# instance-based-loc/instance-based-loc

Hardware: AMD Instinct MI355X
Metric: query-frames localized/sec (embed+match+register) (higher is better)
Workload: dtype f16 (ViT MFMA operands, f32 accumulate) / f32+f64 (match, registration); 1 GPU; T: dinov2_vitb14 crops 224^2 (Q=7), 10000-instance memory (E=4), FPFH+RANSAC+coloured ICP on 5000-pt clouds, whole-memory evaluate; synthetic objects of extent U[0.15, 0.6] m on a 2.50 m grid (SURVEY 8d's U[0.2, 1.5] m re-scoped: its 5 000 points are too sparse to survive the radius-outlier removal); memory_instances=10000, points_per_object=5000, resident_feature_bytes_per_point=264, parallelism=frames-dp1+memory-replicated

## Files before the change

### include/ibloc.h

```cpp
#ifndef IBLOC_H
#define IBLOC_H

#include <stdint.h>

#ifdef __cplusplus
extern "C" {
#endif

int ibl_version(void);
const char* ibl_last_error(void);

int ibl_prof_enable(int on);
int ibl_prof_read(int id, double* ms, double* units, int64_t* launches);


#define IBL_VIT_MAX_LAYERS 32
#define IBL_VIT_LAYERSCALE 1
#define IBL_VIT_PRE_LN 2
#define IBL_VIT_FINAL_LN 4
#define IBL_VIT_QUICK_GELU 8
#define IBL_VIT_PROJ 16
#define IBL_VIT_OUT_ALL_TOKENS 32
#define IBL_VIT_ACT_TERMS2 64
#define IBL_VIT_ACT_TERMS3 128
// ... 92 lines not shown

int ibl_preprocess_depth(const float* src, const int64_t* offsets, const int32_t* sizes, int n_crops, int out_h, int out_w,
                         int patch, int patch_k_pad, float dmin, float dmax, void* patches, void* stream);


int ibl_normalize_rows(const float* in, float* out, int64_t n_rows, int dim, void* stream);

int64_t ibl_closest_similarity_workspace_bytes(int64_t n_query, int64_t n_mem_rows);
int ibl_closest_similarity(const float* det, int64_t n_query, const float* mem, int64_t n_mem_rows,
                           const int32_t* emb_offsets, int64_t n_inst, int dim, float* out_sims,
                           uint16_t* out_aug, void* workspace, int64_t workspace_bytes, void* stream);

int ibl_topk_select(const uint16_t* aug, int64_t n_rows, int64_t ld, int n_cols, int k_hi, int k_lo, int index_base,
                    uint16_t* out_val, int32_t* out_idx, int32_t* out_cnt, void* stream);

int64_t ibl_match_topk_workspace_bytes(int64_t n_query, int64_t n_mem_rows, int64_t n_inst);
int ibl_match_topk(const float* det, int64_t n_query, const float* mem, int64_t n_mem_rows, const int32_t* emb_offsets, int64_t n_inst,
                   int dim, int k_hi, int k_lo, int index_base, uint16_t* out_val, int32_t* out_idx, int32_t* out_cnt, uint16_t* out_aug,
                   void* workspace, int64_t workspace_bytes, void* stream);


int ibl_assign_batch(const uint16_t* aug_half, const int32_t* q_per_frame, int n_frames, int q_stride,
                     int M, int num_per_length, int32_t* out_assn, int32_t* out_len, int32_t* out_count,
                     int max_assn, int n_threads);

int ibl_assign_candidates(const uint16_t* cand_val, const int32_t* cand_idx, const int32_t* cand_cnt, int64_t cand_stride,
                          const int32_t* row_first, const int32_t* q_per_frame, int n_frames, int M_total, int k_hi, int k_lo,
                          int num_per_length, int32_t* out_assn, int32_t* out_len, int32_t* out_count, uint8_t* out_exact,
                          int max_assn, int n_threads);


typedef struct ibl_comm ibl_comm;
int ibl_comm_unique_id(void* out, int out_bytes);
int ibl_comm_init(ibl_comm** out, int rank, int world, const void* unique_id, int id_bytes);
int ibl_comm_destroy(ibl_comm* comm);
int ibl_allgather_topk(ibl_comm* comm, const void* send, void* recv, int64_t bytes_per_rank, void* stream);
int ibl_alltoall(ibl_comm* comm, const void* send, void* recv, int64_t bytes_per_pair, void* stream);
int ibl_allreduce_min(ibl_comm* comm, float* buf, int64_t n, void* stream);
int ibl_allreduce_max_i32(ibl_comm* comm, int32_t* buf, int64_t n, void* stream);


typedef struct ibl_reg_ctx ibl_reg_ctx;
int ibl_reg_ctx_create(ibl_reg_ctx** out, int64_t arena_bytes);
int ibl_reg_ctx_destroy(ibl_reg_ctx* ctx);
int ibl_reg_ctx_reset(ibl_reg_ctx* ctx);
int64_t ibl_reg_ctx_high_water(const ibl_reg_ctx* ctx);
int ibl_reg_ctx_status(ibl_reg_ctx* ctx, int clear);


enum { IBL_DEPTH_F32 = 0, IBL_DEPTH_U16 = 1, IBL_DEPTH_F64 = 2 };
int ibl_unproject_masks(ibl_reg_ctx* ctx, const void* depth, int depth_type, const uint8_t* rgb, const uint8_t* masks, int n_masks,
                        int H, int W, double fx, double fy, double depth_factor, float* pts4, int64_t capacity,
                        int32_t* seg_off_dev, int32_t* seg_off_host, void* stream);
int ibl_unproject_masks_f64(ibl_reg_ctx* ctx, const void* depth, int depth_type, const uint8_t* rgb, const uint8_t* masks, int n_masks,
                            int H, int W, double fx, double fy, double depth_factor, float* pts4, double* pts3_f64, double* colors3_f64,
                            int64_t capacity, int32_t* seg_off_dev, int32_t* seg_off_host, void* stream);

int ibl_radius_outlier_batch(ibl_reg_ctx* ctx, const float* pts4, const int32_t* seg_off_dev, const int32_t* seg_off_host,
                             int n_seg, double radius, int nb_points, uint8_t* keep, void* stream);

int ibl_normals_fpfh_batch(ibl_reg_ctx* ctx, const float* pts4, const int32_t* seg_off_dev, const int32_t* seg_off_host,
                           int n_seg, double radius_normal, int max_nn_normal, double radius_feature, int max_nn_feature,
                           float* normals4, float* fpfh, void* stream);

#define IBL_REG_HAVE_COLORS 1
#define IBL_REG_CENTER 2
#define IBL_REG_FIXED_BUDGET 4
int ibl_register_batch(ibl_reg_ctx* ctx, const float* det_pts4, const int32_t* det_off_dev, const int32_t* det_off_host,
                       int n_det_seg, const float* mem_pts4, const int32_t* mem_off_dev, const int32_t* mem_off_host,
                       int n_mem_seg, const int32_t* job_src_seg, const int32_t* job_tgt_seg, int n_jobs, double voxel_size,
                       double global_dist_factor, double local_dist_factor, uint64_t seed, uint32_t job_id_base,
                       int64_t ransac_max_iter, int flags, double* T_out, double* rmse_out, double* fitness_out,
                       double* means_out, double* T_ransac_out, int64_t* ransac_stats_out, void* stream);

typedef struct {
    const float* normals4;
    const float* fpfh;
    const uint16_t* fpfh_split;
    const float* fpfh_norm;
    const float* grad4;
    const float* bbox;
    double voxel_size;
    double grad_radius;
} ibl_instance_features;
int ibl_instance_features_batch(ibl_reg_ctx* ctx, const float* pts4, const int32_t* seg_off_dev, const int32_t* seg_off_host,
                                int n_seg, double voxel_size, double grad_radius, float* normals4, float* fpfh, uint16_t* fpfh_split,
                                float* fpfh_norm, float* grad4, float* bbox_host, void* stream);
int ibl_register_batch_cached(ibl_reg_ctx* ctx, const float* det_pts4, const int32_t* det_off_dev, const int32_t* det_off_host,
                              int n_det_seg, const float* mem_pts4, const int32_t* mem_off_dev, const int32_t* mem_off_host,
                              int n_mem_seg, const int32_t* job_src_seg, const int32_t* job_tgt_seg, int n_jobs, double voxel_size,
                              double global_dist_factor, double local_dist_factor, uint64_t seed, uint32_t job_id_base,
                              int64_t ransac_max_iter, int flags, const ibl_instance_features* det_features,
                              const ibl_instance_features* mem_features, double* T_out, double* rmse_out, double* fitness_out,
                              double* means_out, double* T_ransac_out, int64_t* ransac_stats_out, int64_t* reuse_stats_out,
                              void* stream);
int ibl_register_batch_ids(ibl_reg_ctx* ctx, const float* det_pts4, const int32_t* det_off_dev, const int32_t* det_off_host,
                           int n_det_seg, const float* mem_pts4, const int32_t* mem_off_dev, const int32_t* mem_off_host,
                           int n_mem_seg, const int32_t* job_src_seg, const int32_t* job_tgt_seg, const uint32_t* job_ids, int n_jobs,
                           double voxel_size, double global_dist_factor, double local_dist_factor, uint64_t seed,
                           int64_t ransac_max_iter, int flags, const ibl_instance_features* det_features,
                           const ibl_instance_features* mem_features, double* T_out, double* rmse_out, double* fitness_out,
                           double* means_out, double* T_ransac_out, int64_t* ransac_stats_out, int64_t* reuse_stats_out, void* stream);


int ibl_voxel_downsample_batch(ibl_reg_ctx* ctx, const double* points, const double* colors, const int32_t* seg_off_host, int32_t n_seg,
                               double voxel_size, double* out_points, double* out_colors, int32_t* out_counts,
                               int32_t* out_seg_off_host, void* stream);

int ibl_dbscan_batch(ibl_reg_ctx* ctx, const double* points, const int32_t* grp_off_host, int32_t n_grp, double eps, int32_t min_points,
                     int32_t* labels, int32_t* n_clusters_host, void* stream);

typedef struct ibl_memgrid ibl_memgrid;
int ibl_memgrid_build(ibl_reg_ctx* ctx, const float* mem_pts4, int64_t n, double cell, ibl_memgrid** out, void* stream);
int ibl_memgrid_destroy(ibl_memgrid* grid);

int ibl_evaluate_batch(ibl_reg_ctx* ctx, const ibl_memgrid* grid, const float* det_pts4, const int32_t* job_begin,
                       const int32_t* job_end, const double* T_global, int n_jobs, double threshold, double* rmse_out,
                       double* fitness_out, void* stream);

int ibl_register_evaluate_batch(ibl_reg_ctx* ctx, const float* det_pts4, const int32_t* det_off_dev, const int32_t* det_off_host,
                                int n_det_seg, const int32_t* q_per_frame, int n_frames, const int32_t* assn, const int32_t* assn_len,
                                const int32_t* assn_count, int max_assn, const float* mem_pts4, const int32_t* mem_off_dev,
                                const int32_t* mem_off_host, int n_mem_seg, const ibl_instance_features* mem_features,
                                const ibl_memgrid* grid, double voxel_size, double global_dist_factor, double local_dist_factor,
                                double outlier_radius, int outlier_nb_points, double eval_threshold, uint64_t seed, uint32_t job_id_base,
                                int64_t ransac_max_iter, int flags, int max_jobs, int32_t* clean_off_host, int32_t* n_jobs_out,
                                double* T_out, double* rmse_out, double* fitness_out, double* means_out, double* T_ransac_out,
                                int64_t* ransac_stats_out, int64_t* reuse_stats_out, double* T_global_out, double* full_rmse_out,
                                double* full_fitness_out, int32_t* best_out, void* stream);

int ibl_evaluate_points(ibl_reg_ctx* ctx, const ibl_memgrid* grid, const float* det_pts4, const int32_t* job_begin,
                        const int32_t* job_end, const double* T_global, int n_jobs, double threshold, float* d2_out, double* rmse_out,
                        double* fitness_out, void* stream);

int ibl_obb_iou_matrix(ibl_reg_ctx* ctx, const double* boxes, const int32_t* valid, int64_t n, double* dist,
                       int64_t* n_overlapping, void* stream);

#ifdef __cplusplus
}
#endif
#endif
```

### instance-based-loc_amd/_lib.py

```python
import ctypes as C
import os

import torch

_HERE = os.path.dirname(os.path.abspath(__file__))
LIB_PATH = os.environ.get("IBLOC_LIB") or os.path.join(_HERE, "libibloc_hip.so")


class IblError(RuntimeError):
    pass


def _load():
    if not os.path.exists(LIB_PATH):
        raise IblError(
            f"{LIB_PATH} not found: build it with `python -c 'import __graft_entry__ as g; g.build()'` "
            "(or `make -C instance-based-loc_amd/csrc`). There is no CPU fallback.")
    return C.CDLL(LIB_PATH)


lib = _load()

c_i32p = C.POINTER(C.c_int32)
c_u16p = C.POINTER(C.c_uint16)
vp = C.c_void_p

_SIGS = {
    "ibl_version": (C.c_int, []),
    "ibl_last_error": (C.c_char_p, []),
    "ibl_prof_enable": (C.c_int, [C.c_int]),
    "ibl_prof_read": (C.c_int, [C.c_int, C.POINTER(C.c_double), C.POINTER(C.c_double), C.POINTER(C.c_int64)]),
    "ibl_normalize_rows": (C.c_int, [vp, vp, C.c_int64, C.c_int, vp]),
    "ibl_closest_similarity_workspace_bytes": (C.c_int64, [C.c_int64, C.c_int64]),
    "ibl_closest_similarity": (C.c_int, [vp, C.c_int64, vp, C.c_int64, vp, C.c_int64, C.c_int, vp, vp, vp,
                                         C.c_int64, vp]),
    "ibl_preprocess_crops": (C.c_int, [vp, vp, C.c_int, C.c_int, vp, vp, C.c_int, C.c_int, C.c_int, C.c_int, C.c_int,
                                       vp, vp, vp, vp, vp]),
    "ibl_vit_workspace_bytes": (C.c_int64, [vp, C.c_int]),
    "ibl_linear_f16": (C.c_int, [vp, C.c_int64, vp, C.c_int64, vp, vp, C.c_int64, C.c_int, C.c_int, C.c_int, vp, C.c_int64, vp]),
    "ibl_vit_forward": (C.c_int, [vp, vp, vp, C.c_int, vp, vp, C.c_int64, vp]),
    "ibl_attention_f16": (C.c_int, [vp, vp, C.c_int, C.c_int, C.c_int, C.c_int, C.c_int, C.c_int, vp]),
    "ibl_layernorm_f32": (C.c_int, [vp, C.c_int64, C.c_int64, C.c_int, vp, vp, C.c_float, vp, C.c_int64, C.c_int, vp]),
    "ibl_reg_ctx_create": (C.c_int, [C.POINTER(vp), C.c_int64]),
    "ibl_reg_ctx_destroy": (C.c_int, [vp]),
    "ibl_reg_ctx_reset": (C.c_int, [vp]),
    "ibl_reg_ctx_high_water": (C.c_int64, [vp]),
    "ibl_reg_ctx_status": (C.c_int, [vp, C.c_int]),
    "ibl_unproject_masks": (C.c_int, [vp, vp, C.c_int, vp, vp, C.c_int, C.c_int, C.c_int, C.c_double, C.c_double, C.c_double, vp, C.c_int64,
                                      vp, vp, vp]),
    "ibl_voxel_downsample_batch": (C.c_int, [vp, vp, vp, vp, C.c_int32, C.c_double, vp, vp, vp, vp, vp]),
    "ibl_dbscan_batch": (C.c_int, [vp, vp, vp, C.c_int32, C.c_double, C.c_int32, vp, vp, vp]),
    "ibl_unproject_masks_f64": (C.c_int, [vp, vp, C.c_int, vp, vp, C.c_int, C.c_int, C.c_int, C.c_double, C.c_double, C.c_double, vp, vp, vp,
                                          C.c_int64, vp, vp, vp]),
    "ibl_radius_outlier_batch": (C.c_int, [vp, vp, vp, vp, C.c_int, C.c_double, C.c_int, vp, vp]),
    "ibl_normals_fpfh_batch": (C.c_int, [vp, vp, vp, vp, C.c_int, C.c_double, C.c_int, C.c_double, C.c_int, vp, vp, vp]),
    "ibl_register_batch": (C.c_int, [vp, vp, vp, vp, C.c_int, vp, vp, vp, C.c_int, vp, vp, C.c_int, C.c_double, C.c_double,
                                     C.c_double, C.c_uint64, C.c_uint32, C.c_int64, C.c_int, vp, vp, vp, vp, vp, vp, vp]),
    "ibl_instance_features_batch": (C.c_int, [vp, vp, vp, vp, C.c_int, C.c_double, C.c_double, vp, vp, vp, vp, vp, vp, vp]),
    "ibl_register_batch_cached": (C.c_int, [vp, vp, vp, vp, C.c_int, vp, vp, vp, C.c_int, vp, vp, C.c_int, C.c_double, C.c_double,
                                            C.c_double, C.c_uint64, C.c_uint32, C.c_int64, C.c_int, vp, vp, vp, vp, vp, vp, vp, vp,
                                            vp, vp]),
    "ibl_register_batch_ids": (C.c_int, [vp, vp, vp, vp, C.c_int, vp, vp, vp, C.c_int, vp, vp, vp, C.c_int, C.c_double, C.c_double,
                                         C.c_double, C.c_uint64, C.c_int64, C.c_int, vp, vp, vp, vp, vp, vp, vp, vp, vp, vp]),
    "ibl_memgrid_build": (C.c_int, [vp, vp, C.c_int64, C.c_double, C.POINTER(vp), vp]),
    "ibl_memgrid_destroy": (C.c_int, [vp]),
    "ibl_evaluate_batch": (C.c_int, [vp, vp, vp, vp, vp, vp, C.c_int, C.c_double, vp, vp, vp]),
    "ibl_register_evaluate_batch": (C.c_int, [vp, vp, vp, vp, C.c_int, vp, C.c_int, vp, vp, vp, C.c_int, vp, vp, vp, C.c_int, vp, vp,
                                              C.c_double, C.c_double, C.c_double, C.c_double, C.c_int, C.c_double, C.c_uint64, C.c_uint32,
                                              C.c_int64, C.c_int, C.c_int, vp, vp, vp, vp, vp, vp, vp, vp, vp, vp, vp, vp, vp, vp]),
    "ibl_evaluate_points": (C.c_int, [vp, vp, vp, vp, vp, vp, C.c_int, C.c_double, vp, vp, vp, vp]),
    "ibl_dator_head_workspace_bytes": (C.c_int64, [C.c_int]),
    "ibl_dator_head_forward": (C.c_int, [vp, vp, vp, C.c_int, vp, vp, C.c_int64, vp]),
    "ibl_preprocess_depth": (C.c_int, [vp, vp, vp, C.c_int, C.c_int, C.c_int, C.c_int, C.c_int, C.c_float, C.c_float, vp, vp]),
    "ibl_assign_batch": (C.c_int, [vp, vp, C.c_int, C.c_int, C.c_int, C.c_int, vp, vp, vp, C.c_int, C.c_int]),
    "ibl_assign_candidates": (C.c_int, [vp, vp, vp, C.c_int64, vp, vp, C.c_int, C.c_int, C.c_int, C.c_int, C.c_int, vp, vp, vp, vp,
                                        C.c_int, C.c_int]),
    "ibl_resample_ksize": (C.c_int, [C.c_int, C.c_int, C.c_int]),
    "ibl_resample_table": (C.c_int, [C.c_int, C.c_int, C.c_int, C.c_int, C.c_int, vp]),
    "ibl_comm_unique_id": (C.c_int, [vp, C.c_int]),
    "ibl_comm_init": (C.c_int, [vp, C.c_int, C.c_int, vp, C.c_int]),
    "ibl_comm_destroy": (C.c_int, [vp]),
    "ibl_allgather_topk": (C.c_int, [vp, vp, vp, C.c_int64, vp]),
    "ibl_alltoall": (C.c_int, [vp, vp, vp, C.c_int64, vp]),
    "ibl_allreduce_min": (C.c_int, [vp, vp, C.c_int64, vp]),
    "ibl_allreduce_max_i32": (C.c_int, [vp, vp, C.c_int64, vp]),
    "ibl_topk_select": (C.c_int, [vp, C.c_int64, C.c_int64, C.c_int, C.c_int, C.c_int, C.c_int, vp, vp, vp, vp]),
    "ibl_match_topk_workspace_bytes": (C.c_int64, [C.c_int64, C.c_int64, C.c_int64]),
    "ibl_match_topk": (C.c_int, [vp, C.c_int64, vp, C.c_int64, vp, C.c_int64, C.c_int, C.c_int, C.c_int, C.c_int, vp, vp, vp, vp, vp,
                                 C.c_int64, vp]),
    "ibl_obb_iou_matrix": (C.c_int, [vp, vp, vp, C.c_int64, vp, vp, vp]),
}


def _bind():
    for name, (res, args) in _SIGS.items():
        fn = getattr(lib, name)
        fn.restype = res
        fn.argtypes = args


_bind()


def check(status, what=""):
    if status != 0:
        msg = lib.ibl_last_error()
        raise IblError(f"{what} failed ({status}): {msg.decode() if msg else ''}")


def declared_symbols():
    return list(_SIGS.keys())
```

### instance-based-loc_amd/csrc/localise.hip

```cpp
#pragma clang fp contract(off)
#include <hip/hip_runtime.h>
#include <hipcub/hipcub.hpp>

#include <cmath>
#include <vector>

#include "ibloc.h"
#include "reg_common.h"

namespace {

struct KeepToInt {
    __host__ __device__ __forceinline__ int operator()(unsigned char v) const { return v ? 1 : 0; }
};

__global__ __launch_bounds__(256) void ibl_compact_kept_kernel(const float4* __restrict__ pts, const unsigned char* __restrict__ keep,
                                                               const int* __restrict__ pos, int n, float4* __restrict__ clean) {
    const int i = blockIdx.x * 256 + threadIdx.x;
    if (i < n && keep[i]) clean[pos[i]] = pts[i];
}

__global__ __launch_bounds__(256) void ibl_compact_offsets_kernel(const int* __restrict__ seg_off, const int* __restrict__ pos, int n_seg,
                                                                  int* __restrict__ new_off) {
    const int s = blockIdx.x * 256 + threadIdx.x;
// ... 3 lines not shown
}

extern "C" int ibl_register_evaluate_batch(ibl_reg_ctx* ctx, const float* det_pts4, const int32_t* det_off_dev, const int32_t* det_off_host,
                                           int n_det_seg, const int32_t* q_per_frame, int n_frames, const int32_t* assn,
                                           const int32_t* assn_len, const int32_t* assn_count, int max_assn, const float* mem_pts4,
                                           const int32_t* mem_off_dev, const int32_t* mem_off_host, int n_mem_seg,
                                           const ibl_instance_features* mem_features, const ibl_memgrid* grid, double voxel_size,
                                           double global_dist_factor, double local_dist_factor, double outlier_radius, int outlier_nb_points,
                                           double eval_threshold, uint64_t seed, uint32_t job_id_base, int64_t ransac_max_iter, int flags,
                                           int max_jobs, int32_t* clean_off_host, int32_t* n_jobs_out, double* T_out, double* rmse_out,
                                           double* fitness_out, double* means_out, double* T_ransac_out, int64_t* ransac_stats_out,
                                           int64_t* reuse_stats_out, double* T_global_out, double* full_rmse_out, double* full_fitness_out,
                                           int32_t* best_out, void* stream) {
    if (!ctx || !det_pts4 || !det_off_dev || !det_off_host || !q_per_frame || !assn || !assn_len || !assn_count || !mem_pts4 || !mem_off_dev ||
        !mem_off_host || !mem_features || !grid || !clean_off_host || !n_jobs_out || !T_out || !rmse_out || !fitness_out || !means_out ||
        !T_global_out || !full_rmse_out || !full_fitness_out || !best_out)
        return ibl_set_error(IBL_ERR_ARG, "ibl_register_evaluate_batch: null pointer");
    if (n_frames < 0 || n_det_seg < 0 || max_assn <= 0 || voxel_size <= 0 || outlier_radius <= 0 || eval_threshold <= 0)
        return ibl_set_error(IBL_ERR_ARG, "ibl_register_evaluate_batch: bad sizes");
    hipStream_t s = (hipStream_t)stream;
    std::vector<int> row0(n_frames + 1, 0);
    for (int f = 0; f < n_frames; ++f) {
        if (q_per_frame[f] < 0 || q_per_frame[f] > 7) return ibl_set_error(IBL_ERR_ARG, "ibl_register_evaluate_batch: q_per_frame out of range");
        row0[f + 1] = row0[f] + q_per_frame[f];
    }
    if (row0[n_frames] != n_det_seg) return ibl_set_error(IBL_ERR_ARG, "ibl_register_evaluate_batch: detections per frame do not add up to the segments");
    std::vector<int32_t> job_src, job_tgt;
    std::vector<int> job_frame, first_job(n_frames + 1, 0);
    for (int f = 0; f < n_frames; ++f) {
        const int na = assn_count[f];
        if (na < 0 || na > max_assn) return ibl_set_error(IBL_ERR_ARG, "ibl_register_evaluate_batch: assignment count out of range");
        for (int a = 0; a < na; ++a) {
            const int len = assn_len[(size_t)f * max_assn + a];
            if (len < 1 || len > 3) return ibl_set_error(IBL_ERR_ARG, "ibl_register_evaluate_batch: an assignment has 1 to 3 pairs");
            const int32_t* pr = assn + ((size_t)f * max_assn + a) * 6;
            for (int t = 0; t < 3; ++t) {
                if (t < len) {
                    if (pr[2 * t] < 0 || pr[2 * t] >= q_per_frame[f] || pr[2 * t + 1] < 0 || pr[2 * t + 1] >= n_mem_seg)
                        return ibl_set_error(IBL_ERR_ARG, "ibl_register_evaluate_batch: assignment index out of range");
                    job_src.push_back(row0[f] + pr[2 * t]);
                    job_tgt.push_back(pr[2 * t + 1]);
                } else {
                    job_src.push_back(-1);
                    job_tgt.push_back(-1);
                }
            }
            job_frame.push_back(f);
        }
        first_job[f + 1] = (int)job_frame.size();
    }
    const int J = (int)job_frame.size();
    *n_jobs_out = J;
    for (int f = 0; f < n_frames; ++f) best_out[f] = -1;
    if (J > max_jobs) return ibl_set_error(IBL_ERR_ARG, "ibl_register_evaluate_batch: %d jobs, the output arrays hold %d", J, max_jobs);

    ArenaMark mark(ctx);
    const int n = det_off_host[n_det_seg];
    unsigned char* keep; int *pos, *new_off; float4* clean;
    IBL_ARENA(keep, unsigned char, (int64_t)n + 64);
    IBL_ARENA(pos, int, (int64_t)n + 64);
    IBL_ARENA(new_off, int, n_det_seg + 2);
    IBL_ARENA(clean, float4, (int64_t)n + 1);
    for (int i = 0; i <= n_det_seg; ++i) clean_off_host[i] = 0;
    if (n > 0) {
        int st = ibl_radius_outlier_batch(ctx, det_pts4, det_off_dev, det_off_host, n_det_seg, outlier_radius, outlier_nb_points, keep, stream);
        if (st) return st;
        IBL_HIP_CHECK(hipMemsetAsync(keep + n, 0, 1, s));
        size_t tmp_bytes = 0;
        hipcub::TransformInputIterator<int, KeepToInt, const unsigned char*> flags(keep, KeepToInt());
        IBL_HIP_CHECK(hipcub::DeviceScan::ExclusiveSum(nullptr, tmp_bytes, flags, pos, n + 1, s));
        unsigned char* tmp;
        IBL_ARENA(tmp, unsigned char, (int64_t)tmp_bytes + 256);
        IBL_HIP_CHECK(hipcub::DeviceScan::ExclusiveSum(tmp, tmp_bytes, flags, pos, n + 1, s));
        hipLaunchKernelGGL(ibl_compact_kept_kernel, dim3((n + 255) / 256), dim3(256), 0, s, reinterpret_cast<const float4*>(det_pts4), keep, pos, n, clean);
        IBL_LAUNCH_CHECK();
        hipLaunchKernelGGL(ibl_compact_offsets_kernel, dim3((n_det_seg + 256) / 256), dim3(256), 0, s, det_off_dev, pos, n_det_seg, new_off);
        IBL_LAUNCH_CHECK();
        IBL_HIP_CHECK(hipMemcpyAsync(clean_off_host, new_off, sizeof(int) * (size_t)(n_det_seg + 1), hipMemcpyDeviceToHost, s));
        IBL_HIP_CHECK(hipStreamSynchronize(s));
    }
    if (J == 0) return IBL_OK;
    const int nc = clean_off_host[n_det_seg];

    float4* nrm; float* fpfh; uint16_t* split; float* fnorm;
    IBL_ARENA(nrm, float4, (int64_t)nc + 1);
    IBL_ARENA(fpfh, float, (int64_t)nc * 33 + 64);
    IBL_ARENA(split, uint16_t, (int64_t)nc * 48 + 64);
    IBL_ARENA(fnorm, float, (int64_t)nc + 64);
    std::vector<float> bbox((size_t)n_det_seg * 6 + 6, 0.0f);
    int st = ibl_instance_features_batch(ctx, reinterpret_cast<const float*>(clean), new_off, clean_off_host, n_det_seg, voxel_size, 0.0,
                                         reinterpret_cast<float*>(nrm), fpfh, split, fnorm, nullptr, bbox.data(), stream);
    if (st) return st;
    ibl_instance_features det_feat{reinterpret_cast<const float*>(nrm), fpfh, split, fnorm, nullptr, bbox.data(), voxel_size, 0.0};

    st = ibl_register_batch_cached(ctx, reinterpret_cast<const float*>(clean), new_off, clean_off_host, n_det_seg, mem_pts4, mem_off_dev,
                                   mem_off_host, n_mem_seg, job_src.data(), job_tgt.data(), J, voxel_size, global_dist_factor, local_dist_factor,
                                   seed, job_id_base, ransac_max_iter, flags, &det_feat, mem_features, T_out, rmse_out, fitness_out, means_out,
                                   T_ransac_out, ransac_stats_out, reuse_stats_out, stream);
    if (st) return st;

    std::vector<int32_t> jb(J), je(J);
    for (int j = 0; j < J; ++j) {
        const double* T = T_out + 16 * (size_t)j;
        const double* dm = means_out + 6 * (size_t)j;
        const double* mm = dm + 3;
        double* G = T_global_out + 16 * (size_t)j;
        for (int i = 0; i < 16; ++i) G[i] = T[i];
        for (int r = 0; r < 3; ++r) G[4 * r + 3] = T[4 * r + 3] + mm[r] - ((T[4 * r] * dm[0] + T[4 * r + 1] * dm[1]) + T[4 * r + 2] * dm[2]);
        const int f = job_frame[j];
        jb[j] = clean_off_host[row0[f]];
        je[j] = clean_off_host[row0[f + 1]];
    }
    st = ibl_evaluate_batch(ctx, grid, reinterpret_cast<const float*>(clean), jb.data(), je.data(), T_global_out, J, eval_threshold, full_rmse_out,
                            full_fitness_out, stream);
    if (st) return st;

    for (int f = 0; f < n_frames; ++f) {
        int best = -1;
        for (int j = first_job[f]; j < first_job[f + 1]; ++j)
            if (best < 0 || full_fitness_out[j] > full_fitness_out[best]) best = j;
        best_out[f] = best < 0 ? -1 : best - first_job[f];
    }
    return IBL_OK;
}
```

### instance-based-loc_amd/csrc/reg_api.hip

```cpp
#pragma clang fp contract(off)
#include <hip/hip_runtime.h>

#include <hipcub/hipcub.hpp>

#include <vector>

#include "ibloc.h"
#include "reg_common.h"

#ifndef KNN_CELLS_NORMAL
#define KNN_CELLS_NORMAL 3.0
#endif
#ifndef KNN_CELLS_FEATURE
#define KNN_CELLS_FEATURE 5.0
#endif

#ifndef KNN_TILE_NORMAL
#define KNN_TILE_NORMAL 4
#endif
#ifndef KNN_TILE_FEATURE
#define KNN_TILE_FEATURE 2
#endif

int ibl_launch_normals(ibl_reg_ctx* ctx, const BatchGrid& g, const float4* pts, const int* seg_off, int n, double radius, int max_nn, float4* normals,
                       int* status, hipStream_t s);
int ibl_launch_fpfh(ibl_reg_ctx* ctx, const BatchGrid& g, const float4* pts, const float4* normals, const int* seg_off, int n, double radius, int max_nn,
                    unsigned char* spfh, int* nbr_idx, float* nbr_d2, int* nbr_cnt, float* fpfh, int matching_order, int* status,
                    hipStream_t s);
int ibl_launch_radius_count(const BatchGrid& g, const float4* pts, const int* seg_off, int n, double radius, int nb_points,
                            unsigned char* keep, hipStream_t s);

bool ibl_normals_fpfh_fusable(double radius_normal, int max_nn_normal, double radius_feature, int max_nn_feature);
int ibl_launch_normals_fpfh(ibl_reg_ctx* ctx, const BatchGrid& g, const float4* pts, const int* seg_off, int n, double radius_normal,
                            int max_nn_normal, double radius_feature, int max_nn_feature, float4* normals, unsigned char* spfh, int* nbr_idx,
                            float* nbr_d2, int* nbr_cnt, float* fpfh, int matching_order, int* status, hipStream_t s);
int ibl_launch_color_grad(ibl_reg_ctx* ctx, const BatchGrid& g, const float4* pts, const float4* normals, const int* seg_off, int q0, int q1, double radius,
                          int max_nn, float4* grad, int* status, hipStream_t s);

static int ibl_bbox_to_host(ibl_reg_ctx* ctx, const float4* P, const int* seg_off_dev, int n_seg, float* bbox_host, hipStream_t s) {
    if (n_seg <= 0) return IBL_OK;
    ArenaMark m(ctx);
    float* bbox;
    IBL_ARENA(bbox, float, (int64_t)n_seg * 6 + 6);
    int st = ibl_launch_bbox(P, seg_off_dev, n_seg, bbox, s);
    if (st) return st;
    IBL_HIP_CHECK(hipMemcpyAsync(bbox_host, bbox, sizeof(float) * 6 * (size_t)n_seg, hipMemcpyDeviceToHost, s));
    IBL_HIP_CHECK(hipStreamSynchronize(s));
    return IBL_OK;
}

extern "C" int ibl_reg_ctx_create(ibl_reg_ctx** out, int64_t arena_bytes) {
    if (!out || arena_bytes < (1 << 20)) return ibl_set_error(IBL_ERR_ARG, "ibl_reg_ctx_create: bad argument");
    ibl_reg_ctx* c = new ibl_reg_ctx();
    IBL_HIP_CHECK(hipGetDevice(&c->device));
    hipError_t e = hipMalloc(reinterpret_cast<void**>(&c->base), (size_t)arena_bytes);
    if (e != hipSuccess) {
        delete c;
        return ibl_set_error(IBL_ERR_HIP, "ibl_reg_ctx_create: hipMalloc(%lld) failed: %s", (long long)arena_bytes, hipGetErrorString(e));
    }
    c->size = arena_bytes;
    c->d_status = reinterpret_cast<int*>(c->base);
    c->used = 256;
    e = hipMemset(c->base, 0, 256);
    if (e != hipSuccess) { (void)hipFree(c->base); delete c; return ibl_set_error(IBL_ERR_HIP, "ibl_reg_ctx_create: memset failed"); }
    c->pin_size = 32 << 20;
    if (hipHostMalloc(reinterpret_cast<void**>(&c->pin), (size_t)c->pin_size, hipHostMallocDefault) != hipSuccess) { c->pin = nullptr; c->pin_size = 0; }
    *out = c;
    return IBL_OK;
}

extern "C" int ibl_reg_ctx_destroy(ibl_reg_ctx* ctx) {
    if (!ctx) return IBL_OK;
    (void)hipFree(ctx->base);
    if (ctx->pin) (void)hipHostFree(ctx->pin);
    delete ctx;
    return IBL_OK;
}

extern "C" int ibl_reg_ctx_reset(ibl_reg_ctx* ctx) {
    if (!ctx) return ibl_set_error(IBL_ERR_ARG, "ibl_reg_ctx_reset: null context");
    ctx->used = 256;
    return IBL_OK;
}

extern "C" int64_t ibl_reg_ctx_high_water(const ibl_reg_ctx* ctx) { return ctx ? ctx->high_water : -1; }

extern "C" int ibl_reg_ctx_status(ibl_reg_ctx* ctx, int clear) {
    if (!ctx) return -1;
    int h = 0;
    if (hipMemcpy(&h, ctx->d_status, sizeof(int), hipMemcpyDeviceToHost) != hipSuccess) return -1;
    if (clear) (void)hipMemset(ctx->d_status, 0, sizeof(int));
    return h;
}

static int check_seg(const int32_t* seg_off_host, int n_seg, const char* who) {
    if (!seg_off_host || n_seg < 0) return ibl_set_error(IBL_ERR_ARG, "%s: bad segment table", who);
    if (seg_off_host[0] != 0) return ibl_set_error(IBL_ERR_ARG, "%s: seg_off[0] must be 0", who);
    for (int s = 0; s < n_seg; ++s)
        if (seg_off_host[s + 1] < seg_off_host[s]) return ibl_set_error(IBL_ERR_ARG, "%s: seg_off must be non-decreasing", who);
    return IBL_OK;
}

extern "C" int ibl_radius_outlier_batch(ibl_reg_ctx* ctx, const float* pts4, const int32_t* seg_off_dev, const int32_t* seg_off_host,
                                        int n_seg, double radius, int nb_points, uint8_t* keep, void* stream) {
    if (!ctx || !pts4 || !seg_off_dev || !keep || radius <= 0) return ibl_set_error(IBL_ERR_ARG, "ibl_radius_outlier_batch: bad argument");
    int st = check_seg(seg_off_host, n_seg, "ibl_radius_outlier_batch");
    if (st) return st;
    ArenaMark mark(ctx);
    hipStream_t s = (hipStream_t)stream;
    BatchGrid g;
    void* tok;
    ibl_prof_begin(IBL_PROF_ST_OUTLIER, 13.0 * (double)seg_off_host[n_seg], s, &tok);
    st = ibl_build_batch_grid(ctx, reinterpret_cast<const float4*>(pts4), seg_off_dev, seg_off_host, n_seg, (float)radius,
                              (int64_t)64 << 20, &g, s);
    if (st) return st;
    st = ibl_launch_radius_count(g, reinterpret_cast<const float4*>(pts4), seg_off_dev, seg_off_host[n_seg], radius, nb_points, keep, s);
    ibl_prof_end(tok, s);
    return st;
}

extern "C" int ibl_normals_fpfh_batch(ibl_reg_ctx* ctx, const float* pts4, const int32_t* seg_off_dev, const int32_t* seg_off_host,
                                      int n_seg, double radius_normal, int max_nn_normal, double radius_feature, int max_nn_feature,
                                      float* normals4, float* fpfh, void* stream) {
    if (!ctx || !pts4 || !seg_off_dev || !normals4 || radius_normal <= 0 || max_nn_normal <= 0)
        return ibl_set_error(IBL_ERR_ARG, "ibl_normals_fpfh_batch: bad argument");
    int st = check_seg(seg_off_host, n_seg, "ibl_normals_fpfh_batch");
    if (st) return st;
    const int n = seg_off_host[n_seg];
    ArenaMark mark(ctx);
    hipStream_t s = (hipStream_t)stream;
    const float4* P = reinterpret_cast<const float4*>(pts4);
    std::vector<float> bbox_host((size_t)n_seg * 6 + 6);
    st = ibl_bbox_to_host(ctx, P, seg_off_dev, n_seg, bbox_host.data(), s);
    if (st) return st;
    const bool fused = fpfh && radius_feature > 0 && max_nn_feature > 0 && ibl_normals_fpfh_fusable(radius_normal, max_nn_normal, radius_feature, max_nn_feature);
    if (!fused) {
        ArenaMark m2(ctx);
        BatchGrid g;
        st = ibl_build_tile_grid(ctx, P, seg_off_dev, seg_off_host, n_seg, bbox_host.data(), radius_normal, max_nn_normal, KNN_TILE_NORMAL,
                                 (int64_t)64 << 20, &g, s);
        if (st) return st;
        st = ibl_launch_normals(ctx, g, P, seg_off_dev, n, radius_normal, max_nn_normal, reinterpret_cast<float4*>(normals4), ctx->d_status, s);
        if (st) return st;
    }
    if (fpfh) {
        if (radius_feature <= 0 || max_nn_feature <= 0) return ibl_set_error(IBL_ERR_ARG, "ibl_normals_fpfh_batch: bad feature parameters");
        BatchGrid g;
        st = ibl_build_tile_grid(ctx, P, seg_off_dev, seg_off_host, n_seg, bbox_host.data(), radius_feature, max_nn_feature, KNN_TILE_FEATURE,
                                 (int64_t)64 << 20, &g, s);
        if (st) return st;
        unsigned char* spfh; int* nbr_idx; float* nbr_d2; int* nbr_cnt;
        IBL_ARENA(spfh, unsigned char, (int64_t)n * 36 + 64);
        IBL_ARENA(nbr_idx, int, (int64_t)n * max_nn_feature + 64);
        IBL_ARENA(nbr_d2, float, (int64_t)n * max_nn_feature + 64);
        IBL_ARENA(nbr_cnt, int, n + 64);
        if (fused)
            st = ibl_launch_normals_fpfh(ctx, g, P, seg_off_dev, n, radius_normal, max_nn_normal, radius_feature, max_nn_feature,
                                         reinterpret_cast<float4*>(normals4), spfh, nbr_idx, nbr_d2, nbr_cnt, fpfh, 0, ctx->d_status, s);
        else
            st = ibl_launch_fpfh(ctx, g, P, reinterpret_cast<const float4*>(normals4), seg_off_dev, n, radius_feature, max_nn_feature, spfh,
                                 nbr_idx, nbr_d2, nbr_cnt, fpfh, 0, ctx->d_status, s);
        if (st) return st;
    }
    IBL_HIP_CHECK(hipStreamSynchronize(s));
    ibl_stage_reset(ctx);
    return IBL_OK;
}

__global__ __launch_bounds__(256) void ibl_fpfh_half_kernel(const float* __restrict__ fpfh, int n, unsigned short* __restrict__ split,
                                                            float* __restrict__ norm) {
    const int i = blockIdx.x * 256 + threadIdx.x;
    if (i >= n) return;
    const float* __restrict__ x = fpfh + (int64_t)i * 33;
    const float a = fm_centred_norm(x);
    norm[i] = a;
    if (!split) return;
    uint4* dst = reinterpret_cast<uint4*>(split + (int64_t)i * 48);
#pragma unroll
    for (int pc = 0; pc < 6; ++pc) {
        float x8[8];
#pragma unroll
        for (int e = 0; e < 8; ++e) x8[e] = 8 * pc + e < 33 ? x[8 * pc + e] : 0.0f;
        const fm_piece_t r = fm_operand_piece(x8, a, pc);
        uint4 v;
        __builtin_memcpy(&v, &r, 16);
        dst[pc] = v;
    }
}

int ibl_features_on_batch(ibl_reg_ctx* ctx, const float4* P, const int* seg_off_dev, const int* seg_off_host, int n_seg, const float* bbox_host,
                          double voxel_size, double grad_radius, int gq0, int gq1, float4* normals, float* fpfh, unsigned short* fpfh_split,
                          float* fpfh_norm, float4* grad, hipStream_t s) {
    const int n = seg_off_host[n_seg];
    if (n <= 0) return IBL_OK;
    int st;
    std::vector<float> own_bbox;
    if (!bbox_host) {
        own_bbox.resize((size_t)n_seg * 6 + 6);
        st = ibl_bbox_to_host(ctx, P, seg_off_dev, n_seg, own_bbox.data(), s);
        if (st) return st;
        bbox_host = own_bbox.data();
    }
    const bool fused = fpfh && ibl_normals_fpfh_fusable(voxel_size * 2, 30, voxel_size * 5, 100);
    if (!fused) {
        ArenaMark mA(ctx);
        BatchGrid gA;
        st = ibl_build_tile_grid(ctx, P, seg_off_dev, seg_off_host, n_seg, bbox_host, voxel_size * 2, 30, KNN_TILE_NORMAL, (int64_t)128 << 20, &gA, s);
        if (st) return st;
        st = ibl_launch_normals(ctx, gA, P, seg_off_dev, n, voxel_size * 2, 30, normals, ctx->d_status, s);
        if (st) return st;
    }
    if (fpfh) {
        ArenaMark mB(ctx);
        BatchGrid gB;
        st = ibl_build_tile_grid(ctx, P, seg_off_dev, seg_off_host, n_seg, bbox_host, voxel_size * 5, 100, KNN_TILE_FEATURE, (int64_t)128 << 20, &gB, s);
        if (st) return st;
        unsigned char* spfh; float* nbr_d2; int *nbr_idx, *nbr_cnt;
        IBL_ARENA(spfh, unsigned char, (int64_t)n * 36 + 64);
        IBL_ARENA(nbr_idx, int, (int64_t)n * 100 + 64);
        IBL_ARENA(nbr_d2, float, (int64_t)n * 100 + 64);
        IBL_ARENA(nbr_cnt, int, n + 64);
        if (fused) st = ibl_launch_normals_fpfh(ctx, gB, P, seg_off_dev, n, voxel_size * 2, 30, voxel_size * 5, 100, normals, spfh, nbr_idx, nbr_d2, nbr_cnt,
                                                fpfh, 1, ctx->d_status, s);
        else st = ibl_launch_fpfh(ctx, gB, P, normals, seg_off_dev, n, voxel_size * 5, 100, spfh, nbr_idx, nbr_d2, nbr_cnt, fpfh, 1, ctx->d_status, s);
        if (st) return st;
        if (fpfh_norm) {
            hipLaunchKernelGGL(ibl_fpfh_half_kernel, dim3((unsigned)((n + 255) / 256)), dim3(256), 0, s, fpfh, n, fpfh_split, fpfh_norm);
            IBL_LAUNCH_CHECK();
        }
    }
    if (grad && gq1 > gq0) {
        if (grad_radius <= 0) return ibl_set_error(IBL_ERR_ARG, "colour gradients need a positive radius");
        ArenaMark mG(ctx);
        BatchGrid gG;
        st = ibl_build_tile_grid(ctx, P, seg_off_dev, seg_off_host, n_seg, bbox_host, grad_radius, 30, KNN_TILE_NORMAL, (int64_t)128 << 20, &gG, s);
        if (st) return st;
        st = ibl_launch_color_grad(ctx, gG, P, normals, seg_off_dev, gq0, gq1, grad_radius, 30, grad, ctx->d_status, s);
        if (st) return st;
    }
    return IBL_OK;
}

extern "C" int ibl_instance_features_batch(ibl_reg_ctx* ctx, const float* pts4, const int32_t* seg_off_dev, const int32_t* seg_off_host,
                                           int n_seg, double voxel_size, double grad_radius, float* normals4, float* fpfh,
                                           uint16_t* fpfh_split, float* fpfh_norm, float* grad4, float* bbox_host, void* stream) {
    if (!ctx || !pts4 || !seg_off_dev || !normals4 || !fpfh || !fpfh_norm || voxel_size <= 0)
        return ibl_set_error(IBL_ERR_ARG, "ibl_instance_features_batch: bad argument");
    if (grad4 && grad_radius <= 0) return ibl_set_error(IBL_ERR_ARG, "ibl_instance_features_batch: colour gradients need grad_radius > 0");
    int st = check_seg(seg_off_host, n_seg, "ibl_instance_features_batch");
    if (st) return st;
    ArenaMark mark(ctx);
    hipStream_t s = (hipStream_t)stream;
    const float4* P = reinterpret_cast<const float4*>(pts4);
    std::vector<float> own_bbox;
    if (!bbox_host) { own_bbox.resize((size_t)n_seg * 6 + 6); bbox_host = own_bbox.data(); }
    if (n_seg > 0) {
        st = ibl_bbox_to_host(ctx, P, seg_off_dev, n_seg, bbox_host, s);
        if (st) return st;
    }
    void* tok;
    ibl_prof_begin(IBL_PROF_ST_FEATURES, 444.0 * (double)(n_seg > 0 ? seg_off_host[n_seg] : 0), s, &tok);
    const int64_t total_pts = n_seg > 0 ? (int64_t)seg_off_host[n_seg] : 0;
    const int64_t cap_pts = (int64_t)3 << 19;
    const int64_t n_chunks = std::max<int64_t>(1, (total_pts + cap_pts - 1) / cap_pts);
    const int64_t chunk_pts = std::min<int64_t>(cap_pts, (total_pts + n_chunks - 1) / n_chunks + 65536);
    std::vector<int> rebased;
    for (int s0 = 0; s0 < n_seg;) {
        int s1 = s0 + 1;
        while (s1 < n_seg && (int64_t)seg_off_host[s1 + 1] - seg_off_host[s0] <= chunk_pts) ++s1;
        const int o0 = seg_off_host[s0], ns = s1 - s0;
        ArenaMark mc(ctx);
        const int* off_dev = seg_off_dev;
        const int* off_host = seg_off_host;
        if (!(s0 == 0 && s1 == n_seg)) {
            rebased.resize(ns + 1);
            for (int i = 0; i <= ns; ++i) rebased[i] = seg_off_host[s0 + i] - o0;
            int* d;
            IBL_ARENA(d, int, ns + 1);
            st = ibl_stage_upload(ctx, d, rebased.data(), sizeof(int) * (int64_t)(ns + 1), s);
            if (st) return st;
            off_dev = d;
            off_host = rebased.data();
        }
        const int cnt = off_host[ns];
        st = ibl_features_on_batch(ctx, P + o0, off_dev, off_host, ns, bbox_host + 6 * (size_t)s0, voxel_size, grad_radius, 0, grad4 ? cnt : 0,
                                   reinterpret_cast<float4*>(normals4) + o0, fpfh + (int64_t)o0 * 33, fpfh_split ? fpfh_split + (int64_t)o0 * 48 : nullptr,
                                   fpfh_norm + o0, grad4 ? reinterpret_cast<float4*>(grad4) + o0 : nullptr, s);
        if (st) return st;
        s0 = s1;
        if (ctx->pin_used > ctx->pin_size / 2) {
            IBL_HIP_CHECK(hipStreamSynchronize(s));
            ibl_stage_reset(ctx);
        }
    }
    ibl_prof_end(tok, s);
    IBL_HIP_CHECK(hipStreamSynchronize(s));
    ibl_stage_reset(ctx);
    return IBL_OK;
}

__device__ __forceinline__ double depth_at(const void* depth, int type, int64_t p) {
    return type == 1 ? (double)reinterpret_cast<const unsigned short*>(depth)[p]
                     : (type == 2 ? reinterpret_cast<const double*>(depth)[p] : (double)reinterpret_cast<const float*>(depth)[p]);
}
__device__ __forceinline__ double depth_z(const void* depth, int type, int64_t p, double factor) {
    if (type == 0) return (double)(reinterpret_cast<const float*>(depth)[p] / (float)factor);
    return depth_at(depth, type, p) / factor;
}

__global__ __launch_bounds__(256) void ibl_unproject_flag_kernel(const void* __restrict__ depth, int is_u16, const unsigned char* __restrict__ masks,
                                                                 int64_t HW, int64_t total, double depth_factor, int* __restrict__ flags) {
    const int64_t t = (int64_t)blockIdx.x * 256 + threadIdx.x;
    if (t >= total) return;
    const int64_t p = t % HW;
    const double z = depth_z(depth, is_u16, p, depth_factor);
    flags[t] = (masks[t] != 0 && z != 0.0) ? 1 : 0;
}

__global__ __launch_bounds__(256) void ibl_unproject_write_kernel(const void* __restrict__ depth, int is_u16, const unsigned char* __restrict__ rgb,
                                                                  const int* __restrict__ flags, const int* __restrict__ pos, int64_t HW, int W,
                                                                  int64_t total, const float* __restrict__ hx, const float* __restrict__ vy,
                                                                  double fx, double fy, double depth_factor, int64_t capacity,
                                                                  float4* __restrict__ out, double* __restrict__ out_pts64, double* __restrict__ out_cols64) {
    const int64_t t = (int64_t)blockIdx.x * 256 + threadIdx.x;
    if (t >= total || !flags[t]) return;
    const int o = pos[t];
    if (o >= capacity) return;
    const int64_t p = t % HW;
    const int row = (int)(p / W), col = (int)(p - (int64_t)row * W);
    const double z = depth_z(depth, is_u16, p, depth_factor);
    double x, y;
    if (is_u16 == 0) {
        const float zf = (float)z;
        x = (double)((hx[col] * zf) / (float)fx);
        y = (double)((vy[row] * zf) / (float)fy);
    } else {
        x = (double)hx[col] * z / fx;
        y = (double)vy[row] * z / fy;
    }
    const float r = (float)rgb[3 * p] / 255.0f, g = (float)rgb[3 * p + 1] / 255.0f, b = (float)rgb[3 * p + 2] / 255.0f;
    const double inten = ((double)r + (double)g + (double)b) / 3.0;
    out[o] = make_float4((float)x, (float)y, (float)z, (float)inten);
    if (out_pts64) {
        out_pts64[3 * (int64_t)o] = x; out_pts64[3 * (int64_t)o + 1] = y; out_pts64[3 * (int64_t)o + 2] = is_u16 == 0 ? (double)(float)z : z;
    }
    if (out_cols64) { out_cols64[3 * (int64_t)o] = (double)r; out_cols64[3 * (int64_t)o + 1] = (double)g; out_cols64[3 * (int64_t)o + 2] = (double)b; }
}

static void linspace_f32(double start, double stop, int num, std::vector<float>& out) {
    out.resize(num);
    if (num == 1) { out[0] = (float)start; return; }
    const double step = (stop - start) / (double)(num - 1);
    for (int i = 0; i < num; ++i) {
        volatile double prod = (double)i * step;
        out[i] = (float)(prod + start);
    }
    out[num - 1] = (float)stop;
}

extern "C" int ibl_unproject_masks_f64(ibl_reg_ctx* ctx, const void* depth, int depth_type, const uint8_t* rgb, const uint8_t* masks,
                                       int n_masks, int H, int W, double fx, double fy, double depth_factor, float* pts4, double* pts3_f64,
                                       double* colors3_f64, int64_t capacity, int32_t* seg_off_dev, int32_t* seg_off_host, void* stream);

extern "C" int ibl_unproject_masks(ibl_reg_ctx* ctx, const void* depth, int depth_type, const uint8_t* rgb, const uint8_t* masks,
                                   int n_masks, int H, int W, double fx, double fy, double depth_factor, float* pts4, int64_t capacity,
                                   int32_t* seg_off_dev, int32_t* seg_off_host, void* stream) {
    return ibl_unproject_masks_f64(ctx, depth, depth_type, rgb, masks, n_masks, H, W, fx, fy, depth_factor, pts4, nullptr, nullptr, capacity,
                                   seg_off_dev, seg_off_host, stream);
}

extern "C" int ibl_unproject_masks_f64(ibl_reg_ctx* ctx, const void* depth, int depth_type, const uint8_t* rgb, const uint8_t* masks,
                                       int n_masks, int H, int W, double fx, double fy, double depth_factor, float* pts4, double* pts3_f64,
                                       double* colors3_f64, int64_t capacity, int32_t* seg_off_dev, int32_t* seg_off_host, void* stream) {
    if (!ctx || !seg_off_dev || !seg_off_host || n_masks < 0 || (n_masks > 0 && (!depth || !rgb || !masks || !pts4)) || H <= 0 || W <= 0 || fx == 0 || fy == 0 ||
        depth_factor == 0 || capacity < 0 || depth_type < 0 || depth_type > 2)
        return ibl_set_error(IBL_ERR_ARG, "ibl_unproject_masks: bad argument");
// ... 40 lines not shown
```

### instance-based-loc_amd/csrc/reg_common.h

```cpp
#pragma once
#include <hip/hip_runtime.h>

#include <cstdint>

#include "ibl_common.h"

struct SegGrid {
    float minx, miny, minz, inv;
    int nx, ny, nz;
    int cell_base;
};

struct BatchGrid {
    const SegGrid* seg;
    const int* cell_start;
    const float4* sorted_pts;
    const int* order;
    int n_seg;
    const int* tile_base;
    const int* tile_seg;
    int n_tiles;
    int ts;
};

struct ibl_reg_ctx {
    unsigned char* base = nullptr;
    int64_t size = 0;
    int64_t used = 0;
    int64_t high_water = 0;
    int device = 0;
    int* d_status = nullptr;
    unsigned char* pin = nullptr;
    int64_t pin_size = 0;
    int64_t pin_used = 0;
};

int ibl_stage_upload(ibl_reg_ctx* ctx, void* dst_dev, const void* src_host, int64_t bytes, hipStream_t s);
static inline void ibl_stage_reset(ibl_reg_ctx* ctx) { ctx->pin_used = 0; }

struct ArenaMark {
    ibl_reg_ctx* ctx;
    int64_t mark;
    explicit ArenaMark(ibl_reg_ctx* c) : ctx(c), mark(c->used) {}
    ~ArenaMark() { ctx->used = mark; }
};

template <typename T>
static inline T* arena_alloc(ibl_reg_ctx* ctx, int64_t count, bool* ok) {
    int64_t bytes = ibl_align_up(count * (int64_t)sizeof(T), 256);
    if (bytes < 256) bytes = 256;
    if (ctx->used + bytes > ctx->size) {
        *ok = false;
        return nullptr;
    }
    T* p = reinterpret_cast<T*>(ctx->base + ctx->used);
    ctx->used += bytes;
    if (ctx->used > ctx->high_water) ctx->high_water = ctx->used;
    return p;
}

#define IBL_ARENA(ptr, type, count)                                                                  \
    do {                                                                                             \
        bool _ok = true;                                                                             \
        ptr = arena_alloc<type>(ctx, (count), &_ok);                                                 \
        if (!_ok)                                                                                    \
            return ibl_set_error(IBL_ERR_ARENA, "device arena exhausted (%lld of %lld bytes used, need %lld more) at %s:%d", \
                                 (long long)ctx->used, (long long)ctx->size,                         \
                                 (long long)((count) * (int64_t)sizeof(type)), __FILE__, __LINE__);  \
    } while (0)

#define IBL_ERR_ARENA (-5)
#define IBL_ERR_OVERFLOW (-6)

#define IBL_ST_GRID_OVERFLOW 1
#define IBL_ST_KNN_SLOWPATH 2
#define IBL_ST_FEAT_OVERFLOW 4
#define IBL_ST_RANSAC_OVERFLOW 8
#define IBL_ST_FEAT_REDONE 16
#define IBL_ST_RANSAC_REDONE 32

int ibl_build_batch_grid(ibl_reg_ctx* ctx, const float4* pts, const int* seg_off_dev, const int* seg_off_host, int n_seg,
                         float cell, int64_t max_cells, BatchGrid* out, hipStream_t s);
int ibl_build_batch_grid_bounded(ibl_reg_ctx* ctx, const float4* pts, const int* seg_off_dev, const int* seg_off_host, int n_seg,
                                 float cell, int64_t cells_bound, BatchGrid* out, hipStream_t s);
double ibl_knn_safety();
int ibl_knn_rho();
int ibl_build_tile_grid(ibl_reg_ctx* ctx, const float4* pts, const int* seg_off_dev, const int* seg_off_host, int n_seg,
                        const float* bbox_host, double radius, int max_nn, int ts, int64_t max_cells, BatchGrid* out, hipStream_t s);

int ibl_launch_bbox(const float4* pts, const int* seg_off_dev, int n_seg, float* bbox_dev, hipStream_t s);

struct FeatSources { const float4* normals[3]; const float* fpfh[3]; const float4* grad[3]; const unsigned short* split[3]; const float* norm[3]; };
struct FeatPair { int qkind, qsrc, qcnt, dkind, dsrc, dcnt, out, pad; };

int ibl_feat_search_mfma(ibl_reg_ctx* ctx, const FeatPair* d_pairs, int n_pairs, int max_q, const FeatSources& src, int* pair_idx,
                         float* pair_d2, const int* need_pos, const int* need_list, int out0, int64_t out_count, bool* overflow,
                         hipStream_t s);

int ibl_features_on_batch(ibl_reg_ctx* ctx, const float4* P, const int* seg_off_dev, const int* seg_off_host, int n_seg, const float* bbox_host, double voxel_size,
                          double grad_radius, int gq0, int gq1, float4* normals, float* fpfh, unsigned short* fpfh_split, float* fpfh_norm,
                          float4* grad, hipStream_t s);

#ifdef __HIPCC__
__device__ __constant__ const float FM_MU[33] = {87.f, 46.f, 101.f, 26.f, 28.f, 17.f, 26.f, 26.f, 17.f, 14.f, 21.f, 7.f, 14.f, 19.f, 7.f, 8.f, 14.f,
                                                 6.f,  8.f,  13.f,  6.f,  5.f,  11.f, 6.f,  5.f,  10.f, 6.f,  3.f,  7.f,  14.f, 3.f, 6.f,  14.f};
typedef __attribute__((ext_vector_type(8))) _Float16 fm_piece_t;
struct __attribute__((aligned(4))) ibl_u4_a4 { unsigned x, y, z, w; };
__device__ __forceinline__ float fm_centred_norm(const float* __restrict__ x) {
    float a = 0.0f;
    for (int k = 0; k < 33; ++k) { const float v = x[k] - FM_MU[k]; a = __builtin_fmaf(v, v, a); }
    return a;
}
__device__ __forceinline__ fm_piece_t fm_operand_piece(const float* x8, float a, int pc) {
    fm_piece_t r;
#pragma unroll
    for (int e = 0; e < 8; ++e) r[e] = (_Float16)0.0f;
    if (pc < 4) {
#pragma unroll
        for (int e = 0; e < 8; ++e) r[e] = (_Float16)(x8[e] - FM_MU[8 * pc + e]);
    } else if (pc == 4) {
        const float w = a * 0.125f;
        const _Float16 nh = (_Float16)w, nl = (_Float16)(w - (float)nh);
        const float cw = 1.0e-3f * a + 4.0e-3f;
        _Float16 cu = (_Float16)cw;
        if ((float)cu < cw) cu = __builtin_bit_cast(_Float16, (unsigned short)(__builtin_bit_cast(unsigned short, cu) + 1));
        r[0] = (_Float16)(x8[0] - FM_MU[32]);
        r[1] = (_Float16)8.0f; r[2] = (_Float16)8.0f; r[3] = nh; r[4] = nl; r[5] = cu;
    }
    return r;
}
__device__ __forceinline__ int seg_of(const int* __restrict__ seg_off, int n_seg, int i) {
    int lo = 0, hi = n_seg;
    while (hi - lo > 1) {
        int mid = (lo + hi) >> 1;
        if (seg_off[mid] <= i) lo = mid; else hi = mid;
    }
    return lo;
}

__device__ __forceinline__ int cell_clamp(float v, float mn, float inv, int n) {
    int c = (int)floorf((v - mn) * inv);
    return c < 0 ? 0 : (c >= n ? n - 1 : c);
}

__device__ __forceinline__ float dist2f(float ax, float ay, float az, float bx, float by, float bz) {
    const float dx = ax - bx, dy = ay - by, dz = az - bz;
    return __builtin_fmaf(dz, dz, __builtin_fmaf(dy, dy, dx * dx));
}

__device__ __forceinline__ double wave_sum_d(double v) {
#pragma unroll
    for (int off = 32; off >= 1; off >>= 1) v += __shfl_xor(v, off, 64);
    return v;
}
__device__ __forceinline__ int wave_sum_i(int v) {
#pragma unroll
    for (int off = 32; off >= 1; off >>= 1) v += __shfl_xor(v, off, 64);
    return v;
}

__device__ __forceinline__ void cross3d(const double* a, const double* b, double* o) {
    o[0] = a[1] * b[2] - a[2] * b[1]; o[1] = a[2] * b[0] - a[0] * b[2]; o[2] = a[0] * b[1] - a[1] * b[0];
}
__device__ __forceinline__ double dot3d(const double* a, const double* b) { return a[0] * b[0] + a[1] * b[1] + a[2] * b[2]; }

__device__ __forceinline__ void xform_d(const double* T, double x, double y, double z, double* o) {
    o[0] = T[0] * x + T[1] * y + T[2] * z + T[3];
    o[1] = T[4] * x + T[5] * y + T[6] * z + T[7];
    o[2] = T[8] * x + T[9] * y + T[10] * z + T[11];
}

__device__ __forceinline__ void philox4x32(unsigned c0, unsigned c1, unsigned c2, unsigned c3, unsigned k0, unsigned k1,
                                           unsigned* out) {
#pragma unroll
    for (int r = 0; r < 10; ++r) {
        const unsigned long long p0 = (unsigned long long)0xD2511F53u * c0, p1 = (unsigned long long)0xCD9E8D57u * c2;
        const unsigned n0 = (unsigned)(p1 >> 32) ^ c1 ^ k0, n1 = (unsigned)p1, n2 = (unsigned)(p0 >> 32) ^ c3 ^ k1, n3 = (unsigned)p0;
        c0 = n0; c1 = n1; c2 = n2; c3 = n3;
        k0 += 0x9E3779B9u; k1 += 0xBB67AE85u;
    }
    out[0] = c0; out[1] = c1; out[2] = c2; out[3] = c3;
}

__device__ inline void jacobi_eig3_d(double A[3][3], double V[3][3], double* w) {
// ... 90 lines not shown
```

### instance-based-loc_amd/csrc/reg_knn.hip

```cpp
#pragma clang fp contract(off)
#include <hip/hip_runtime.h>

#include <algorithm>
#include <cstdio>
#include <cstdlib>

#include "reg_common.h"

#define KNN_BINS 256
#ifndef KNN_ROWS
#define KNN_ROWS 8
#endif
#define KNN_CAPB 256
#ifndef KNN_TILE_CAP3
#define KNN_TILE_CAP3 1600
#endif
#ifndef KNN_GUESS_SHIFT
#define KNN_GUESS_SHIFT 2
#endif

__device__ __forceinline__ int wave_incl_scan_i(int v) {
    v += __builtin_amdgcn_update_dpp(0, v, 0x111, 0xf, 0xf, false);
    v += __builtin_amdgcn_update_dpp(0, v, 0x112, 0xf, 0xf, false);
    v += __builtin_amdgcn_update_dpp(0, v, 0x114, 0xf, 0xf, false);
// ... 1457 lines not shown
};
struct ListNormalFactory {
    static constexpr bool WIDE = true;
    typedef NoPending Pending;
    unsigned* nrm_mask; int* nbr_idx; float* nbr_d2; int* nbr_cnt; int K; float rn2; int kn;
    template <class Acc> __device__ void flush(Pending*, const Acc&) const {}
    template <class Acc> __device__ void flush_block(Pending*, const Acc&) const {}
    template <class Acc> __device__ ListNormalConsumer<Acc> make(int qi, const float4&, WaveLds* L, const Acc& acc, Pending* = nullptr) const {
        ListNormalConsumer<Acc> c;
        c.nrm_mask = nrm_mask; c.acc = acc; c.nbr_idx = nbr_idx; c.nbr_d2 = nbr_d2; c.nbr_cnt = nbr_cnt; c.K = K; c.rn2 = rn2; c.kn = kn;
        c.qi = qi; c.L = L; c.ncount = 0;
        return c;
    }
};
struct GradFactory {
    static constexpr bool WIDE = false;
    typedef NoPending Pending;
    const float4* normals; float4* grad;
    template <class Acc> __device__ void flush(Pending*, const Acc&) const {}
    template <class Acc> __device__ void flush_block(Pending*, const Acc&) const {}
    template <class Acc> __device__ GradConsumer<Acc> make(int qi, const float4& q, WaveLds* L, const Acc& acc, Pending* = nullptr) const {
        GradConsumer<Acc> c;
        c.normals = normals; c.acc = acc; c.grad = grad; c.qi = qi; c.q = q; c.qn = normals[qi]; c.L = L; c.ncount = 0;
        return c;
    }
};

template <int TS, int CAP, class Factory, int NW = 4, bool PACK = false, int OCC = 1>
__global__ __launch_bounds__(NW * 64, OCC) void ibl_knn_tile_kernel(BatchGrid g, float radius, float r2, int max_nn, NeedPop need_pop, Factory fac,
                                                              int q_lo, int q_hi, int* __restrict__ fb_list, int* __restrict__ fb_count) {
    __shared__ TileLds<CAP, PACK> T;
    __shared__ WaveLds wl[NW];
    __shared__ typename Factory::Pending pend[NW];
#ifdef KNN_LAB_PAD_LDS
    __shared__ int lab_pad[KNN_LAB_PAD_LDS / 4];
    if (threadIdx.x == 0 && q_lo == -12345) lab_pad[max_nn] = 1;
#endif
    tile_knn_block<TS, NW>(g, radius, r2, max_nn, need_pop, fb_list, fb_count, fac, q_lo, q_hi, T, wl, pend);
}

template <class Factory>
__global__ __launch_bounds__(256) void ibl_knn_list_kernel(BatchGrid g, const int* __restrict__ seg_off, float radius, float r2, int max_nn,
                                                           Factory fac, const int* __restrict__ list, const int* __restrict__ count, int* status) {
    __shared__ WaveLds lds[4];
    const int n = *count;
    for (int e = blockIdx.x * 4 + (threadIdx.x >> 6); e < n; e += gridDim.x * 4) {
        const int jq = list[e];
        const int qi = g.order[jq];
        const float4 q = g.sorted_pts[jq];
        const int s = seg_of(seg_off, g.n_seg, qi);
        auto cons = fac.template make<GlobalAcc>(qi, q, &lds[threadIdx.x >> 6], GlobalAcc{g.sorted_pts, g.order});
        hybrid_select(g, g.seg[s], q, qi, radius, r2, max_nn, &lds[threadIdx.x >> 6], cons, status);
    }
}

template <class Factory>
__global__ __launch_bounds__(256) void ibl_knn_query_kernel(BatchGrid g, const float4* __restrict__ pts, const int* __restrict__ seg_off,
                                                            float radius, float r2, int max_nn, Factory fac, int q0, int q1, int* status) {
    __shared__ WaveLds lds[4];
    const int qi = q0 + blockIdx.x * 4 + (threadIdx.x >> 6);
    if (qi >= q1) return;
    const int s = seg_of(seg_off, g.n_seg, qi);
    const float4 q = pts[qi];
    auto cons = fac.template make<GlobalAcc>(qi, q, &lds[threadIdx.x >> 6], GlobalAcc{g.sorted_pts, g.order});
    hybrid_select(g, g.seg[s], q, qi, radius, r2, max_nn, &lds[threadIdx.x >> 6], cons, status);
}

__constant__ int FEAT_POS[33] = {29, 23, 17, 11, 5, 2, 8, 14, 20, 26, 32, 27, 21, 15, 9, 3, 0, 6, 12, 18, 24, 30, 28, 22, 16, 10, 4, 1, 7, 13, 19, 25, 31};

__device__ __forceinline__ float spfh_value(const unsigned char* __restrict__ spfh_cnt, const int* __restrict__ nbr_cnt, int j, int b) {
    const int kj = nbr_cnt[j];
    if (kj <= 1) return 0.0f;
    return (float)((double)spfh_cnt[(int64_t)j * 36 + b] * (100.0 / (double)(kj - 1)));
}

struct FpfhTile {
    unsigned char cnt[64][36];
    double w[64];
};

#define FPFH_Q 7
__global__ __launch_bounds__(256) void ibl_fpfh_kernel(const unsigned char* __restrict__ spfh_cnt, const int* __restrict__ nbr_idx,
                                                       const float* __restrict__ nbr_d2, const int* __restrict__ nbr_cnt, int K, int n,
                                                       int matching_order, float* __restrict__ fpfh) {
    __shared__ FpfhTile tiles[FPFH_Q];
    __shared__ double accs[FPFH_Q][33];
    __shared__ int kq[FPFH_Q];
    const int tid = threadIdx.x;
    const int q0 = IBL_XCD_BLOCK(blockIdx.x, gridDim.x) * FPFH_Q;
    if (tid < FPFH_Q) kq[tid] = q0 + tid < n ? nbr_cnt[q0 + tid] : 0;
    __syncthreads();
    int kmax = 0;
#pragma unroll
    for (int u = 0; u < FPFH_Q; ++u) kmax = max(kmax, kq[u]);
    const int qq = tid / 33, b = tid - qq * 33;
    const bool mine = qq < FPFH_Q && q0 + qq < n;
    const int qi = q0 + qq;
    const int k = mine ? kq[qq] : 0;
    double acc = 0.0;
    for (int t0 = 0; t0 < kmax; t0 += 64) {
        for (int e = tid; e < FPFH_Q * 64; e += 256) {
            const int sq = e >> 6, r = e & 63, t = t0 + r, si = q0 + sq;
            if (si < n && t < kq[sq]) {
                FpfhTile& S = tiles[sq];
                const int j = nbr_idx[(int64_t)si * K + t];
                const double dist = (double)nbr_d2[(int64_t)si * K + t];
                const int kj = nbr_cnt[j];
                const unsigned char* src = spfh_cnt + (int64_t)j * 36;
                const ibl_u4_a4 r0 = *reinterpret_cast<const ibl_u4_a4*>(src), r1 = *reinterpret_cast<const ibl_u4_a4*>(src + 16);
                const unsigned r2w = *reinterpret_cast<const unsigned*>(src + 32);
                unsigned int* dst = reinterpret_cast<unsigned int*>(S.cnt[r]);
                dst[0] = r0.x; dst[1] = r0.y; dst[2] = r0.z; dst[3] = r0.w; dst[4] = r1.x; dst[5] = r1.y; dst[6] = r1.z; dst[7] = r1.w; dst[8] = r2w;
                S.w[r] = (j == si || dist == 0.0 || kj <= 1) ? 0.0 : (100.0 / (double)(kj - 1)) / dist;
            }
        }
        __syncthreads();
        if (mine && k > 1) {
            const FpfhTile& T = tiles[qq];
            const int m = min(64, k - t0);
            for (int r = 0; r < m; ++r)
                acc = fma(__hiloint2double(0x43300000, (int)T.cnt[r][b]) - 4503599627370496.0, T.w[r], acc);
        }
        __syncthreads();
    }
    if (mine) accs[qq][b] = acc;
    __syncthreads();
    if (mine) {
        double sum = 0.0;
        const int blk = b / 11;
        for (int t = 0; t < 11; ++t) sum += accs[qq][blk * 11 + t];
        float out = 0.0f;
        if (k > 1) {
            const double sc = sum != 0.0 ? 100.0 / sum : 0.0;
            out = (float)(acc * sc + (double)spfh_value(spfh_cnt, nbr_cnt, qi, b));
        }
        fpfh[(int64_t)qi * 33 + (matching_order ? FEAT_POS[b] : b)] = out;
    }
}

__global__ __launch_bounds__(256) void ibl_radius_count_kernel(BatchGrid g, const float4* __restrict__ pts, const int* __restrict__ seg_off,
                                                               float radius, float r2, int nb_points, unsigned char* __restrict__ keep) {
    const int n = seg_off[g.n_seg];
    const int qi = blockIdx.x * 256 + threadIdx.x;
    if (qi >= n) return;
    const SegGrid sg = g.seg[seg_of(seg_off, g.n_seg, qi)];
    const float4 q = pts[qi];
    int reach = (int)ceilf(radius * sg.inv);
    if (reach < 1) reach = 1;
    const int cx = cell_clamp(q.x, sg.minx, sg.inv, sg.nx), cy = cell_clamp(q.y, sg.miny, sg.inv, sg.ny),
              cz = cell_clamp(q.z, sg.minz, sg.inv, sg.nz);
    int cnt = 0;
    for (int z = max(cz - reach, 0); z <= min(cz + reach, sg.nz - 1) && cnt <= nb_points; ++z)
        for (int y = max(cy - reach, 0); y <= min(cy + reach, sg.ny - 1) && cnt <= nb_points; ++y) {
            const int row = sg.cell_base + (z * sg.ny + y) * sg.nx;
            const int b = g.cell_start[row + max(cx - reach, 0)], e = g.cell_start[row + min(cx + reach, sg.nx - 1) + 1];
            for (int j = b; j < e && cnt <= nb_points; j += 4) {
                float4 p[4];
#pragma unroll
                for (int v = 0; v < 4; ++v) p[v] = g.sorted_pts[min(j + v, e - 1)];
#pragma unroll
                for (int v = 0; v < 4; ++v) cnt += (j + v < e && dist2f(q.x, q.y, q.z, p[v].x, p[v].y, p[v].z) < r2) ? 1 : 0;
            }
        }
    keep[qi] = cnt > nb_points ? 1 : 0;
}

static NeedPop need_pop_table(int max_nn, int ts) {
    NeedPop np;
    np.v[0] = 0.f;
    for (int rho = 1; rho < 8; ++rho)
        np.v[rho] = (float)(ibl_knn_safety() * max_nn * (ts + 2.0 * rho) * (ts + 2.0 * rho) / (3.14159265358979 * rho * rho));
    np.rho_start = ibl_knn_rho();
    const char* e = getenv("IBL_KNN_NOGUESS");
    np.guess = (e && atoi(e)) ? 0 : 1;
    return np;
}

template <class Factory>
static int launch_knn(ibl_reg_ctx* ctx, const BatchGrid& g, const float4* pts, const int* seg_off, int n, int q0, int q1, double radius, int max_nn,
                      const Factory& fac, int* status, hipStream_t s) {
    if (q1 <= q0) return IBL_OK;
    const float r = (float)radius, r2 = (float)(radius * radius);
    if (g.tile_base && g.n_tiles > 0) {
        ArenaMark m(ctx);
        int *fb_list, *fb_count;
        IBL_ARENA(fb_list, int, (int64_t)n + 64);
        IBL_ARENA(fb_count, int, 64);
        IBL_HIP_CHECK(hipMemsetAsync(fb_count, 0, sizeof(int), s));
        const NeedPop np = need_pop_table(max_nn, g.ts);
        bool packed = false;
        if constexpr (Factory::WIDE) {
            if (g.ts == 2) {
                packed = true;
#ifdef KNN_LAB_NW
                hipLaunchKernelGGL((ibl_knn_tile_kernel<2, KNN_TILE_CAP3, Factory, KNN_LAB_NW, true, KNN_LAB_OCC>), dim3(g.n_tiles), dim3(64 * KNN_LAB_NW), 0, s, g, r, r2, max_nn, np, fac, q0, q1, fb_list, fb_count);
#else
                hipLaunchKernelGGL((ibl_knn_tile_kernel<2, KNN_TILE_CAP3, Factory, 4, true, 3>), dim3(g.n_tiles), dim3(256), 0, s, g, r, r2, max_nn, np, fac, q0, q1, fb_list, fb_count);
#endif
            }
        }
        if (packed) {}
        else
        if (g.ts == 2) hipLaunchKernelGGL((ibl_knn_tile_kernel<2, 2560, Factory>), dim3(g.n_tiles), dim3(256), 0, s, g, r, r2, max_nn, np, fac, q0, q1, fb_list, fb_count);
        else if (g.ts == 4) hipLaunchKernelGGL((ibl_knn_tile_kernel<4, 1024, Factory>), dim3(g.n_tiles), dim3(256), 0, s, g, r, r2, max_nn, np, fac, q0, q1, fb_list, fb_count);
        else return ibl_set_error(IBL_ERR_INTERNAL, "k-NN tiles of %d^3 cells are not built", g.ts);
        IBL_LAUNCH_CHECK();
#ifdef KNN_LAB_CLK
        { unsigned long long h[16]; (void)hipStreamSynchronize(s); (void)hipMemcpyFromSymbol(h, HIP_SYMBOL(knn_lab_clk), sizeof(h));
          const double nt = (double)std::max<unsigned long long>(h[6], 1);
          fprintf(stderr, "[knn-clk] k=%d ts=%d tiles with queries %llu (%.1f queries each): clocks (100 MHz ticks) per tile: query rows %.0f, rho loop %.0f, staging %.0f, "
                  "pilot %.0f, queries(wave 0) %.0f, flush %.0f\n", max_nn, g.ts, h[6], (double)h[7] / nt, h[0] / nt, h[1] / nt, h[2] / nt, h[3] / nt, h[4] / nt, h[5] / nt);
          const double nq0 = (double)h[7] / 4.0;
          fprintf(stderr, "[knn-clk]   per query of wave 0: pass 1 %.0f, threshold %.0f, pass 2 %.0f, boundary rank %.0f, consumer finish %.0f\n", h[8] / nq0, h[9] / nq0,
                  h[10] / nq0, h[11] / nq0, h[12] / nq0);
          fprintf(stderr, "[knn-clk]   consumer finish: index sort %.0f, list write %.0f, inner selection %.0f\n", h[13] / nq0, h[14] / nq0, h[15] / nq0);
          unsigned long long z[16] = {0}; (void)hipMemcpyToSymbol(HIP_SYMBOL(knn_lab_clk), z, sizeof(z)); }
#endif
#ifdef KNN_LAB_STATS
        { int h[8]; (void)hipMemcpyFromSymbol(h, HIP_SYMBOL(knn_lab_stats), sizeof(h)); fprintf(stderr, "[knn-lab] k=%d queries %d from_list %d select_all %d guess_low %d overflow %d\n", max_nn, h[0], h[1], h[2], h[3], h[4]); int z[8] = {0}; (void)hipMemcpyToSymbol(HIP_SYMBOL(knn_lab_stats), z, sizeof(z)); }
#endif
        const int blocks = std::max(1, std::min(2048, (q1 - q0 + 3) / 4));
        hipLaunchKernelGGL((ibl_knn_list_kernel<Factory>), dim3(blocks), dim3(256), 0, s, g, seg_off, r, r2, max_nn, fac, fb_list, fb_count, status);
        if (getenv("IBL_KNN_DEBUG")) {
            int h = 0;
            (void)hipMemcpyAsync(&h, fb_count, sizeof(int), hipMemcpyDeviceToHost, s);
            (void)hipStreamSynchronize(s);
            fprintf(stderr, "[knn] r=%.3f k=%d ts=%d tiles=%d queries=%d fallback=%d (%.1f %%)\n", radius, max_nn, g.ts, g.n_tiles, q1 - q0, h, 100.0 * h / (q1 - q0));
        }
    } else {
        hipLaunchKernelGGL((ibl_knn_query_kernel<Factory>), dim3((q1 - q0 + 3) / 4), dim3(256), 0, s, g, pts, seg_off, r, r2, max_nn, fac, q0, q1, status);
    }
    IBL_LAUNCH_CHECK();
    return IBL_OK;
}

int ibl_launch_normals(ibl_reg_ctx* ctx, const BatchGrid& g, const float4* pts, const int* seg_off, int n, double radius, int max_nn, float4* normals,
                       int* status, hipStream_t s) {
    if (n <= 0) return IBL_OK;
    if (max_nn > 256) return ibl_set_error(IBL_ERR_UNSUPPORTED, "normals: max_nn %d > 256", max_nn);
    void* tok;
    ibl_prof_begin(IBL_PROF_NORMALS, 24.0 * (double)n, s, &tok);
    const int st = launch_knn(ctx, g, pts, seg_off, n, 0, n, radius, max_nn, NormalFactory{normals}, status, s);
    ibl_prof_end(tok, s);
    return st;
}

int ibl_launch_fpfh(ibl_reg_ctx* ctx, const BatchGrid& g, const float4* pts, const float4* normals, const int* seg_off, int n, double radius, int max_nn,
                    unsigned char* spfh, int* nbr_idx, float* nbr_d2, int* nbr_cnt, float* fpfh, int matching_order, int* status,
                    hipStream_t s) {
    if (n <= 0) return IBL_OK;
    if (max_nn > 256) return ibl_set_error(IBL_ERR_UNSUPPORTED, "fpfh: max_nn %d > 256 (SPFH histograms are stored as bytes)", max_nn);
    void* tok;
    ibl_prof_begin(IBL_PROF_SPFH, 156.0 * (double)n, s, &tok);
    const int st = launch_knn(ctx, g, pts, seg_off, n, 0, n, radius, max_nn, SpfhFactory{normals, spfh, nbr_idx, nbr_d2, nbr_cnt, max_nn}, status, s);
    ibl_prof_end(tok, s);
    if (st) return st;
    hipLaunchKernelGGL(ibl_fpfh_kernel, dim3((n + FPFH_Q - 1) / FPFH_Q), dim3(256), 0, s, spfh, nbr_idx, nbr_d2, nbr_cnt, max_nn, n, matching_order, fpfh);
    IBL_LAUNCH_CHECK();
    return IBL_OK;
}

__global__ __launch_bounds__(256) void ibl_normals_from_mask_kernel(const float4* __restrict__ pts, const int* __restrict__ nbr_idx, int K,
                                                                    const unsigned* __restrict__ nrm_mask, int n, float4* __restrict__ normals) {
    const int qi = IBL_XCD_BLOCK(blockIdx.x, gridDim.x) * 256 + threadIdx.x;
    if (qi >= n) return;
    const uint4 m4 = *reinterpret_cast<const uint4*>(nrm_mask + 4 * (int64_t)qi);
    const unsigned w[4] = {m4.x, m4.y, m4.z, m4.w};
    double c[9];
#pragma unroll
    for (int t = 0; t < 9; ++t) c[t] = 0.0;
    int k = 0;
#pragma unroll
    for (int u = 0; u < 4; ++u) {
        unsigned bits = w[u];
        while (bits) {
            int t[8];
#pragma unroll
            for (int v = 0; v < 8; ++v) {
                t[v] = -1;
                if (bits) { t[v] = 32 * u + __ffs((int)bits) - 1; bits &= bits - 1u; }
            }
            int j[8];
#pragma unroll
            for (int v = 0; v < 8; ++v) j[v] = nbr_idx[(int64_t)qi * K + (t[v] >= 0 ? t[v] : 0)];
            float4 p[8];
#pragma unroll
            for (int v = 0; v < 8; ++v) p[v] = pts[j[v]];
#pragma unroll
            for (int v = 0; v < 8; ++v) {
                if (t[v] < 0) continue;
                const double x = p[v].x, y = p[v].y, z = p[v].z;
                c[0] += x; c[1] += y; c[2] += z;
                c[3] += x * x; c[4] += x * y; c[5] += x * z; c[6] += y * y; c[7] += y * z; c[8] += z * z;
                ++k;
            }
        }
    }
    normal_from_moments(c, k, qi, normals);
}

#define SPFH_NQ 256
#define SPFH_QSTRIDE 64
template <bool FAST>
__global__ __launch_bounds__(256) void ibl_spfh_lists_kernel(const float4* __restrict__ pts, const float4* __restrict__ normals,
                                                             const int* __restrict__ nbr_idx, const int* __restrict__ nbr_cnt, int K, int n,
                                                             unsigned char* __restrict__ spfh_cnt, int2* __restrict__ queue, int* __restrict__ q_count,
                                                             int q_cap) {
    __shared__ int hists[4][36];
    __shared__ int stash[4][FAST ? 128 : 1];
    const int lane = threadIdx.x & 63, wave = threadIdx.x >> 6;
    if (!FAST && q_count != nullptr && q_count[SPFH_NQ * SPFH_QSTRIDE] == 0) return;
    int* hist = hists[wave];
  for (int qi = IBL_XCD_BLOCK(blockIdx.x, gridDim.x) * 4 + wave; qi < n; qi += gridDim.x * 4) {
    if (lane < 36) hist[lane] = 0;
    wave_lds_sync();
    const int k = nbr_cnt[qi];
    const float4 q = pts[qi], qn = normals[qi];
    int n_unsure = 0;
    for (int t0 = 0; t0 < k; t0 += 64) {
        const int t = t0 + lane;
        const int jo = t < k ? nbr_idx[(int64_t)qi * K + t] : qi;
        bool unsure = false;
        if (jo != qi) {
            if (FAST) {
                int b0, b1, b2;
                if (pair_bins_f32(q, qn, pts[jo], normals[jo], &b0, &b1, &b2)) {
                    atomicAdd(&hist[b0], 1);
                    atomicAdd(&hist[11 + b1], 1);
                    atomicAdd(&hist[22 + b2], 1);
                } else {
                    unsure = true;
                }
            } else {
                double f[3];
                pair_features_d(q, qn, pts[jo], normals[jo], f);
                atomicAdd(&hist[clamp_bin11((int)f[0])], 1);
                atomicAdd(&hist[11 + clamp_bin11((int)floor(11 * (f[1] + 1.0) * 0.5))], 1);
                atomicAdd(&hist[22 + clamp_bin11((int)floor(11 * (f[2] + 1.0) * 0.5))], 1);
            }
        }
        if (FAST) {
            const unsigned long long m = __ballot(unsure);
            if (unsure) stash[wave][(n_unsure + __popcll(m & ((1ull << lane) - 1ull))) & 127] = jo;
            n_unsure += __popcll(m);
        }
    }
    wave_lds_sync();
    if (lane < 36) spfh_cnt[(int64_t)qi * 36 + lane] = lane < 33 ? (unsigned char)hist[lane] : (unsigned char)0;
    if (FAST && n_unsure > 0) {
        const int qsel = blockIdx.x & (SPFH_NQ - 1);
        int base = 0;
        if (lane == 0) base = atomicAdd(&q_count[qsel * SPFH_QSTRIDE], n_unsure);
        base = __shfl(base, 0, 64);
        if (base + n_unsure <= q_cap) {
            for (int e = lane; e < n_unsure; e += 64) queue[(int64_t)qsel * q_cap + base + e] = make_int2(qi, stash[wave][e]);
        } else if (lane == 0) {
            q_count[SPFH_NQ * SPFH_QSTRIDE] = 1;
        }
    }
    wave_lds_sync();
  }
}

__global__ __launch_bounds__(256) void ibl_spfh_queue_kernel(const float4* __restrict__ pts, const float4* __restrict__ normals,
                                                             const int2* __restrict__ queue, const int* __restrict__ q_count, int q_cap,
                                                             unsigned char* __restrict__ spfh_cnt) {
    if (q_count[SPFH_NQ * SPFH_QSTRIDE] != 0) return;
    const int qsel = blockIdx.x & (SPFH_NQ - 1), part = blockIdx.x / SPFH_NQ, parts = gridDim.x / SPFH_NQ;
    const int total = min(q_count[qsel * SPFH_QSTRIDE], q_cap);
    for (int e = part * 256 + threadIdx.x; e < total; e += parts * 256) {
        const int2 pr = queue[(int64_t)qsel * q_cap + e];
        double f[3];
        pair_features_d(pts[pr.x], normals[pr.x], pts[pr.y], normals[pr.y], f);
        const int b[3] = {clamp_bin11((int)f[0]), 11 + clamp_bin11((int)floor(11 * (f[1] + 1.0) * 0.5)), 22 + clamp_bin11((int)floor(11 * (f[2] + 1.0) * 0.5))};
        unsigned* words = reinterpret_cast<unsigned*>(spfh_cnt + (int64_t)pr.x * 36);
#pragma unroll
        for (int c = 0; c < 3; ++c) atomicAdd(&words[b[c] >> 2], 1u << (8 * (b[c] & 3)));
    }
}

bool ibl_normals_fpfh_fusable(double radius_normal, int max_nn_normal, double radius_feature, int max_nn_feature) {
    const char* e = getenv("IBL_FEAT_UNFUSED");
    const bool off = e && atoi(e);
    return !off && radius_normal <= radius_feature && max_nn_normal <= max_nn_feature && max_nn_normal <= NP_MAXK && max_nn_feature <= 128;
}
int ibl_launch_normals_fpfh(ibl_reg_ctx* ctx, const BatchGrid& g, const float4* pts, const int* seg_off, int n, double radius_normal,
                            int max_nn_normal, double radius_feature, int max_nn_feature, float4* normals, unsigned char* spfh, int* nbr_idx,
                            float* nbr_d2, int* nbr_cnt, float* fpfh, int matching_order, int* status, hipStream_t s) {
    if (n <= 0) return IBL_OK;
    ArenaMark mk(ctx);
    unsigned* nrm_mask;
    IBL_ARENA(nrm_mask, unsigned, 4 * (int64_t)n + 64);
    void* tok;
    ibl_prof_begin(IBL_PROF_SPFH, 156.0 * (double)n, s, &tok);
    const int st = launch_knn(ctx, g, pts, seg_off, n, 0, n, radius_feature, max_nn_feature,
                              ListNormalFactory{nrm_mask, nbr_idx, nbr_d2, nbr_cnt, max_nn_feature, (float)(radius_normal * radius_normal), max_nn_normal},
                              status, s);
    ibl_prof_end(tok, s);
    if (st) return st;
    hipLaunchKernelGGL(ibl_normals_from_mask_kernel, dim3((n + 255) / 256), dim3(256), 0, s, pts, nbr_idx, max_nn_feature, nrm_mask, n, normals);
    IBL_LAUNCH_CHECK();
    {
        const char* e64 = getenv("IBL_SPFH_F64");
        bool fast = !(e64 && atoi(e64));
        if (fast) {
            int64_t cap64 = std::min<int64_t>((int64_t)n * max_nn_feature / (16 * SPFH_NQ) + 256, (int64_t)1 << 20);
            if (const char* ec = getenv("IBL_SPFH_QCAP")) cap64 = std::max<int64_t>(1, atoll(ec));
            int2* queue; int* q_count;
            IBL_ARENA(queue, int2, cap64 * SPFH_NQ);
            IBL_ARENA(q_count, int, SPFH_NQ * SPFH_QSTRIDE + 64);
            IBL_HIP_CHECK(hipMemsetAsync(q_count, 0, sizeof(int) * (SPFH_NQ * SPFH_QSTRIDE + 1), s));
            hipLaunchKernelGGL(ibl_spfh_lists_kernel<true>, dim3((n + 3) / 4), dim3(256), 0, s, pts, normals, nbr_idx, nbr_cnt, max_nn_feature, n, spfh,
                               queue, q_count, (int)cap64);
            IBL_LAUNCH_CHECK();
            hipLaunchKernelGGL(ibl_spfh_queue_kernel, dim3(SPFH_NQ * 4), dim3(256), 0, s, pts, normals, queue, q_count, (int)cap64, spfh);
            IBL_LAUNCH_CHECK();
            hipLaunchKernelGGL(ibl_spfh_lists_kernel<false>, dim3(2048), dim3(256), 0, s, pts, normals, nbr_idx, nbr_cnt, max_nn_feature, n, spfh,
                               (int2*)nullptr, q_count, (int)cap64);
            IBL_LAUNCH_CHECK();
            if (const char* es = getenv("IBL_SPFH_STATS"); es && atoi(es)) {
                std::vector<int> cnt(SPFH_NQ * SPFH_QSTRIDE + 1);
                IBL_HIP_CHECK(hipMemcpyAsync(cnt.data(), q_count, sizeof(int) * cnt.size(), hipMemcpyDeviceToHost, s));
                IBL_HIP_CHECK(hipStreamSynchronize(s));
                long long tot = 0; int mx = 0;
                for (int i = 0; i < SPFH_NQ; ++i) { tot += cnt[i * SPFH_QSTRIDE]; mx = std::max(mx, cnt[i * SPFH_QSTRIDE]); }
                fprintf(stderr, "[ibloc] spfh: %lld undecided pairs of at most %lld; fullest queue %d of %lld; overflow %d\n", tot,
                        (long long)n * max_nn_feature, mx, (long long)cap64, cnt.back());
            }
        } else {
            hipLaunchKernelGGL(ibl_spfh_lists_kernel<false>, dim3((n + 3) / 4), dim3(256), 0, s, pts, normals, nbr_idx, nbr_cnt, max_nn_feature, n, spfh,
                               (int2*)nullptr, (int*)nullptr, 0);
            IBL_LAUNCH_CHECK();
        }
    }
    if (fpfh) {
        hipLaunchKernelGGL(ibl_fpfh_kernel, dim3((n + FPFH_Q - 1) / FPFH_Q), dim3(256), 0, s, spfh, nbr_idx, nbr_d2, nbr_cnt, max_nn_feature, n, matching_order, fpfh);
        IBL_LAUNCH_CHECK();
    }
    return IBL_OK;
}

int ibl_launch_color_grad(ibl_reg_ctx* ctx, const BatchGrid& g, const float4* pts, const float4* normals, const int* seg_off, int q0, int q1, double radius,
                          int max_nn, float4* grad, int* status, hipStream_t s) {
    if (q1 <= q0) return IBL_OK;
    if (max_nn > 256) return ibl_set_error(IBL_ERR_UNSUPPORTED, "colour gradient: max_nn %d > 256", max_nn);
    return launch_knn(ctx, g, pts, seg_off, q1, q0, q1, radius, max_nn, GradFactory{normals, grad}, status, s);
}

int ibl_launch_radius_count(const BatchGrid& g, const float4* pts, const int* seg_off, int n, double radius, int nb_points,
                            unsigned char* keep, hipStream_t s) {
    if (n <= 0) return IBL_OK;
    hipLaunchKernelGGL(ibl_radius_count_kernel, dim3((n + 255) / 256), dim3(256), 0, s, g, pts, seg_off, (float)radius,
                       (float)(radius * radius), nb_points, keep);
    IBL_LAUNCH_CHECK();
    return IBL_OK;
}
```

### instance-based-loc_amd/csrc/reg_match.hip

```cpp
#pragma clang fp contract(off)
#include <hip/hip_runtime.h>

#include <hipcub/hipcub.hpp>

#include <algorithm>
#include <array>
#include <cmath>
#include <cstdlib>
#include <map>
#include <vector>

#include "ibloc.h"
#include "reg_common.h"
#include "reg_stages.h"

#define FEATCOPY_GRAD 4

__global__ __launch_bounds__(256) void ibl_group_gather_kernel(const GroupDesc* __restrict__ groups, int G, const float4* __restrict__ det,
                                                               const int* __restrict__ det_off, const float4* __restrict__ mem,
                                                               const int* __restrict__ mem_off, const int* __restrict__ grp_off,
                                                               float4* __restrict__ out) {
    const int n = grp_off[G];
    const int i = blockIdx.x * 256 + threadIdx.x;
    if (i >= n) return;
    const int g = seg_of(grp_off, G, i);
    int local = i - grp_off[g];
    const float4* pool = groups[g].pool ? mem : det;
    const int* off = groups[g].pool ? mem_off : det_off;
    float4 p = make_float4(0.f, 0.f, 0.f, 0.f);
    for (int t = 0; t < 3; ++t) {
        const int sg = groups[g].seg[t];
        if (sg < 0) continue;
        const int len = off[sg + 1] - off[sg];
        if (local < len) { p = pool[off[sg] + local]; break; }
        local -= len;
    }
    out[i] = p;
}

#define NEAR_SPLIT 8
#define NEAR_CAP 5120

__device__ __forceinline__ float box_dist2(const float* bx, float x, float y, float z) {
    const float dx = fmaxf(fmaxf(bx[0] - x, x - bx[3]), 0.0f), dy = fmaxf(fmaxf(bx[1] - y, y - bx[4]), 0.0f),
                dz = fmaxf(fmaxf(bx[2] - z, z - bx[5]), 0.0f);
    return dx * dx + dy * dy + dz * dz;
}

__global__ __launch_bounds__(256) void ibl_near_pair_kernel(const NearPair* __restrict__ pairs, const float4* __restrict__ det,
                                                            const int* __restrict__ det_off, const float4* __restrict__ mem,
                                                            const int* __restrict__ mem_off, float R2, int* __restrict__ flags) {
    const NearPair P = pairs[blockIdx.y];
    const float4* pool = P.pool ? mem : det;
    const int* off = P.pool ? mem_off : det_off;
    const int ab = off[P.a], ae = off[P.a + 1], bb = off[P.b], be = off[P.b + 1];
    __shared__ float sx[NEAR_CAP], sy[NEAR_CAP], sz[NEAR_CAP];
    __shared__ int nb, found;
    if (threadIdx.x == 0) { nb = 0; found = 0; }
    __syncthreads();
    for (int i = bb + threadIdx.x; i < be; i += 256) {
        const float4 p = pool[i];
        if (box_dist2(P.boxa, p.x, p.y, p.z) < R2) {
            const int pos = atomicAdd(&nb, 1);
            if (pos < NEAR_CAP) { sx[pos] = p.x; sy[pos] = p.y; sz[pos] = p.z; }
        }
    }
    __syncthreads();
    const int n = nb;
    if (n > NEAR_CAP) { if (threadIdx.x == 0) atomicOr(&flags[blockIdx.y], 1); return; }
    if (n == 0) return;
    for (int i0 = ab + blockIdx.x * 256; i0 < ae; i0 += NEAR_SPLIT * 256) {
        const int i = i0 + threadIdx.x;
        bool hit = false;
        if (i < ae) {
            const float4 p = pool[i];
            if (box_dist2(P.boxb, p.x, p.y, p.z) < R2)
                for (int j = 0; j < n; ++j)
                    if (dist2f(p.x, p.y, p.z, sx[j], sy[j], sz[j]) < R2) { hit = true; break; }
        }
        if (hit) found = 1;
        __syncthreads();
        if (found) break;
    }
    if (threadIdx.x == 0 && found) atomicOr(&flags[blockIdx.y], 1);
}

__global__ __launch_bounds__(256) void ibl_feat_assemble_kernel(const FeatCopy* __restrict__ copies, FeatSources src, float4* __restrict__ normals,
                                                                float* __restrict__ fpfh, float4* __restrict__ grad) {
    const FeatCopy c = copies[blockIdx.y];
    const int k = c.kind & 3;
    if (fpfh) {
        const float* sf = src.fpfh[k] + (int64_t)c.src * 33;
        float* df = fpfh + (int64_t)c.dst * 33;
        const int nf = c.count * 33;
        for (int i = blockIdx.x * 256 + threadIdx.x; i < nf; i += gridDim.x * 256) df[i] = sf[i];
    }
    const float4* sn = src.normals[k] + c.src;
    const float4* sg = src.grad[k] + c.src;
    const bool want_grad = (c.kind & FEATCOPY_GRAD) != 0;
    for (int i = blockIdx.x * 256 + threadIdx.x; i < c.count; i += gridDim.x * 256) {
        normals[c.dst + i] = sn[i];
        if (want_grad) grad[c.dst + i] = sg[i];
    }
}

#define FT_TILE 32

template <bool INDEXED>
__global__ __launch_bounds__(256) void ibl_feat_pair_nn_kernel(const FeatPair* __restrict__ pairs, FeatSources src, int* __restrict__ out_idx,
                                                               float* __restrict__ out_d2, const int* __restrict__ need_pos,
                                                               const int* __restrict__ need_list, int out0) {
    const FeatPair P = pairs[blockIdx.y];
    const int q0 = blockIdx.x * 256;
    int n_q = P.qcnt, l0 = 0;
    if (INDEXED) { l0 = need_pos[P.out - out0]; n_q = need_pos[P.out - out0 + P.qcnt] - l0; }
    if (q0 >= n_q) return;
    const float* __restrict__ qf = src.fpfh[P.qkind] + (int64_t)P.qsrc * 33;
    const float* __restrict__ df = src.fpfh[P.dkind] + (int64_t)P.dsrc * 33;
    const bool valid = q0 + (int)threadIdx.x < n_q;
    const int qv = valid ? q0 + (int)threadIdx.x : n_q - 1;
    const int qi = INDEXED ? need_list[l0 + qv] - (P.out - out0) : qv;
    float f[33];
    {
        const float* s = qf + (int64_t)qi * 33;
#pragma unroll
        for (int k = 0; k < 33; ++k) f[k] = s[k];
    }
    __shared__ __attribute__((aligned(16))) float tiles[2][FT_TILE * 36];
    constexpr int PRE = (FT_TILE * 33 + 255) / 256;
    float pre[PRE];
    auto fetch = [&](int t0) {
        const int nt = min(FT_TILE, P.dcnt - t0) * 33;
        const float* __restrict__ g = df + (int64_t)t0 * 33;
#pragma unroll
        for (int i = 0; i < PRE; ++i) { const int e = threadIdx.x + 256 * i; pre[i] = e < nt ? g[e] : 0.0f; }
    };
    auto stash = [&](float* __restrict__ tile) {
#pragma unroll
        for (int i = 0; i < PRE; ++i) {
            const int e = threadIdx.x + 256 * i;
            if (e < FT_TILE * 33) { const int r = e / 33; tile[r * 36 + (e - r * 33)] = pre[i]; }
        }
    };
    float best = INFINITY;
    int bj = 0;
    fetch(0);
    stash(tiles[0]);
    __syncthreads();
    int cur = 0;
    for (int t0 = 0; t0 < P.dcnt; t0 += FT_TILE, cur ^= 1) {
        const bool more = t0 + FT_TILE < P.dcnt;
        if (more) fetch(t0 + FT_TILE);
        const float* __restrict__ tile = tiles[cur];
        const int nt = min(FT_TILE, P.dcnt - t0);
        for (int t = 0; t < nt; ++t) {
            const float* __restrict__ row = tile + t * 36;
            float acc = 0.0f;
#define FT_STAGE(k0, k1)                                                                                       \
            _Pragma("unroll") for (int k = k0; k < k1; ++k) { const float d = f[k] - row[k]; acc = __builtin_fmaf(d, d, acc); }
// ... 38 lines not shown
        dbase += S.dcnt[b];
    }
    nn[i] = bj;
}

__global__ __launch_bounds__(256) void ibl_feat_need_kernel(const SidePairs* __restrict__ sides, const FeatPair* __restrict__ pairs,
                                                            const int* __restrict__ job_off, int J, const int* __restrict__ nn, int out0,
                                                            int* __restrict__ need) {
    const int ns = job_off[J];
    const int i = blockIdx.x * 256 + threadIdx.x;
    if (i >= ns) return;
    const int j = seg_of(job_off, J, i);
    const SidePairs S = sides[j];
    int local = nn[i], b = 0;
    if (local >= S.dcnt[0] + S.dcnt[1] + S.dcnt[2]) return;
    while (b < 2 && local >= S.dcnt[b]) { local -= S.dcnt[b]; ++b; }
    const SidePairs T = sides[J + j];
#pragma unroll
    for (int a = 0; a < 3; ++a) {
        const int p = T.pair[b][a];
        if (p >= 0) need[pairs[p].out - out0 + local] = 1;
    }
}

__global__ __launch_bounds__(256) void ibl_feat_need_list_kernel(const int* __restrict__ need, const int* __restrict__ pos, int n,
                                                                 int* __restrict__ list) {
    const int e = blockIdx.x * 256 + threadIdx.x;
    if (e < n && need[e]) list[pos[e]] = e;
}

__global__ __launch_bounds__(256) void ibl_mutual_kernel(const int* __restrict__ nn, const int* __restrict__ job_off, int J, int mutual,
                                                         int min_mutual, int2* __restrict__ corr ,
                                                         int* __restrict__ n_corr) {
    const int j = blockIdx.x;
    const int sb = job_off[j], se = job_off[j + 1], tb = job_off[J + j], te = job_off[J + j + 1];
    const int ns = se - sb, nt = te - tb;
    __shared__ int wave_cnt[4];
    __shared__ int base;
    if (threadIdx.x == 0) base = 0;
    __syncthreads();
    if (ns == 0 || nt == 0) { if (threadIdx.x == 0) n_corr[j] = 0; return; }
    const int lane = threadIdx.x & 63, wave = threadIdx.x >> 6;
    if (mutual) {
        for (int i0 = 0; i0 < ns; i0 += 256) {
            const int i = i0 + threadIdx.x;
            bool keep = false;
            int tj = 0;
            if (i < ns) { tj = nn[sb + i]; keep = nn[tb + tj] == i; }
            const unsigned long long m = __ballot(keep);
            if (lane == 0) wave_cnt[wave] = __popcll(m);
            __syncthreads();
            int pre = base;
            for (int w = 0; w < wave; ++w) pre += wave_cnt[w];
            if (keep) corr[sb + pre + __popcll(m & ((1ull << lane) - 1ull))] = make_int2(i, tj);
            __syncthreads();
            if (threadIdx.x == 0) base += wave_cnt[0] + wave_cnt[1] + wave_cnt[2] + wave_cnt[3];
            __syncthreads();
        }
        if (base >= min_mutual) { if (threadIdx.x == 0) n_corr[j] = base; return; }
    }
    for (int i = threadIdx.x; i < ns; i += 256) corr[sb + i] = make_int2(i, nn[sb + i]);
    if (threadIdx.x == 0) n_corr[j] = ns;
}

static double box_gap2(const float* ba, const float* bb) {
    double g2 = 0;
    for (int c = 0; c < 3; ++c) {
        const double gap = std::max(0.0, std::max((double)ba[c] - (double)bb[3 + c], (double)bb[c] - (double)ba[3 + c]));
        g2 += gap * gap;
    }
    return g2;
}

static void list_near_candidates(const HostTables& h, double R, MatchPlan* plan) {
    for (int sgi = 0; sgi < 2 * h.J; ++sgi) {
        const int pl = sgi >= h.J ? 1 : 0, j = pl ? sgi - h.J : sgi;
        if (!h.bbox[pl]) continue;
        const int* segs = pl ? h.jobs[j].tgt_seg : h.jobs[j].src_seg;
        for (int a = 0; a < 3; ++a)
            for (int b = a + 1; b < 3; ++b) {
                if (segs[a] < 0 || segs[b] < 0) continue;
                const std::array<int, 3> key = {pl, std::min(segs[a], segs[b]), std::max(segs[a], segs[b])};
                const float *ba = h.bbox[pl] + 6 * (size_t)key[1], *bb = h.bbox[pl] + 6 * (size_t)key[2];
                if (plan->near_id.count(key) || box_gap2(ba, bb) >= R * R) continue;
                NearPair np;
                np.pool = pl; np.a = key[1]; np.b = key[2]; np.pad = 0;
                for (int c = 0; c < 6; ++c) { np.boxa[c] = ba[c]; np.boxb[c] = bb[c]; }
                plan->near_id[key] = (int)plan->near.size();
                plan->near.push_back(np);
            }
    }
    plan->near_flag.assign(plan->near.size(), 0);
}

static void plan_feature_reuse(const HostTables& h, MatchPlan* plan) {
    std::map<std::array<int, 4>, int> gid[2];
    std::vector<std::array<int, 4>> gkeys[2];
    std::vector<SlotPlan>& slots = plan->slots;
    slots.reserve((size_t)6 * h.J);
    int64_t pts_cached = 0;
    for (int sgi = 0; sgi < 2 * h.J; ++sgi) {
        const int pl = sgi >= h.J ? 1 : 0, j = pl ? sgi - h.J : sgi;
        const int* segs = pl ? h.jobs[j].tgt_seg : h.jobs[j].src_seg;
        const int* off = h.off[pl];
        bool dirty[3] = {false, false, false};
        for (int a = 0; a < 3; ++a) {
            if (segs[a] < 0) continue;
            if (!h.bbox[pl]) { dirty[a] = true; continue; }
            for (int b = 0; b < 3; ++b) {
                if (b == a || segs[b] < 0) continue;
                const auto it = plan->near_id.find({pl, std::min(segs[a], segs[b]), std::max(segs[a], segs[b])});
                if (it != plan->near_id.end() && plan->near_flag[it->second]) dirty[a] = true;
            }
        }
        std::array<int, 4> key = {pl, -1, -1, -1};
        int nd = 0, pos[3] = {0, 0, 0}, acc = 0;
        for (int a = 0; a < 3; ++a)
            if (segs[a] >= 0 && dirty[a]) { key[1 + nd++] = segs[a]; pos[a] = acc; acc += off[segs[a] + 1] - off[segs[a]]; }
        int g = -1;
        if (nd > 0) {
            auto it = gid[pl].find(key);
            if (it == gid[pl].end()) { g = (int)gkeys[pl].size(); gid[pl][key] = g; gkeys[pl].push_back(key); }
            else g = it->second;
        }
        int dst = h.job_off[sgi];
        for (int a = 0; a < 3; ++a) {
            if (segs[a] < 0) continue;
            const int cnt = off[segs[a] + 1] - off[segs[a]];
            slots.push_back({dst, cnt, pl, segs[a], dirty[a] ? g : -1, pos[a], sgi, 0, 0});
            if (!dirty[a]) pts_cached += cnt;
            dst += cnt;
        }
    }
    const int G0 = (int)gkeys[0].size(), G = G0 + (int)gkeys[1].size();
    plan->G0 = G0;
    plan->groups.resize(G);
    plan->grp_off.assign(G + 1, 0);
    for (int g = 0; g < G; ++g) {
        const std::array<int, 4>& k = g < G0 ? gkeys[0][g] : gkeys[1][g - G0];
        const int* off = h.off[k[0]];
        plan->groups[g].pool = k[0];
        int cnt = 0;
        for (int t = 0; t < 3; ++t) { plan->groups[g].seg[t] = k[1 + t]; if (k[1 + t] >= 0) cnt += off[k[1 + t] + 1] - off[k[1 + t]]; }
        plan->grp_off[g + 1] = plan->grp_off[g] + cnt;
    }
    plan->reuse_stats[0] = pts_cached; plan->reuse_stats[1] = plan->grp_off[G]; plan->reuse_stats[2] = G; plan->reuse_stats[3] = 2 * h.J;
    plan->copies.reserve(slots.size());
    for (SlotPlan& sp : slots) {
        if (sp.grp < 0) { sp.kind = sp.pool; sp.src = h.off[sp.pool][sp.seg]; }
        else { sp.kind = 2; sp.src = plan->grp_off[(sp.pool ? G0 : 0) + sp.grp] + sp.pos; }
        if (sp.count <= 0) continue;
        FeatCopy c;
        c.dst = sp.dst; c.count = sp.count; c.kind = sp.kind; c.src = sp.src;
        if (sp.pool == 1) c.kind |= FEATCOPY_GRAD;
        plan->copies.push_back(c);
    }
}

static int plan_feature_pairs(const HostTables& h, MatchPlan* plan) {
    const int J = h.J;
    const std::vector<SlotPlan>& slots = plan->slots;
    std::vector<FeatPair>& pairs = plan->pairs;
    std::vector<int> side_first(2 * J + 1, 0);
    for (const SlotPlan& sp : slots) ++side_first[sp.side + 1];
    for (int i = 0; i < 2 * J; ++i) side_first[i + 1] += side_first[i];
    std::map<std::array<int, 4>, int> pid;
    plan->sides.assign(2 * J, SidePairs{});
    int64_t pair_pts = 0;
    for (int sgi = 0; sgi < 2 * J; ++sgi) {
        if (sgi == J) { plan->pts0 = pair_pts; plan->n_pairs0 = (int)pairs.size(); }
        const int other = sgi < J ? sgi + J : sgi - J;
        SidePairs& S = plan->sides[sgi];
        for (int a = 0; a < 3; ++a) { S.qcnt[a] = S.dcnt[a] = 0; for (int b = 0; b < 3; ++b) S.pair[a][b] = -1; }
        const int nq = side_first[sgi + 1] - side_first[sgi], nd = side_first[other + 1] - side_first[other];
        for (int a = 0; a < nq; ++a) S.qcnt[a] = slots[side_first[sgi] + a].count;
        for (int b = 0; b < nd; ++b) S.dcnt[b] = slots[side_first[other] + b].count;
        for (int a = 0; a < nq; ++a)
            for (int b = 0; b < nd; ++b) {
                const SlotPlan& q = slots[side_first[sgi] + a];
                const SlotPlan& d = slots[side_first[other] + b];
                if (q.count <= 0 || d.count <= 0) continue;
                const std::array<int, 4> key = {q.kind, q.src, d.kind, d.src};
                auto it = pid.find(key);
                int id;
                if (it == pid.end()) {
                    if (pair_pts + q.count > 0x7fffffff) return ibl_set_error(IBL_ERR_OVERFLOW, "feature matching: pair table exceeds 2^31 entries");
                    id = (int)pairs.size();
                    pid[key] = id;
                    pairs.push_back({q.kind, q.src, q.count, d.kind, d.src, d.count, (int)pair_pts, 0});
                    pair_pts += q.count;
                    plan->max_q = std::max(plan->max_q, q.count);
                } else id = it->second;
                S.pair[a][b] = id;
            }
    }
    plan->pair_pts = pair_pts;
    int64_t uses = 0;
    for (const SidePairs& S : plan->sides)
        for (int a = 0; a < 3; ++a)
            for (int b = 0; b < 3; ++b) uses += S.pair[a][b] >= 0 ? 1 : 0;
    plan->reuse_stats[4] = (int64_t)pairs.size();
    plan->reuse_stats[5] = uses;
    return IBL_OK;
}

static std::vector<float> group_boxes(const HostTables& h, const MatchPlan& plan) {
    std::vector<float> grp_bbox;
    for (const GroupDesc& g : plan.groups)
        if (!h.bbox[g.pool]) return grp_bbox;
    grp_bbox.resize(plan.groups.size() * 6);
    for (size_t g = 0; g < plan.groups.size(); ++g) {
        const GroupDesc& gd = plan.groups[g];
        union_of_boxes(gd.seg, -1, h.off[gd.pool], h.bbox[gd.pool], &grp_bbox[6 * g], &grp_bbox[6 * g + 3]);
    }
    return grp_bbox;
}

struct MatchDev { int* nn; SidePairs* d_sides; FeatPair* d_pairs; int* pair_idx; float* pair_d2; };

static int check_instance_features(const RegCall& c, double grad_radius) {
    const ibl_instance_features* feat[2] = {c.det_features, c.mem_features};
    for (int pl = 0; pl < 2; ++pl) {
        if (!feat[pl]) continue;
        if (!feat[pl]->normals4 || !feat[pl]->fpfh || !feat[pl]->fpfh_norm || !feat[pl]->bbox)
            return ibl_set_error(IBL_ERR_ARG, "ibl_register_batch_cached: instance features with null arrays");
        if (fabs(feat[pl]->voxel_size - c.voxel_size) > 1e-12 * c.voxel_size)
            return ibl_set_error(IBL_ERR_ARG, "ibl_register_batch_cached: instance features were built for voxel_size %g, not %g",
                                 feat[pl]->voxel_size, c.voxel_size);
        if (pl == 1 && (!feat[pl]->grad4 || fabs(feat[pl]->grad_radius - grad_radius) > 1e-12 * grad_radius))
            return ibl_set_error(IBL_ERR_ARG, "ibl_register_batch_cached: memory features need colour gradients of radius %g "
                                 "(2 * voxel_size * local_dist_factor)", grad_radius);
    }
    return IBL_OK;
}

static int test_near_pairs(ibl_reg_ctx* ctx, RegPass& ps, double R) {
    std::vector<NearPair>& near = ps.plan.near;
    if (near.empty()) return IBL_OK;
    hipStream_t s = ps.s;
    ArenaMark mn(ctx);
    NearPair* d_near; int* d_flags;
    IBL_ARENA(d_near, NearPair, (int64_t)near.size());
    IBL_ARENA(d_flags, int, (int64_t)near.size());
    const int st = ibl_stage_upload(ctx, d_near, near.data(), sizeof(NearPair) * (int64_t)near.size(), s);
    if (st) return st;
    IBL_HIP_CHECK(hipMemsetAsync(d_flags, 0, sizeof(int) * near.size(), s));
    const float Rf = nextafterf((float)R, INFINITY);
    for (size_t p0 = 0; p0 < near.size(); p0 += 32768) {
        const unsigned np = (unsigned)std::min<size_t>(32768, near.size() - p0);
        hipLaunchKernelGGL(ibl_near_pair_kernel, dim3(NEAR_SPLIT, np), dim3(256), 0, s, d_near + p0, ps.det, ps.call->det_off_dev, ps.mem,
                           ps.call->mem_off_dev, Rf * Rf * 1.000001f, d_flags + p0);
        IBL_LAUNCH_CHECK();
    }
    IBL_HIP_CHECK(hipMemcpyAsync(ps.plan.near_flag.data(), d_flags, sizeof(int) * near.size(), hipMemcpyDeviceToHost, s));
    IBL_HIP_CHECK(hipStreamSynchronize(s));
    return IBL_OK;
}

static int recompute_groups(ibl_reg_ctx* ctx, RegPass& ps, const HostTables& h, double grad_radius, FeatSources* src) {
    const MatchPlan& plan = ps.plan;
    const RegCall& c = *ps.call;
    hipStream_t s = ps.s;
    const int G = (int)plan.groups.size(), Nd = plan.grp_off[G];
    GroupDesc* d_groups; int* d_grp_off; float4 *Pd, *normals_d, *grad_d; float *fpfh_d, *norm_d; unsigned short* split_d;
    IBL_ARENA(d_groups, GroupDesc, G);
    IBL_ARENA(d_grp_off, int, G + 1);
    IBL_ARENA(Pd, float4, Nd + 1);
    IBL_ARENA(normals_d, float4, Nd + 1);
    IBL_ARENA(grad_d, float4, Nd + 1);
    IBL_ARENA(fpfh_d, float, (int64_t)Nd * 33 + 64);
    IBL_ARENA(split_d, unsigned short, (int64_t)Nd * 48 + 64);
    IBL_ARENA(norm_d, float, (int64_t)Nd + 64);
    int st = ibl_stage_upload(ctx, d_groups, plan.groups.data(), sizeof(GroupDesc) * (int64_t)G, s);
    if (st) return st;
    st = ibl_stage_upload(ctx, d_grp_off, plan.grp_off.data(), sizeof(int) * (int64_t)(G + 1), s);
    if (st) return st;
    hipLaunchKernelGGL(ibl_group_gather_kernel, dim3((Nd + 255) / 256), dim3(256), 0, s, d_groups, G, ps.det, c.det_off_dev, ps.mem,
                       c.mem_off_dev, d_grp_off, Pd);
    IBL_LAUNCH_CHECK();
    const std::vector<float> grp_bbox = group_boxes(h, plan);
    st = ibl_features_on_batch(ctx, Pd, d_grp_off, plan.grp_off.data(), G, grp_bbox.empty() ? nullptr : grp_bbox.data(), c.voxel_size, grad_radius,
                               plan.grp_off[plan.G0], Nd, normals_d, fpfh_d, split_d, norm_d, grad_d, s);
    if (st) return st;
    src->normals[2] = normals_d; src->fpfh[2] = fpfh_d; src->grad[2] = grad_d; src->split[2] = split_d; src->norm[2] = norm_d;
    return IBL_OK;
}

static int assemble_features(ibl_reg_ctx* ctx, RegPass& ps, const FeatSources& src) {
    const std::vector<FeatCopy>& copies = ps.plan.copies;
    FeatCopy* d_copies;
    IBL_ARENA(d_copies, FeatCopy, (int64_t)copies.size());
    const int st = ibl_stage_upload(ctx, d_copies, copies.data(), sizeof(FeatCopy) * (int64_t)copies.size(), ps.s);
    if (st) return st;
    for (size_t c0 = 0; c0 < copies.size(); c0 += 32768) {
        const unsigned nc = (unsigned)std::min<size_t>(32768, copies.size() - c0);
        hipLaunchKernelGGL(ibl_feat_assemble_kernel, dim3(8, nc), dim3(256), 0, ps.s, d_copies + c0, src, ps.normals, (float*)nullptr, ps.grad);
        IBL_LAUNCH_CHECK();
    }
    return IBL_OK;
}

static int search_needed_targets(ibl_reg_ctx* ctx, RegPass& ps, const FeatSources& src, const MatchDev& d, bool use_mfma) {
    const MatchPlan& plan = ps.plan;
    hipStream_t s = ps.s;
    const int J = ps.J, Ns = ps.Ns, n_pairs0 = plan.n_pairs0, max_q = plan.max_q;
    const int64_t pts0 = plan.pts0;
    const int n1 = (int)(plan.pair_pts - pts0);
    const int n_pairs1 = (int)plan.pairs.size() - n_pairs0;
    if (!(n1 > 0 && n_pairs1 > 0 && Ns > 0)) return IBL_OK;
    int *need, *need_pos, *need_list;
    IBL_ARENA(need, int, (int64_t)n1 + 1);
    IBL_ARENA(need_pos, int, (int64_t)n1 + 1);
    IBL_ARENA(need_list, int, (int64_t)n1 + 1);
    IBL_HIP_CHECK(hipMemsetAsync(need, 0, sizeof(int) * ((size_t)n1 + 1), s));
    IBL_HIP_CHECK(hipMemsetD32Async((hipDeviceptr_t)(d.pair_d2 + pts0), 0x7f800000, (size_t)n1, s));
    IBL_HIP_CHECK(hipMemsetAsync(d.pair_idx + pts0, 0, sizeof(int) * (size_t)n1, s));
    hipLaunchKernelGGL(ibl_feat_need_kernel, dim3((Ns + 255) / 256), dim3(256), 0, s, d.d_sides, d.d_pairs, ps.d_job_off, J, d.nn, (int)pts0, need);
    IBL_LAUNCH_CHECK();
    size_t tmp_bytes = 0;
    IBL_HIP_CHECK(hipcub::DeviceScan::ExclusiveSum(nullptr, tmp_bytes, need, need_pos, n1 + 1, s));
    unsigned char* tmp;
    IBL_ARENA(tmp, unsigned char, (int64_t)tmp_bytes + 256);
    IBL_HIP_CHECK(hipcub::DeviceScan::ExclusiveSum(tmp, tmp_bytes, need, need_pos, n1 + 1, s));
    hipLaunchKernelGGL(ibl_feat_need_list_kernel, dim3((n1 + 255) / 256), dim3(256), 0, s, need, need_pos, n1, need_list);
    IBL_LAUNCH_CHECK();
    ps.dbg("need list");
    bool over = !use_mfma;
    if (use_mfma) {
        const int st = ibl_feat_search_mfma(ctx, d.d_pairs + n_pairs0, n_pairs1, max_q, src, d.pair_idx, d.pair_d2, need_pos, need_list, (int)pts0, n1,
                                            &over, s);
        if (st) return st;
    }
    for (int p0 = 0; over && p0 < n_pairs1; p0 += 32768) {
        const unsigned np = (unsigned)std::min(32768, n_pairs1 - p0);
        hipLaunchKernelGGL(ibl_feat_pair_nn_kernel<true>, dim3((max_q + 255) / 256, np), dim3(256), 0, s, d.d_pairs + n_pairs0 + p0, src,
                           d.pair_idx, d.pair_d2, need_pos, need_list, (int)pts0);
        IBL_LAUNCH_CHECK();
    }
    return IBL_OK;
}

static int search_features(ibl_reg_ctx* ctx, RegPass& ps, const FeatSources& src, const MatchDev& d) {
    const MatchPlan& plan = ps.plan;
    hipStream_t s = ps.s;
    const int J = ps.J, N = ps.N, Ns = ps.Ns, n_pairs0 = plan.n_pairs0, max_q = plan.max_q;
    int st = ibl_stage_upload(ctx, d.d_sides, plan.sides.data(), sizeof(SidePairs) * (int64_t)plan.sides.size(), s);
    if (st) return st;
    if (plan.pairs.empty() || N <= 0) {
        if (N > 0) IBL_HIP_CHECK(hipMemsetAsync(d.nn, 0, sizeof(int) * (size_t)N, s));
        return IBL_OK;
    }
    st = ibl_stage_upload(ctx, d.d_pairs, plan.pairs.data(), sizeof(FeatPair) * (int64_t)plan.pairs.size(), s);
    if (st) return st;
    const bool use_mfma = getenv("IBL_FEAT_VALU") == nullptr && !ps.opt.force_valu;
    bool over = !use_mfma;
    ps.dbg("plan uploads");
    if (use_mfma) {
        st = ibl_feat_search_mfma(ctx, d.d_pairs, n_pairs0, max_q, src, d.pair_idx, d.pair_d2, nullptr, nullptr, 0, plan.pts0, &over, s);
        if (st) return st;
    }
    ps.dbg("forward search");
    for (int p0 = 0; over && p0 < n_pairs0; p0 += 32768) {
        const unsigned np = (unsigned)std::min(32768, n_pairs0 - p0);
        hipLaunchKernelGGL(ibl_feat_pair_nn_kernel<false>, dim3((max_q + 255) / 256, np), dim3(256), 0, s, d.d_pairs + p0, src, d.pair_idx,
                           d.pair_d2, (const int*)nullptr, (const int*)nullptr, 0);
        IBL_LAUNCH_CHECK();
    }
    if (Ns > 0) {
        hipLaunchKernelGGL(ibl_feat_fold_kernel, dim3((Ns + 255) / 256), dim3(256), 0, s, d.d_sides, d.d_pairs, d.pair_idx, d.pair_d2, ps.d_job_off,
                           J, 0, Ns, d.nn);
        IBL_LAUNCH_CHECK();
    }
    ps.dbg("forward fold");
    st = search_needed_targets(ctx, ps, src, d, use_mfma);
    if (st) return st;
    ps.dbg("reverse search");
    if (N > Ns) {
        hipLaunchKernelGGL(ibl_feat_fold_kernel, dim3((N - Ns + 255) / 256), dim3(256), 0, s, d.d_sides, d.d_pairs, d.pair_idx, d.pair_d2, ps.d_job_off,
                           J, Ns, N, d.nn);
        IBL_LAUNCH_CHECK();
    }
    ps.dbg("reverse fold");
    return IBL_OK;
}

static int features_and_search(ibl_reg_ctx* ctx, RegPass& ps, const HostTables& h, double grad_radius, const MatchDev& d) {
    const RegCall& c = *ps.call;
    ArenaMark md(ctx);
    FeatSources src{};
    const ibl_instance_features* feat[2] = {c.det_features, c.mem_features};
    for (int pl = 0; pl < 2; ++pl)
        if (feat[pl]) {
            src.normals[pl] = reinterpret_cast<const float4*>(feat[pl]->normals4);
            src.fpfh[pl] = feat[pl]->fpfh;
            src.split[pl] = feat[pl]->fpfh_split;
            src.norm[pl] = feat[pl]->fpfh_norm;
            src.grad[pl] = reinterpret_cast<const float4*>(feat[pl]->grad4);
        }
    int st;
    if (ps.plan.grp_off.back() > 0) {
        st = recompute_groups(ctx, ps, h, grad_radius, &src);
        if (st) return st;
    }
    if (!ps.plan.copies.empty()) {
        st = assemble_features(ctx, ps, src);
        if (st) return st;
    }
    ps.phase("recomputed groups + assemble");
    double fl = 0;
    for (int j = 0; j < ps.J; ++j)
        fl += 4.0 * 33.0 * (double)(ps.job_off[j + 1] - ps.job_off[j]) * (double)(ps.job_off[ps.J + j + 1] - ps.job_off[ps.J + j]);
    ibl_prof_begin(IBL_PROF_ST_FEATMATCH, fl, ps.s, &ps.tok_match);
    return search_features(ctx, ps, src, d);
}

int ibl_reg_match_stage(ibl_reg_ctx* ctx, RegPass& ps) {
    const RegCall& c = *ps.call;
    MatchPlan& plan = ps.plan;
    ArenaMark m2(ctx);
    MatchDev d = {};
    IBL_ARENA(d.nn, int, ps.N + 64);
    const double grad_radius = ps.max_dist_icp * 2.0;
    int st = check_instance_features(c, grad_radius);
    if (st) return st;
    const HostTables h = {ps.J, ps.jobs.data(), ps.job_off.data(), {c.det_off_host, c.mem_off_host},
                          {c.det_features ? c.det_features->bbox : nullptr, c.mem_features ? c.mem_features->bbox : nullptr}};
    const double rn = c.voxel_size * 2, rf = c.voxel_size * 5;
    const double R = std::max(2 * rf + rn, grad_radius + rn) * 1.001 + 1e-4;
    list_near_candidates(h, R, &plan);
    st = test_near_pairs(ctx, ps, R);
    if (st) return st;
    ps.phase("near-pair test");
    plan_feature_reuse(h, &plan);
    if (c.reuse_stats_out) for (int i = 0; i < 4; ++i) c.reuse_stats_out[i] = plan.reuse_stats[i];
    st = plan_feature_pairs(h, &plan);
    if (st) return st;
    if (c.reuse_stats_out) for (int i = 4; i < 6; ++i) c.reuse_stats_out[i] = plan.reuse_stats[i];
    ps.phase("host plan");
    IBL_ARENA(d.d_sides, SidePairs, 2 * ps.J);
    IBL_ARENA(d.d_pairs, FeatPair, (int64_t)plan.pairs.size() + 1);
    IBL_ARENA(d.pair_idx, int, plan.pair_pts + 64);
    IBL_ARENA(d.pair_d2, float, plan.pair_pts + 64);
    st = features_and_search(ctx, ps, h, grad_radius, d);
    if (st) return st;
    ibl_prof_end(ps.tok_match, ps.s);
    ps.phase("feature search");
    hipLaunchKernelGGL(ibl_mutual_kernel, dim3(ps.J), dim3(256), 0, ps.s, d.nn, ps.d_job_off, ps.J, 1, 9, ps.corr, ps.n_corr);
    IBL_LAUNCH_CHECK();
    return IBL_OK;
}
```

### instance-based-loc_amd/csrc/reg_stages.h

```cpp
#pragma once
#include <algorithm>
#include <array>
#include <map>
#include <vector>

#include "ibloc.h"
#include "reg_common.h"

#define ICP_BPJ 8

struct RegCall {
    const float* det_pts4; const int32_t* det_off_dev; const int32_t* det_off_host; int n_det_seg;
    const float* mem_pts4; const int32_t* mem_off_dev; const int32_t* mem_off_host; int n_mem_seg;
    const int32_t* job_src_seg; const int32_t* job_tgt_seg;
    const uint32_t* job_ids;
    int n_jobs;
    double voxel_size, global_dist_factor, local_dist_factor;
    uint64_t seed; uint32_t job_id_base; int64_t ransac_max_iter; int flags;
    const ibl_instance_features* det_features; const ibl_instance_features* mem_features;
    double *T_out, *rmse_out, *fitness_out, *means_out, *T_ransac_out;
    int64_t *ransac_stats_out, *reuse_stats_out;
    hipStream_t stream;
};
struct RegPassOpts {
    bool force_valu = false;
    bool ransac_full_list = false;
};

struct JobDesc {
    int src_seg[3];
    int tgt_seg[3];
};
struct GroupDesc { int pool; int seg[3]; };
struct FeatCopy { int dst, src, count, kind; };
struct NearPair { int pool, a, b, pad; float boxa[6], boxb[6]; };
struct SidePairs { int qcnt[3]; int dcnt[3]; int pair[3][3]; };

struct RansacState {
    double best_T[16];
    double best_fit, best_rmse;
    long long est_k, next_i, walked, validated, last_update;
    int best_inl;
    int done;
    unsigned job_id;
    int pad_;
};
struct IcpState {
    double T[16];
    double fitness, rmse;
    int iter, done, started;
};

struct HostTables { int J; const JobDesc* jobs; const int* job_off; const int* off[2]; const float* bbox[2]; };
struct SlotPlan { int dst, count, pool, seg, grp, pos, side, kind, src; };
struct MatchPlan {
    std::vector<NearPair> near;
    std::map<std::array<int, 3>, int> near_id;
    std::vector<int> near_flag;
    std::vector<SlotPlan> slots;
    std::vector<GroupDesc> groups;
    std::vector<int> grp_off;
    int G0 = 0;
    std::vector<FeatCopy> copies;
    std::vector<FeatPair> pairs;
    std::vector<SidePairs> sides;
    int64_t pair_pts = 0, pts0 = 0;
    int n_pairs0 = 0, max_q = 1;
    int64_t reuse_stats[6] = {0, 0, 0, 0, 0, 0};
};

static inline void union_of_boxes(const int* segs, int only, const int* off, const float* boxes, float* lo, float* hi) {
    bool any = false;
    for (int c = 0; c < 3; ++c) lo[c] = hi[c] = 0.0f;
    for (int t = 0; t < 3; ++t) {
        if (only >= 0 && t != only) continue;
        if (segs[t] < 0 || off[segs[t] + 1] == off[segs[t]]) continue;
        const float* b = boxes + 6 * (size_t)segs[t];
        for (int c = 0; c < 3; ++c) { lo[c] = any ? std::min(lo[c], b[c]) : b[c]; hi[c] = any ? std::max(hi[c], b[3 + c]) : b[3 + c]; }
        any = true;
    }
}

struct RegPass {
    const RegCall* call;
    RegPassOpts opt;
    hipStream_t s;
    int J, N, Ns;
    bool colored;
    double max_dist_icp;
    std::vector<JobDesc> jobs;
    std::vector<int> job_off;
    MatchPlan plan;
    const float4 *det, *mem;
    JobDesc* d_jobs; int* d_job_off; int* d_piece_off; double* d_means;
    float4 *P, *normals, *grad;
    BatchGrid gC;
    int2* corr; int* n_corr;
    RansacState* rs;
    IcpState* is;
    void *tok_match, *tok_ransac, *tok_icp;
    bool timing;
    double t_prev;
    void phase(const char* what);
    void dbg(const char* what) const;
};

int ibl_reg_match_stage(ibl_reg_ctx* ctx, RegPass& ps);
int ibl_reg_ransac_stage(ibl_reg_ctx* ctx, RegPass& ps);
int ibl_reg_icp_stage(ibl_reg_ctx* ctx, RegPass& ps);
```

### instance-based-loc_amd/engine.py

```python
import os
import warnings
from collections import deque
from concurrent.futures import ThreadPoolExecutor
from dataclasses import dataclass, field

import numpy as np
import torch
from scipy.spatial.transform import Rotation

from . import match
from .assign import K_HI, K_LO, assign_batch, assign_candidates
from .parallel import ShardExchange, shard_range, sharded_candidates
from .registration import (CloudBatch, InstanceFeatures, MemGrid, RegContext, evaluate_batch, evaluate_points,
                           instance_features_batch, radius_outlier_batch, register_batch, register_evaluate_batch)

IBL_ST_GRID_OVERFLOW = 1


def intensity_from_colors(colors) -> np.ndarray:
    c = np.asarray(colors, dtype=np.float64)
    return ((c[:, 0] + c[:, 1] + c[:, 2]) / 3.0).astype(np.float32)


class MemoryShard:

    def __init__(self, ctx: RegContext, embeddings, clouds=None, colors=None, intensities=None, eval_threshold=0.02, device="cuda",
                 shard=None, shard_clouds=False, compact_features=False):
        self.ctx = ctx
        self.compact_features = bool(compact_features)
        self.device = torch.device(device)
        self.M = len(embeddings)
        self.shard = shard
        self.lo, self.hi = shard_range(self.M, *shard) if shard is not None else (0, self.M)
        own = embeddings[self.lo:self.hi]
        counts = [len(e) for e in own]
        self.emb_offsets_host = np.concatenate([[0], np.cumsum(counts)]).astype(np.int32)
        dim = np.asarray(embeddings[0]).shape[-1] if self.M else 0
        raw = np.concatenate([np.asarray(e, dtype=np.float32) for e in own]) if len(own) else np.zeros((0, dim), np.float32)
        if len(raw):
            self.mem_emb = match.normalize_rows(torch.from_numpy(np.ascontiguousarray(raw)).to(self.device))
        else:
            self.mem_emb = torch.zeros((0, dim), dtype=torch.float32, device=self.device)
        self.emb_offsets = torch.from_numpy(self.emb_offsets_host).to(self.device)
        self.eval_threshold = eval_threshold
        self._features = {}
        self.clouds = self.grid = None
        self.shard_clouds = bool(shard_clouds and shard is not None and clouds is not None)
        self.inst_sizes_all = None
        if self.shard_clouds:
            def own_part(x):
                return x if x is None or len(x) == self.hi - self.lo else x[self.lo:self.hi]
            if clouds is not None and len(clouds) == self.M:
                self.inst_sizes_all = np.array([len(c) for c in clouds], dtype=np.int64)
            clouds, colors, intensities = own_part(clouds), own_part(colors), own_part(intensities)
        if clouds is not None:
            if intensities is None:
                intensities = [intensity_from_colors(c) for c in colors] if colors is not None else None
            self.clouds = CloudBatch.from_numpy(clouds, intensities, device=device)
            self.grid = MemGrid(ctx, self.clouds.pts4, cell=2 * eval_threshold)

    def features(self, voxel_size, local_dist_factor):
        key = (float(voxel_size), float(local_dist_factor))
        if key not in self._features:
            self._features[key] = instance_features_batch(self.ctx, self.clouds, voxel_size, 2.0 * (voxel_size * local_dist_factor),
                                                          compact=self.compact_features)
        return self._features[key]

    def close(self):
        if self.grid is not None:
            self.grid.close()
            self.grid = None
        self._features = {}


@dataclass
class FrameResult:
    pose: np.ndarray
    pose_corrected: np.ndarray
    assignments: list = field(default_factory=list)
    records: list = field(default_factory=list)
    best: int = -1
    n_clean: int = 0


@dataclass
class _Lane:
    ctx: RegContext
    lane: int
    stream: "torch.cuda.Stream"


class LocaliseEngine:
    def __init__(self, memory: MemoryShard, encoder=None, assign_threads=0, k_hi=K_HI, k_lo=K_LO, group=None, rows_cap=224, comm=None):
        self.memory = memory
        self.encoder = encoder
        self.ctx = memory.ctx
        self.assign_threads = assign_threads or min(os.cpu_count() or 1, 16)
        self.k_hi, self.k_lo = int(k_hi), int(k_lo)
        self.reuse_features = True
        self.use_candidates = True
        self.fused_stage_b = True
        self._pool_a = None
        self._pool_w = None
        self._lanes = []
        self.exchange = ShardExchange(group, rows_cap, comm) if memory.shard is not None and (memory.shard[1] > 1 or comm is not None) else None
        self.stats = {"frames": 0, "fallback_frames": 0}
        self.route = None
        if memory.shard_clouds:
            from .routing import Transport
            self.route = Transport(group)
            if memory.inst_sizes_all is None:
                parts = self.route.all_gather_object(np.diff(memory.clouds.seg_off_host).astype(np.int64))
                memory.inst_sizes_all = np.concatenate(parts)
            assert len(memory.inst_sizes_all) == memory.M
            self.route_stats = {}

    def close(self):
        for lane in self._lanes:
            lane.ctx.close()
        self._lanes = []
        for p in (self._pool_a, self._pool_w):
            if p is not None:
                p.shutdown(wait=True)
        self._pool_a = self._pool_w = None

    def check_status(self):
        st = self.ctx.status()
        if st & IBL_ST_GRID_OVERFLOW:
            warnings.warn("registration scratch grid overflowed its cell budget: a neighbourhood search fell back to the slow path "
                          "(results unaffected); clouds this large want a larger arena or a coarser fpfh_voxel_size")
        return st

    def match_assign(self, q_per_frame, crops=None, det_emb=None, num_per_length=4, lane=0, tick=lambda name: None):
        mem = self.memory
        q_per_frame = np.asarray(q_per_frame, dtype=np.int32)
        F = len(q_per_frame)
        ex = self.exchange
        q_emb = np.minimum(q_per_frame, mem.M).astype(np.int32)
        err = None
        if (q_per_frame > 7).any():
            err = ValueError("more than 7 detections in a frame: select the 7 largest first (object_memory.py:900-908)")
        elif (q_emb < np.minimum(q_per_frame, 3)).any():
            err = AssertionError("fewer memory objects than the sub-volume dimension (reference asserts at similarity_volume.py:112)")
        elif det_emb is None and self.encoder is None:
            err = ValueError("no encoder: pass det_emb")
        elif ex is not None and int(q_per_frame.sum()) > ex.cap:
            err = ValueError(f"{int(q_per_frame.sum())} query rows in a step, rows_cap is {ex.cap}")
        if ex is not None:
# ... 104 lines not shown
                yield pending.popleft().result()
        while pending:
            yield pending.popleft().result()

    def localise_stream(self, batches, **kw):
        depth = max(1, int(kw.pop("lookahead", os.environ.get("IBL_STAGE_A_LOOKAHEAD", "2"))))
        if self.route is not None:
            for b in batches:
                args = {k: b[k] for k in ("det", "q_per_frame", "crops", "det_emb", "seed", "job_id_base") if k in b}
                yield self.localise_batch(**args, **kw)
            return
        dev = self.memory.mem_emb.device
        side = torch.cuda.Stream(device=dev)
        main = torch.cuda.current_stream(dev)
        npl = kw.get("num_per_length", 4)

        def stage_a(b, ready):
            torch.cuda.set_device(dev)
            with torch.cuda.stream(side):
                side.wait_event(ready)
                return self.match_assign(b["q_per_frame"], b.get("crops"), b.get("det_emb"), npl)

        def submit(b):
            ready = torch.cuda.Event()
            ready.record(main)
            return self._pool_a.submit(stage_a, b, ready)

        def stage_done():
            torch.cuda.set_device(dev)
            with torch.cuda.stream(side):
                _, _, any_active = self.exchange.agree(False, True, dev)
            if any_active:
                raise RuntimeError("sharded memory: the ranks were given different numbers of batches")

        fut_done = None
        it = iter(batches)
        pending = deque()
        exhausted = False
        if self._pool_a is None:
            self._pool_a = ThreadPoolExecutor(max_workers=1)

        def fill():
            nonlocal exhausted, fut_done
            while not exhausted and len(pending) < depth:
                b = next(it, None)
                if b is None:
                    exhausted = True
                    if self.exchange is not None:
                        fut_done = self._pool_a.submit(stage_done)
                else:
                    pending.append((b, submit(b)))

        try:
            fill()
            while pending:
                cur, fut = pending[0]
                assns = fut.result()
                pending.popleft()
                fill()
                args = dict(kw)
                for k in ("seed", "job_id_base"):
                    if k in cur:
                        args[k] = cur[k]
                yield self.localise_batch(cur["det"], cur["q_per_frame"], assns=assns, **args)
            if fut_done is not None:
                fut_done.result()
        finally:
            for _, f in pending:
                try:
                    f.result()
                except Exception:
                    pass
            side.synchronize()

    def _register_routed(self, ctx, clean, det_feat, mem_feat, job_src, job_tgt, job_id_base, voxel, gdf, ldf, seed, ransac_max_iter):
        from .routing import InstanceStore, routed_register
        mem = self.memory
        assert det_feat is not None and mem_feat is not None, "sharded clouds need reuse_features (the cached instance features travel)"
        arrays = {"pts": mem.clouds.pts4, "normals": mem_feat.normals, "fpfh": mem_feat.fpfh, "fpfh_norm": mem_feat.fpfh_norm}
        if mem_feat.fpfh_split is not None:
            arrays["fpfh_split"] = mem_feat.fpfh_split
        if mem_feat.grad is not None:
            arrays["grad"] = mem_feat.grad
        store = InstanceStore(mem.lo, mem.clouds.seg_off_host, arrays, {"bbox": mem_feat.bbox})

        def compute(pool_pts, pool_off, n_home, arr, per_inst, mem_off, js, jt, ids):
            det_pool = CloudBatch(pool_pts.contiguous(), pool_off.astype(np.int32))
            feat = det_feat
            if det_pool.n_seg > n_home:
                b0 = int(pool_off[n_home])
                extra = instance_features_batch(ctx, CloudBatch(pool_pts[b0:].contiguous(), (pool_off[n_home:] - b0).astype(np.int32)), voxel)
                feat = InstanceFeatures(torch.cat([det_feat.normals[:clean.n], extra.normals]), torch.cat([det_feat.fpfh[:clean.n], extra.fpfh]),
                                        torch.cat([det_feat.fpfh_split[:clean.n], extra.fpfh_split]),
                                        torch.cat([det_feat.fpfh_norm[:clean.n], extra.fpfh_norm]), None,
                                        np.concatenate([det_feat.bbox[:clean.n_seg], extra.bbox]), voxel, 0.0)
            mem_pool = CloudBatch(arr["pts"].contiguous(), np.asarray(mem_off).astype(np.int32))
            mf = InstanceFeatures(arr["normals"].contiguous(), arr["fpfh"].contiguous(), arr["fpfh_split"].contiguous() if "fpfh_split" in arr else None,
                                  arr["fpfh_norm"].contiguous(), arr["grad"].contiguous() if "grad" in arr else None,
                                  np.ascontiguousarray(per_inst["bbox"]), mem_feat.voxel_size, mem_feat.grad_radius)
            r = register_batch(ctx, det_pool, mem_pool, js, jt, voxel, gdf, ldf, seed=seed, ransac_max_iter=ransac_max_iter,
                               have_colors=True, center=True, det_features=feat, mem_features=mf, job_ids=ids)
            return {k: r[k] for k in ("T", "rmse", "fitness", "means", "T_ransac", "ransac_stats")}

        J = len(job_src)
        ids = (np.uint32(job_id_base) + np.arange(J, dtype=np.uint32)).astype(np.uint32)
        src = np.asarray(job_src, dtype=np.int64).reshape(-1, 3)
        tgt = np.asarray(job_tgt, dtype=np.int64).reshape(-1, 3)
        params = (int(seed), float(voxel), float(gdf), float(ldf), int(ransac_max_iter))
        reg, _ = routed_register(self.route, mem.M, clean.pts4, clean.seg_off_host, src, tgt, ids, store, mem.inst_sizes_all, compute,
                                 self.route_stats, params=params)
        return reg

    def _evaluate_routed(self, ctx, clean, jb, je, G, thr):
        from .routing import routed_evaluate
        mem = self.memory
        thr = thr if thr is not None else mem.eval_threshold

        def local(pts, b, e, T):
            return evaluate_points(ctx, mem.grid, pts.contiguous(), b, e, T, thr)[0]

        return routed_evaluate(self.route, clean.pts4, jb, je, G, local)

    def localise_batch(self, det: CloudBatch, q_per_frame, crops=None, det_emb=None, fpfh_voxel_size=0.05,
                       fpfh_global_dist_factor=2, fpfh_local_dist_factor=0.4, outlier_radius=0.05, outlier_nb_points=8,
                       seed=0, job_id_base=0, ransac_max_iter=4000000, num_per_length=4, eval_threshold=None, timings=None,
                       assns=None, _slot=None, register=True, ransac_fixed_budget=False):
        mem = self.memory
        ctx, lane = (self.ctx, 0) if _slot is None else (_slot.ctx, _slot.lane)
        q_per_frame = np.asarray(q_per_frame, dtype=np.int32)
        F = len(q_per_frame)
        row0 = np.concatenate([[0], np.cumsum(q_per_frame)]).astype(np.int64)
        register = register and mem.clouds is not None
        assert not register or det.n_seg == int(row0[-1])
        ev = []

        def tick(name):
            if timings is not None:
                e = torch.cuda.Event(enable_timing=True)
                e.record()
                ev.append((name, e))

        def close_timings():
            if timings is not None:
                torch.cuda.synchronize()
                for (n0, e0), (n1, e1) in zip(ev[:-1], ev[1:]):
                    timings[n1] = timings.get(n1, 0.0) + e0.elapsed_time(e1)

        tick("start")
        if assns is None:
            assns = self.match_assign(q_per_frame, crops, det_emb, num_per_length, lane, tick)
        results = [FrameResult(np.array([0., 0., 0., 0., 0., 0., 1.]), np.array([0., 0., 0., 0., 0., 0., 1.])) for _ in range(F)]
        if not register:
            for f in range(F):
                results[f].assignments = assns[f]
                results[f].best = 0 if assns[f] else -1
            close_timings()
            return results
        if self.fused_stage_b and self.route is None and self.reuse_features:
            if not any(len(a) for a in assns):
                close_timings()
                return results
            thr = eval_threshold if eval_threshold is not None else mem.eval_threshold
            r = register_evaluate_batch(ctx, det, q_per_frame, assns, mem.clouds, mem.features(fpfh_voxel_size, fpfh_local_dist_factor), mem.grid,
                                        fpfh_voxel_size, fpfh_global_dist_factor, fpfh_local_dist_factor, outlier_radius, outlier_nb_points, thr,
                                        seed=seed, job_id_base=job_id_base, ransac_max_iter=ransac_max_iter, fixed_budget=ransac_fixed_budget)
            if timings is not None:
                timings["reuse"] = r["reuse"].tolist()
            tick("stage_b")
            self._assemble(results, assns, row0, r["clean_off"], r, r["T_global"], r["full_rmse"], r["full_fitness"])
            tick("select")
            close_timings()
            return results
        keep = radius_outlier_batch(ctx, det, outlier_radius, outlier_nb_points)
        keepb = keep.bool()
        csum = torch.cumsum(keep.to(torch.int32), 0)
        csum0 = torch.cat([torch.zeros(1, dtype=torch.int32, device=csum.device), csum])
        new_off = csum0[det.seg_off.long()]
        clean_pts = det.pts4[keepb].contiguous()
        new_off_h = new_off.cpu().numpy().astype(np.int32)
        clean = CloudBatch(clean_pts, new_off_h)
        tick("outlier")
        job_frame, job_src, job_tgt = [], [], []
        for f in range(F):
            for a in assns[f]:
                job_frame.append(f)
                job_src.append([int(row0[f]) + d for d, m in a] + [-1] * (3 - len(a)))
                job_tgt.append([m for d, m in a] + [-1] * (3 - len(a)))
        if not job_frame and self.route is None:
            close_timings()
            return results
        det_feat = mem_feat = None
        if self.reuse_features:
            det_feat = instance_features_batch(ctx, clean, fpfh_voxel_size)
            mem_feat = mem.features(fpfh_voxel_size, fpfh_local_dist_factor)
        tick("det_features")
        if self.route is not None:
            reg = self._register_routed(ctx, clean, det_feat, mem_feat, job_src, job_tgt, job_id_base, fpfh_voxel_size,
                                        fpfh_global_dist_factor, fpfh_local_dist_factor, seed, ransac_max_iter)
            if not job_frame:
                self._evaluate_routed(ctx, clean, [], [], np.zeros((0, 4, 4)), eval_threshold)
                close_timings()
                return results
        else:
            reg = register_batch(ctx, clean, mem.clouds, job_src, job_tgt, fpfh_voxel_size, fpfh_global_dist_factor,
                                 fpfh_local_dist_factor, seed=seed, job_id_base=job_id_base, ransac_max_iter=ransac_max_iter,
                                 have_colors=True, center=True, det_features=det_feat, mem_features=mem_feat, fixed_budget=ransac_fixed_budget)
            if timings is not None:
                timings["reuse"] = reg["reuse"].tolist()
        tick("register")
        T = reg["T"]
        means = reg["means"]
        G = T.copy()
        Rm = T[:, :3, :3]
        dm = means[:, 0]
        G[:, :3, 3] = T[:, :3, 3] + means[:, 1] - ((Rm[:, :, 0] * dm[:, 0:1] + Rm[:, :, 1] * dm[:, 1:2]) + Rm[:, :, 2] * dm[:, 2:3])
        jb = [int(new_off_h[row0[f]]) for f in job_frame]
        je = [int(new_off_h[row0[f + 1]]) for f in job_frame]
        thr = eval_threshold if eval_threshold is not None else mem.eval_threshold
        if self.route is not None:
            full_fit, full_rmse = self._evaluate_routed(ctx, clean, jb, je, G, thr)
        else:
            full_rmse, full_fit = evaluate_batch(ctx, mem.grid, clean.pts4, jb, je, G, thr)
        tick("evaluate")
        self._assemble(results, assns, row0, new_off_h, reg, G, full_rmse, full_fit)
        tick("select")
        close_timings()
        return results

    @staticmethod
    def _assemble(results, assns, row0, new_off_h, reg, G, full_rmse, full_fit):
        T, means = reg["T"], reg["means"]
        j = 0
        picked = []
        for f in range(len(assns)):
            n_a = len(assns[f])
            if n_a == 0:
                continue
            ff = full_fit[j:j + n_a]
            best = max(range(n_a), key=lambda k: (ff[k], -k))
            picked.append((f, j, best))
            j += n_a
        if picked:
            quats = Rotation.from_matrix(np.stack([T[j0 + b, :3, :3] for _, j0, b in picked])).as_quat()
        for (f, j0, best), q in zip(picked, quats if picked else []):
            n_a = len(assns[f])
            recs = [dict(assn=assns[f][k], T=T[j0 + k], rmse=reg["rmse"][j0 + k], fitness=reg["fitness"][j0 + k],
                         full_rmse=full_rmse[j0 + k], full_fitness=full_fit[j0 + k], T_global=G[j0 + k],
                         detected_mean=means[j0 + k, 0], memory_mean=means[j0 + k, 1], ransac_stats=reg["ransac_stats"][j0 + k])
                    for k in range(n_a)]
            R = T[j0 + best, :3, :3]
            t = T[j0 + best, :3, 3]
            last = j0 + n_a - 1
            t_ref = t + means[last, 1] - R @ means[last, 0]
            t_fix = t + means[j0 + best, 1] - R @ means[j0 + best, 0]
            results[f] = FrameResult(np.concatenate((t_ref, q)), np.concatenate((t_fix, q)), assns[f], recs, best,
                                     int(new_off_h[row0[f + 1]] - new_off_h[row0[f]]))
        return results
```

### instance-based-loc_amd/registration.py

```python
import ctypes as C

import numpy as np
import torch

from . import _lib


def _stream():
    return torch.cuda.current_stream().cuda_stream


class RegContext:

    def __init__(self, arena_bytes=4 << 30):
        self._h = C.c_void_p()
        _lib.check(_lib.lib.ibl_reg_ctx_create(C.byref(self._h), int(arena_bytes)), "ibl_reg_ctx_create")

    def close(self):
        if self._h:
            _lib.lib.ibl_reg_ctx_destroy(self._h)
            self._h = C.c_void_p()

    def __del__(self):
        try:
# ... 25 lines not shown
        self.seg_off = torch.from_numpy(self.seg_off_host).to(pts4.device)

    @property
    def n_seg(self):
        return len(self.seg_off_host) - 1

    @property
    def n(self):
        return int(self.seg_off_host[-1])

    @staticmethod
    def from_numpy(clouds, intensities=None, device="cuda"):
        sizes = [len(c) for c in clouds]
        off = np.concatenate([[0], np.cumsum(sizes)]).astype(np.int32)
        p4 = np.zeros((int(off[-1]), 4), dtype=np.float32)
        for i, c in enumerate(clouds):
            p4[off[i]:off[i + 1], :3] = np.asarray(c, dtype=np.float32)
            if intensities is not None:
                p4[off[i]:off[i + 1], 3] = np.asarray(intensities[i], dtype=np.float32)
        return CloudBatch(torch.from_numpy(p4).to(device), off)


def unproject_masks(ctx: RegContext, depth: torch.Tensor, rgb: torch.Tensor, masks: torch.Tensor, fx: float, fy: float,
                    depth_factor: float = 1.0, want_f64: bool = False):
    dev = depth.device
    assert depth.is_cuda and rgb.is_cuda and masks.is_cuda and depth.dim() == 2
    H, W = depth.shape
    if depth.dtype in (torch.uint16, torch.int16):
        is_u16, d = 1, depth.contiguous()
    elif depth.dtype == torch.float32:
        is_u16, d = 0, depth.contiguous()
    else:
        is_u16, d = 2, depth.to(torch.float64).contiguous()
    rgb = rgb.to(torch.uint8).contiguous()
    m = masks.reshape(-1, H, W).to(torch.uint8).contiguous()
    n = m.shape[0]
    assert rgb.shape == (H, W, 3)
    cap = int(m.count_nonzero().item()) if n else 0
    pts4 = torch.empty((max(cap, 1), 4), dtype=torch.float32, device=dev)
    off_dev = torch.zeros(n + 1, dtype=torch.int32, device=dev)
    off_host = np.zeros(n + 1, dtype=np.int32)
    p64 = torch.empty((max(cap, 1), 3), dtype=torch.float64, device=dev) if want_f64 else None
    c64 = torch.empty((max(cap, 1), 3), dtype=torch.float64, device=dev) if want_f64 else None
    st = _lib.lib.ibl_unproject_masks_f64(ctx.handle, d.data_ptr(), is_u16, rgb.data_ptr(), m.data_ptr(), n, H, W, float(fx), float(fy),
                                          float(depth_factor), pts4.data_ptr(), p64.data_ptr() if want_f64 else None,
                                          c64.data_ptr() if want_f64 else None, cap, off_dev.data_ptr(), off_host.ctypes.data, _stream())
    _lib.check(st, "ibl_unproject_masks_f64")
    batch = CloudBatch(pts4[:int(off_host[-1])].contiguous() if off_host[-1] != cap or cap == 0 else pts4, off_host)
    if want_f64:
        return batch, p64[:int(off_host[-1])], c64[:int(off_host[-1])]
    return batch


def radius_outlier_batch(ctx: RegContext, batch: CloudBatch, radius: float, nb_points: int) -> torch.Tensor:
    keep = torch.empty(max(batch.n, 1), dtype=torch.uint8, device=batch.pts4.device)
    st = _lib.lib.ibl_radius_outlier_batch(ctx.handle, batch.pts4.data_ptr(), batch.seg_off.data_ptr(),
                                           batch.seg_off_host.ctypes.data, batch.n_seg, float(radius), int(nb_points),
                                           keep.data_ptr(), _stream())
    _lib.check(st, "ibl_radius_outlier_batch")
    return keep[:batch.n]


def normals_fpfh_batch(ctx: RegContext, batch: CloudBatch, radius_normal, max_nn_normal=30, radius_feature=None,
                       max_nn_feature=100):
    dev = batch.pts4.device
    normals = torch.empty((max(batch.n, 1), 4), dtype=torch.float32, device=dev)
    fpfh = torch.empty((max(batch.n, 1), 33), dtype=torch.float32, device=dev) if radius_feature else None
    st = _lib.lib.ibl_normals_fpfh_batch(ctx.handle, batch.pts4.data_ptr(), batch.seg_off.data_ptr(),
                                         batch.seg_off_host.ctypes.data, batch.n_seg, float(radius_normal), int(max_nn_normal),
                                         float(radius_feature or 0.0), int(max_nn_feature), normals.data_ptr(),
                                         fpfh.data_ptr() if fpfh is not None else None, _stream())
    _lib.check(st, "ibl_normals_fpfh_batch")
    return normals[:batch.n], (fpfh[:batch.n] if fpfh is not None else None)


FEAT_ORDER = np.array([b * 11 + c for c in (5, 4, 6, 3, 7, 2, 8, 1, 9, 0, 10) for b in (1, 2, 0)], dtype=np.int64)
FEAT_MU = np.array([87, 46, 101, 26, 28, 17, 26, 26, 17, 14, 21, 7, 14, 19, 7, 8, 14, 6, 8, 13, 6, 5, 11, 6, 5, 10, 6, 3, 7, 14, 3, 6, 14],
                   dtype=np.float32)


class _FeatStruct(C.Structure):
    _fields_ = [("normals4", C.c_void_p), ("fpfh", C.c_void_p), ("fpfh_split", C.c_void_p), ("fpfh_norm", C.c_void_p),
                ("grad4", C.c_void_p), ("bbox", C.c_void_p),
                ("voxel_size", C.c_double), ("grad_radius", C.c_double)]


class InstanceFeatures:

    def __init__(self, normals, fpfh, fpfh_split, fpfh_norm, grad, bbox, voxel_size, grad_radius):
        self.normals, self.fpfh, self.grad, self.bbox = normals, fpfh, grad, bbox
        self.fpfh_split, self.fpfh_norm = fpfh_split, fpfh_norm
        self.voxel_size, self.grad_radius = float(voxel_size), float(grad_radius)

    def as_struct(self):
        return _FeatStruct(self.normals.data_ptr(), self.fpfh.data_ptr(), self.fpfh_split.data_ptr() if self.fpfh_split is not None else None,
                           self.fpfh_norm.data_ptr(),
                           self.grad.data_ptr() if self.grad is not None else None,
                           self.bbox.ctypes.data, self.voxel_size, self.grad_radius)


def instance_features_batch(ctx: RegContext, batch: CloudBatch, voxel_size: float, grad_radius: float = 0.0,
                            compact: bool = False) -> InstanceFeatures:
    dev = batch.pts4.device
    n = max(batch.n, 1)
    normals = torch.empty((n, 4), dtype=torch.float32, device=dev)
    fpfh = torch.empty((n, 33), dtype=torch.float32, device=dev)
    fpfh_split = None if compact else torch.empty((n, 48), dtype=torch.float16, device=dev)
    fpfh_norm = torch.empty((n,), dtype=torch.float32, device=dev)
    grad = torch.empty((n, 4), dtype=torch.float32, device=dev) if grad_radius > 0 else None
    bbox = np.zeros((max(batch.n_seg, 1), 6), dtype=np.float32)
    st = _lib.lib.ibl_instance_features_batch(ctx.handle, batch.pts4.data_ptr(), batch.seg_off.data_ptr(), batch.seg_off_host.ctypes.data,
                                              batch.n_seg, float(voxel_size), float(grad_radius), normals.data_ptr(), fpfh.data_ptr(),
                                              fpfh_split.data_ptr() if fpfh_split is not None else None, fpfh_norm.data_ptr(),
                                              grad.data_ptr() if grad is not None else None, bbox.ctypes.data, _stream())
    _lib.check(st, "ibl_instance_features_batch")
    return InstanceFeatures(normals, fpfh, fpfh_split, fpfh_norm, grad, bbox, voxel_size, grad_radius)


REG_HAVE_COLORS = 1
REG_CENTER = 2
REG_FIXED_BUDGET = 4


def register_batch(ctx: RegContext, det: CloudBatch, mem: CloudBatch, job_src_seg, job_tgt_seg, voxel_size,
                   global_dist_factor=1.5, local_dist_factor=0.4, seed=0, job_id_base=0, ransac_max_iter=4000000,
                   have_colors=True, center=True, det_features: InstanceFeatures = None, mem_features: InstanceFeatures = None,
                   job_ids=None, fixed_budget=False):
    def pad(a):
        a = np.asarray(a, dtype=np.int32)
        if a.ndim == 1:
            a = a[:, None]
        out = np.full((a.shape[0], 3), -1, dtype=np.int32)
        out[:, :a.shape[1]] = a
        return np.ascontiguousarray(out)

    js, jt = pad(job_src_seg), pad(job_tgt_seg)
    J = js.shape[0]
    assert jt.shape[0] == J
    T = np.zeros((J, 16), dtype=np.float64)
    rmse = np.zeros(J, dtype=np.float64)
    fit = np.zeros(J, dtype=np.float64)
    means = np.zeros((J, 2, 3), dtype=np.float64)
    Tr = np.zeros((J, 16), dtype=np.float64)
    stats = np.zeros((J, 3), dtype=np.int64)
    flags = (REG_HAVE_COLORS if have_colors else 0) | (REG_CENTER if center else 0) | (REG_FIXED_BUDGET if fixed_budget else 0)
    reuse = np.zeros(6, dtype=np.int64)
    df = det_features.as_struct() if det_features is not None else None
    mf = mem_features.as_struct() if mem_features is not None else None
    if job_ids is not None:
        ids = np.ascontiguousarray(job_ids, dtype=np.uint32)
        assert ids.shape == (J,)
        st = _lib.lib.ibl_register_batch_ids(ctx.handle, det.pts4.data_ptr(), det.seg_off.data_ptr(), det.seg_off_host.ctypes.data,
                                             det.n_seg, mem.pts4.data_ptr(), mem.seg_off.data_ptr(), mem.seg_off_host.ctypes.data,
                                             mem.n_seg, js.ctypes.data, jt.ctypes.data, ids.ctypes.data, J, float(voxel_size),
                                             float(global_dist_factor), float(local_dist_factor), int(seed), int(ransac_max_iter), flags,
                                             C.byref(df) if df is not None else None, C.byref(mf) if mf is not None else None,
                                             T.ctypes.data, rmse.ctypes.data, fit.ctypes.data, means.ctypes.data, Tr.ctypes.data,
                                             stats.ctypes.data, reuse.ctypes.data, _stream())
        _lib.check(st, "ibl_register_batch_ids")
        return dict(T=T.reshape(J, 4, 4), rmse=rmse, fitness=fit, means=means, T_ransac=Tr.reshape(J, 4, 4), ransac_stats=stats,
                    reuse=reuse)
    st = _lib.lib.ibl_register_batch_cached(ctx.handle, det.pts4.data_ptr(), det.seg_off.data_ptr(), det.seg_off_host.ctypes.data,
                                            det.n_seg, mem.pts4.data_ptr(), mem.seg_off.data_ptr(), mem.seg_off_host.ctypes.data,
                                            mem.n_seg, js.ctypes.data, jt.ctypes.data, J, float(voxel_size), float(global_dist_factor),
                                            float(local_dist_factor), int(seed), int(job_id_base), int(ransac_max_iter), flags,
                                            C.byref(df) if df is not None else None, C.byref(mf) if mf is not None else None,
                                            T.ctypes.data, rmse.ctypes.data, fit.ctypes.data, means.ctypes.data, Tr.ctypes.data,
                                            stats.ctypes.data, reuse.ctypes.data, _stream())
    _lib.check(st, "ibl_register_batch_cached")
    return dict(T=T.reshape(J, 4, 4), rmse=rmse, fitness=fit, means=means, T_ransac=Tr.reshape(J, 4, 4), ransac_stats=stats,
                reuse=reuse)


def register_evaluate_batch(ctx: RegContext, det: CloudBatch, q_per_frame, assns, mem: CloudBatch, mem_features: InstanceFeatures, grid,
                            voxel_size, global_dist_factor, local_dist_factor, outlier_radius=0.05, outlier_nb_points=8, eval_threshold=0.02,
                            seed=0, job_id_base=0, ransac_max_iter=4000000, have_colors=True, center=True, fixed_budget=False):
    q = np.ascontiguousarray(q_per_frame, dtype=np.int32)
    F = len(q)
    max_assn = max(6, max((len(a) for a in assns), default=0))
    assn = np.full((F, max_assn, 6), -1, dtype=np.int32)
    alen = np.zeros((F, max_assn), dtype=np.int32)
    acnt = np.zeros(F, dtype=np.int32)
    for f, lst in enumerate(assns):
        acnt[f] = len(lst)
        for a, pairs in enumerate(lst):
            alen[f, a] = len(pairs)
            for t, (d, m) in enumerate(pairs):
                assn[f, a, 2 * t], assn[f, a, 2 * t + 1] = d, m
    J = int(acnt.sum())
    Jc = max(J, 1)
    clean_off = np.zeros(det.n_seg + 1, dtype=np.int32)
    n_jobs = C.c_int32(0)
    T = np.zeros((Jc, 16)); rmse = np.zeros(Jc); fit = np.zeros(Jc); means = np.zeros((Jc, 2, 3)); Tr = np.zeros((Jc, 16))
    stats = np.zeros((Jc, 3), dtype=np.int64); reuse = np.zeros(6, dtype=np.int64)
    G = np.zeros((Jc, 16)); frmse = np.zeros(Jc); ffit = np.zeros(Jc); best = np.full(max(F, 1), -1, dtype=np.int32)
    flags = (REG_HAVE_COLORS if have_colors else 0) | (REG_CENTER if center else 0) | (REG_FIXED_BUDGET if fixed_budget else 0)
    mf = mem_features.as_struct()
    st = _lib.lib.ibl_register_evaluate_batch(
        ctx.handle, det.pts4.data_ptr(), det.seg_off.data_ptr(), det.seg_off_host.ctypes.data, det.n_seg, q.ctypes.data, F, assn.ctypes.data,
# ... 64 lines not shown
```

Before: 833.6 query-frames/s.

## Record per-point FPFH neighbour reach to tighten correspondence search bounds

The FPFH kernel now records, for each point, the squared distance of its farthest kept neighbour, or the full search radius when the neighbour list was not truncated. A new kernel reduces this to a per-instance maximum, which is copied to the host. Both values are carried in the instance-feature struct and the registration host tables, likely so matching can use a tighter candidate radius or floor and skip work. This adds a warp reduction and atomics to the FPFH kernel, an extra per-point buffer, and a host sync/copy.

```diff
diff --git a/include/ibloc.h b/include/ibloc.h
--- a/include/ibloc.h
+++ b/include/ibloc.h
@@ -198,10 +198,12 @@
     const float* bbox;
     double voxel_size;
     double grad_radius;
+    const float* reach2;
+    const float* seg_reach2;
 } ibl_instance_features;
 int ibl_instance_features_batch(ibl_reg_ctx* ctx, const float* pts4, const int32_t* seg_off_dev, const int32_t* seg_off_host,
                                 int n_seg, double voxel_size, double grad_radius, float* normals4, float* fpfh, uint16_t* fpfh_split,
-                                float* fpfh_norm, float* grad4, float* bbox_host, void* stream);
+                                float* fpfh_norm, float* grad4, float* bbox_host, float* reach2, float* seg_reach2_host, void* stream);
 int ibl_register_batch_cached(ibl_reg_ctx* ctx, const float* det_pts4, const int32_t* det_off_dev, const int32_t* det_off_host,
                               int n_det_seg, const float* mem_pts4, const int32_t* mem_off_dev, const int32_t* mem_off_host,
                               int n_mem_seg, const int32_t* job_src_seg, const int32_t* job_tgt_seg, int n_jobs, double voxel_size,
diff --git a/instance-based-loc_amd/_lib.py b/instance-based-loc_amd/_lib.py
--- a/instance-based-loc_amd/_lib.py
+++ b/instance-based-loc_amd/_lib.py
@@ -56,7 +56,7 @@
     "ibl_normals_fpfh_batch": (C.c_int, [vp, vp, vp, vp, C.c_int, C.c_double, C.c_int, C.c_double, C.c_int, vp, vp, vp]),
     "ibl_register_batch": (C.c_int, [vp, vp, vp, vp, C.c_int, vp, vp, vp, C.c_int, vp, vp, C.c_int, C.c_double, C.c_double,
                                      C.c_double, C.c_uint64, C.c_uint32, C.c_int64, C.c_int, vp, vp, vp, vp, vp, vp, vp]),
-    "ibl_instance_features_batch": (C.c_int, [vp, vp, vp, vp, C.c_int, C.c_double, C.c_double, vp, vp, vp, vp, vp, vp, vp]),
+    "ibl_instance_features_batch": (C.c_int, [vp, vp, vp, vp, C.c_int, C.c_double, C.c_double, vp, vp, vp, vp, vp, vp, vp, vp, vp]),
     "ibl_register_batch_cached": (C.c_int, [vp, vp, vp, vp, C.c_int, vp, vp, vp, C.c_int, vp, vp, C.c_int, C.c_double, C.c_double,
                                             C.c_double, C.c_uint64, C.c_uint32, C.c_int64, C.c_int, vp, vp, vp, vp, vp, vp, vp, vp,
                                             vp, vp]),
diff --git a/instance-based-loc_amd/csrc/localise.hip b/instance-based-loc_amd/csrc/localise.hip
--- a/instance-based-loc_amd/csrc/localise.hip
+++ b/instance-based-loc_amd/csrc/localise.hip
@@ -109,16 +109,17 @@
     if (J == 0) return IBL_OK;
     const int nc = clean_off_host[n_det_seg];
 
-    float4* nrm; float* fpfh; uint16_t* split; float* fnorm;
+    float4* nrm; float* fpfh; uint16_t* split; float* fnorm; float* reach2;
     IBL_ARENA(nrm, float4, (int64_t)nc + 1);
     IBL_ARENA(fpfh, float, (int64_t)nc * 33 + 64);
     IBL_ARENA(split, uint16_t, (int64_t)nc * 48 + 64);
     IBL_ARENA(fnorm, float, (int64_t)nc + 64);
-    std::vector<float> bbox((size_t)n_det_seg * 6 + 6, 0.0f);
+    IBL_ARENA(reach2, float, (int64_t)nc + 64);
+    std::vector<float> bbox((size_t)n_det_seg * 6 + 6, 0.0f), seg_reach2((size_t)n_det_seg + 1, 0.0f);
     int st = ibl_instance_features_batch(ctx, reinterpret_cast<const float*>(clean), new_off, clean_off_host, n_det_seg, voxel_size, 0.0,
-                                         reinterpret_cast<float*>(nrm), fpfh, split, fnorm, nullptr, bbox.data(), stream);
+                                         reinterpret_cast<float*>(nrm), fpfh, split, fnorm, nullptr, bbox.data(), reach2, seg_reach2.data(), stream);
     if (st) return st;
-    ibl_instance_features det_feat{reinterpret_cast<const float*>(nrm), fpfh, split, fnorm, nullptr, bbox.data(), voxel_size, 0.0};
+    ibl_instance_features det_feat{reinterpret_cast<const float*>(nrm), fpfh, split, fnorm, nullptr, bbox.data(), voxel_size, 0.0, reach2, seg_reach2.data()};
 
     st = ibl_register_batch_cached(ctx, reinterpret_cast<const float*>(clean), new_off, clean_off_host, n_det_seg, mem_pts4, mem_off_dev,
                                    mem_off_host, n_mem_seg, job_src.data(), job_tgt.data(), J, voxel_size, global_dist_factor, local_dist_factor,
diff --git a/instance-based-loc_amd/csrc/reg_api.hip b/instance-based-loc_amd/csrc/reg_api.hip
--- a/instance-based-loc_amd/csrc/reg_api.hip
+++ b/instance-based-loc_amd/csrc/reg_api.hip
@@ -25,7 +25,7 @@
 int ibl_launch_normals(ibl_reg_ctx* ctx, const BatchGrid& g, const float4* pts, const int* seg_off, int n, double radius, int max_nn, float4* normals,
                        int* status, hipStream_t s);
 int ibl_launch_fpfh(ibl_reg_ctx* ctx, const BatchGrid& g, const float4* pts, const float4* normals, const int* seg_off, int n, double radius, int max_nn,
-                    unsigned char* spfh, int* nbr_idx, float* nbr_d2, int* nbr_cnt, float* fpfh, int matching_order, int* status,
+                    unsigned char* spfh, int* nbr_idx, float* nbr_d2, int* nbr_cnt, float* fpfh, int matching_order, float* reach2, int* status,
                     hipStream_t s);
 int ibl_launch_radius_count(const BatchGrid& g, const float4* pts, const int* seg_off, int n, double radius, int nb_points,
                             unsigned char* keep, hipStream_t s);
@@ -33,7 +33,7 @@
 bool ibl_normals_fpfh_fusable(double radius_normal, int max_nn_normal, double radius_feature, int max_nn_feature);
 int ibl_launch_normals_fpfh(ibl_reg_ctx* ctx, const BatchGrid& g, const float4* pts, const int* seg_off, int n, double radius_normal,
                             int max_nn_normal, double radius_feature, int max_nn_feature, float4* normals, unsigned char* spfh, int* nbr_idx,
-                            float* nbr_d2, int* nbr_cnt, float* fpfh, int matching_order, int* status, hipStream_t s);
+                            float* nbr_d2, int* nbr_cnt, float* fpfh, int matching_order, float* reach2, int* status, hipStream_t s);
 int ibl_launch_color_grad(ibl_reg_ctx* ctx, const BatchGrid& g, const float4* pts, const float4* normals, const int* seg_off, int q0, int q1, double radius,
                           int max_nn, float4* grad, int* status, hipStream_t s);
 
@@ -156,10 +156,10 @@
         IBL_ARENA(nbr_cnt, int, n + 64);
         if (fused)
             st = ibl_launch_normals_fpfh(ctx, g, P, seg_off_dev, n, radius_normal, max_nn_normal, radius_feature, max_nn_feature,
-                                         reinterpret_cast<float4*>(normals4), spfh, nbr_idx, nbr_d2, nbr_cnt, fpfh, 0, ctx->d_status, s);
+                                         reinterpret_cast<float4*>(normals4), spfh, nbr_idx, nbr_d2, nbr_cnt, fpfh, 0, nullptr, ctx->d_status, s);
         else
             st = ibl_launch_fpfh(ctx, g, P, reinterpret_cast<const float4*>(normals4), seg_off_dev, n, radius_feature, max_nn_feature, spfh,
-                                 nbr_idx, nbr_d2, nbr_cnt, fpfh, 0, ctx->d_status, s);
+                                 nbr_idx, nbr_d2, nbr_cnt, fpfh, 0, nullptr, ctx->d_status, s);
         if (st) return st;
     }
     IBL_HIP_CHECK(hipStreamSynchronize(s));
@@ -190,7 +190,7 @@
 
 int ibl_features_on_batch(ibl_reg_ctx* ctx, const float4* P, const int* seg_off_dev, const int* seg_off_host, int n_seg, const float* bbox_host,
                           double voxel_size, double grad_radius, int gq0, int gq1, float4* normals, float* fpfh, unsigned short* fpfh_split,
-                          float* fpfh_norm, float4* grad, hipStream_t s) {
+                          float* fpfh_norm, float4* grad, float* reach2, hipStream_t s) {
     const int n = seg_off_host[n_seg];
     if (n <= 0) return IBL_OK;
     int st;
@@ -221,8 +221,8 @@
         IBL_ARENA(nbr_d2, float, (int64_t)n * 100 + 64);
         IBL_ARENA(nbr_cnt, int, n + 64);
         if (fused) st = ibl_launch_normals_fpfh(ctx, gB, P, seg_off_dev, n, voxel_size * 2, 30, voxel_size * 5, 100, normals, spfh, nbr_idx, nbr_d2, nbr_cnt,
-                                                fpfh, 1, ctx->d_status, s);
-        else st = ibl_launch_fpfh(ctx, gB, P, normals, seg_off_dev, n, voxel_size * 5, 100, spfh, nbr_idx, nbr_d2, nbr_cnt, fpfh, 1, ctx->d_status, s);
+                                                fpfh, 1, reach2, ctx->d_status, s);
+        else st = ibl_launch_fpfh(ctx, gB, P, normals, seg_off_dev, n, voxel_size * 5, 100, spfh, nbr_idx, nbr_d2, nbr_cnt, fpfh, 1, reach2, ctx->d_status, s);
         if (st) return st;
         if (fpfh_norm) {
             hipLaunchKernelGGL(ibl_fpfh_half_kernel, dim3((unsigned)((n + 255) / 256)), dim3(256), 0, s, fpfh, n, fpfh_split, fpfh_norm);
@@ -241,11 +241,26 @@
     return IBL_OK;
 }
 
+__global__ __launch_bounds__(256) void ibl_seg_reach_kernel(const float* __restrict__ reach2, const int* __restrict__ seg_off, float* __restrict__ seg_reach2) {
+    const int b = seg_off[blockIdx.x], e = seg_off[blockIdx.x + 1];
+    __shared__ float part[4];
+    float m = 0.0f;
+    for (int i = b + threadIdx.x; i < e; i += 256) m = fmaxf(m, reach2[i]);
+#pragma unroll
+    for (int off = 32; off >= 1; off >>= 1) m = fmaxf(m, __shfl_xor(m, off, 64));
+    if ((threadIdx.x & 63) == 0) part[threadIdx.x >> 6] = m;
+    __syncthreads();
+    if (threadIdx.x == 0) seg_reach2[blockIdx.x] = fmaxf(fmaxf(part[0], part[1]), fmaxf(part[2], part[3]));
+}
+
 extern "C" int ibl_instance_features_batch(ibl_reg_ctx* ctx, const float* pts4, const int32_t* seg_off_dev, const int32_t* seg_off_host,
                                            int n_seg, double voxel_size, double grad_radius, float* normals4, float* fpfh,
-                                           uint16_t* fpfh_split, float* fpfh_norm, float* grad4, float* bbox_host, void* stream) {
+                                           uint16_t* fpfh_split, float* fpfh_norm, float* grad4, float* bbox_host, float* reach2,
+                                           float* seg_reach2_host, void* stream) {
     if (!ctx || !pts4 || !seg_off_dev || !normals4 || !fpfh || !fpfh_norm || voxel_size <= 0)
         return ibl_set_error(IBL_ERR_ARG, "ibl_instance_features_batch: bad argument");
+    if ((reach2 == nullptr) != (seg_reach2_host == nullptr))
+        return ibl_set_error(IBL_ERR_ARG, "ibl_instance_features_batch: reach2 and seg_reach2_host go together");
     if (grad4 && grad_radius <= 0) return ibl_set_error(IBL_ERR_ARG, "ibl_instance_features_batch: colour gradients need grad_radius > 0");
     int st = check_seg(seg_off_host, n_seg, "ibl_instance_features_batch");
     if (st) return st;
@@ -285,13 +300,20 @@
         const int cnt = off_host[ns];
         st = ibl_features_on_batch(ctx, P + o0, off_dev, off_host, ns, bbox_host + 6 * (size_t)s0, voxel_size, grad_radius, 0, grad4 ? cnt : 0,
                                    reinterpret_cast<float4*>(normals4) + o0, fpfh + (int64_t)o0 * 33, fpfh_split ? fpfh_split + (int64_t)o0 * 48 : nullptr,
-                                   fpfh_norm + o0, grad4 ? reinterpret_cast<float4*>(grad4) + o0 : nullptr, s);
+                                   fpfh_norm + o0, grad4 ? reinterpret_cast<float4*>(grad4) + o0 : nullptr, reach2 ? reach2 + o0 : nullptr, s);
         if (st) return st;
         s0 = s1;
         if (ctx->pin_used > ctx->pin_size / 2) {
             IBL_HIP_CHECK(hipStreamSynchronize(s));
             ibl_stage_reset(ctx);
         }
+    }
+    if (reach2 && n_seg > 0) {
+        float* d_seg;
+        IBL_ARENA(d_seg, float, n_seg);
+        hipLaunchKernelGGL(ibl_seg_reach_kernel, dim3((unsigned)n_seg), dim3(256), 0, s, reach2, seg_off_dev, d_seg);
+        IBL_LAUNCH_CHECK();
+        IBL_HIP_CHECK(hipMemcpyAsync(seg_reach2_host, d_seg, sizeof(float) * (size_t)n_seg, hipMemcpyDeviceToHost, s));
     }
     ibl_prof_end(tok, s);
     IBL_HIP_CHECK(hipStreamSynchronize(s));
diff --git a/instance-based-loc_amd/csrc/reg_common.h b/instance-based-loc_amd/csrc/reg_common.h
--- a/instance-based-loc_amd/csrc/reg_common.h
+++ b/instance-based-loc_amd/csrc/reg_common.h
@@ -99,7 +99,7 @@
 
 int ibl_features_on_batch(ibl_reg_ctx* ctx, const float4* P, const int* seg_off_dev, const int* seg_off_host, int n_seg, const float* bbox_host, double voxel_size,
                           double grad_radius, int gq0, int gq1, float4* normals, float* fpfh, unsigned short* fpfh_split, float* fpfh_norm,
-                          float4* grad, hipStream_t s);
+                          float4* grad, float* reach2, hipStream_t s);
 
 #ifdef __HIPCC__
 __device__ __constant__ const float FM_MU[33] = {87.f, 46.f, 101.f, 26.f, 28.f, 17.f, 26.f, 26.f, 17.f, 14.f, 21.f, 7.f, 14.f, 19.f, 7.f, 8.f, 14.f,
diff --git a/instance-based-loc_amd/csrc/reg_knn.hip b/instance-based-loc_amd/csrc/reg_knn.hip
--- a/instance-based-loc_amd/csrc/reg_knn.hip
+++ b/instance-based-loc_amd/csrc/reg_knn.hip
@@ -1563,13 +1563,14 @@
 #define FPFH_Q 7
 __global__ __launch_bounds__(256) void ibl_fpfh_kernel(const unsigned char* __restrict__ spfh_cnt, const int* __restrict__ nbr_idx,
                                                        const float* __restrict__ nbr_d2, const int* __restrict__ nbr_cnt, int K, int n,
-                                                       int matching_order, float* __restrict__ fpfh) {
+                                                       int matching_order, float* __restrict__ fpfh, float r2, float* __restrict__ reach2) {
     __shared__ FpfhTile tiles[FPFH_Q];
     __shared__ double accs[FPFH_Q][33];
     __shared__ int kq[FPFH_Q];
+    __shared__ unsigned far_bits[FPFH_Q];
     const int tid = threadIdx.x;
     const int q0 = IBL_XCD_BLOCK(blockIdx.x, gridDim.x) * FPFH_Q;
-    if (tid < FPFH_Q) kq[tid] = q0 + tid < n ? nbr_cnt[q0 + tid] : 0;
+    if (tid < FPFH_Q) { kq[tid] = q0 + tid < n ? nbr_cnt[q0 + tid] : 0; far_bits[tid] = 0u; }
     __syncthreads();
     int kmax = 0;
 #pragma unroll
@@ -1582,10 +1583,13 @@
     for (int t0 = 0; t0 < kmax; t0 += 64) {
         for (int e = tid; e < FPFH_Q * 64; e += 256) {
             const int sq = e >> 6, r = e & 63, t = t0 + r, si = q0 + sq;
+            unsigned far = 0u;
             if (si < n && t < kq[sq]) {
                 FpfhTile& S = tiles[sq];
                 const int j = nbr_idx[(int64_t)si * K + t];
-                const double dist = (double)nbr_d2[(int64_t)si * K + t];
+                const float d2f = nbr_d2[(int64_t)si * K + t];
+                far = __float_as_uint(d2f);
+                const double dist = (double)d2f;
                 const int kj = nbr_cnt[j];
                 const unsigned char* src = spfh_cnt + (int64_t)j * 36;
                 const ibl_u4_a4 r0 = *reinterpret_cast<const ibl_u4_a4*>(src), r1 = *reinterpret_cast<const ibl_u4_a4*>(src + 16);
@@ -1593,6 +1597,11 @@
                 unsigned int* dst = reinterpret_cast<unsigned int*>(S.cnt[r]);
                 dst[0] = r0.x; dst[1] = r0.y; dst[2] = r0.z; dst[3] = r0.w; dst[4] = r1.x; dst[5] = r1.y; dst[6] = r1.z; dst[7] = r1.w; dst[8] = r2w;
                 S.w[r] = (j == si || dist == 0.0 || kj <= 1) ? 0.0 : (100.0 / (double)(kj - 1)) / dist;
+            }
+            if (reach2) {
+#pragma unroll
+                for (int off = 32; off >= 1; off >>= 1) far = max(far, (unsigned)__shfl_xor((int)far, off, 64));
+                if (r == 0 && far != 0u) atomicMax(&far_bits[sq], far);
             }
         }
         __syncthreads();
@@ -1616,6 +1625,7 @@
             out = (float)(acc * sc + (double)spfh_value(spfh_cnt, nbr_cnt, qi, b));
         }
         fpfh[(int64_t)qi * 33 + (matching_order ? FEAT_POS[b] : b)] = out;
+        if (reach2 && b == 0) reach2[qi] = k >= K ? __uint_as_float(far_bits[qq]) : r2;
     }
 }
 
@@ -1727,7 +1737,7 @@
 }
 
 int ibl_launch_fpfh(ibl_reg_ctx* ctx, const BatchGrid& g, const float4* pts, const float4* normals, const int* seg_off, int n, double radius, int max_nn,
-                    unsigned char* spfh, int* nbr_idx, float* nbr_d2, int* nbr_cnt, float* fpfh, int matching_order, int* status,
+                    unsigned char* spfh, int* nbr_idx, float* nbr_d2, int* nbr_cnt, float* fpfh, int matching_order, float* reach2, int* status,
                     hipStream_t s) {
     if (n <= 0) return IBL_OK;
     if (max_nn > 256) return ibl_set_error(IBL_ERR_UNSUPPORTED, "fpfh: max_nn %d > 256 (SPFH histograms are stored as bytes)", max_nn);
@@ -1736,7 +1746,8 @@
     const int st = launch_knn(ctx, g, pts, seg_off, n, 0, n, radius, max_nn, SpfhFactory{normals, spfh, nbr_idx, nbr_d2, nbr_cnt, max_nn}, status, s);
     ibl_prof_end(tok, s);
     if (st) return st;
-    hipLaunchKernelGGL(ibl_fpfh_kernel, dim3((n + FPFH_Q - 1) / FPFH_Q), dim3(256), 0, s, spfh, nbr_idx, nbr_d2, nbr_cnt, max_nn, n, matching_order, fpfh);
+    hipLaunchKernelGGL(ibl_fpfh_kernel, dim3((n + FPFH_Q - 1) / FPFH_Q), dim3(256), 0, s, spfh, nbr_idx, nbr_d2, nbr_cnt, max_nn, n, matching_order, fpfh,
+                       (float)(radius * radius), reach2);
     IBL_LAUNCH_CHECK();
     return IBL_OK;
 }
@@ -1867,7 +1878,7 @@
 }
 int ibl_launch_normals_fpfh(ibl_reg_ctx* ctx, const BatchGrid& g, const float4* pts, const int* seg_off, int n, double radius_normal,
                             int max_nn_normal, double radius_feature, int max_nn_feature, float4* normals, unsigned char* spfh, int* nbr_idx,
-                            float* nbr_d2, int* nbr_cnt, float* fpfh, int matching_order, int* status, hipStream_t s) {
+                            float* nbr_d2, int* nbr_cnt, float* fpfh, int matching_order, float* reach2, int* status, hipStream_t s) {
     if (n <= 0) return IBL_OK;
     ArenaMark mk(ctx);
     unsigned* nrm_mask;
@@ -1915,7 +1926,8 @@
         }
     }
     if (fpfh) {
-        hipLaunchKernelGGL(ibl_fpfh_kernel, dim3((n + FPFH_Q - 1) / FPFH_Q), dim3(256), 0, s, spfh, nbr_idx, nbr_d2, nbr_cnt, max_nn_feature, n, matching_order, fpfh);
+        hipLaunchKernelGGL(ibl_fpfh_kernel, dim3((n + FPFH_Q - 1) / FPFH_Q), dim3(256), 0, s, spfh, nbr_idx, nbr_d2, nbr_cnt, max_nn_feature, n, matching_order, fpfh,
+                           (float)(radius_feature * radius_feature), reach2);
         IBL_LAUNCH_CHECK();
     }
     return IBL_OK;
diff --git a/instance-based-loc_amd/csrc/reg_match.hip b/instance-based-loc_amd/csrc/reg_match.hip
--- a/instance-based-loc_amd/csrc/reg_match.hip
+++ b/instance-based-loc_amd/csrc/reg_match.hip
@@ -40,6 +40,7 @@
 
 #define NEAR_SPLIT 8
 #define NEAR_CAP 5120
+#define NEAR_MARGIN 1.00001f
 
 __device__ __forceinline__ float box_dist2(const float* bx, float x, float y, float z) {
     const float dx = fmaxf(fmaxf(bx[0] - x, x - bx[3]), 0.0f), dy = fmaxf(fmaxf(bx[1] - y, y - bx[4]), 0.0f),
@@ -49,18 +50,30 @@
 
 __global__ __launch_bounds__(256) void ibl_near_pair_kernel(const NearPair* __restrict__ pairs, const float4* __restrict__ det,
                                                             const int* __restrict__ det_off, const float4* __restrict__ mem,
-                                                            const int* __restrict__ mem_off, float R2, int* __restrict__ flags) {
+                                                            const int* __restrict__ mem_off, float R2, const float* __restrict__ det_reach2,
+                                                            const float* __restrict__ mem_reach2, float det_floor2, float mem_floor2,
+                                                            int* __restrict__ flags) {
     const NearPair P = pairs[blockIdx.y];
+    const bool by_reach = P.ra2 >= 0.0f;
+    const bool swap = blockIdx.x >= NEAR_SPLIT;
+    if (swap && !by_reach) return;
     const float4* pool = P.pool ? mem : det;
     const int* off = P.pool ? mem_off : det_off;
-    const int ab = off[P.a], ae = off[P.a + 1], bb = off[P.b], be = off[P.b + 1];
+    const float* reach2 = P.pool ? mem_reach2 : det_reach2;
+    const float floor2 = P.pool ? mem_floor2 : det_floor2;
+    const int qs = swap ? P.b : P.a, os = swap ? P.a : P.b;
+    const float* boxq = swap ? P.boxb : P.boxa;
+    const float* boxo = swap ? P.boxa : P.boxb;
+    const float Rq2 = by_reach ? (swap ? P.rb2 : P.ra2) : R2;
+    const int ab = off[qs], ae = off[qs + 1], bb = off[os], be = off[os + 1];
     __shared__ float sx[NEAR_CAP], sy[NEAR_CAP], sz[NEAR_CAP];
     __shared__ int nb, found;
     if (threadIdx.x == 0) { nb = 0; found = 0; }
     __syncthreads();
     for (int i = bb + threadIdx.x; i < be; i += 256) {
         const float4 p = pool[i];
-        if (box_dist2(P.boxa, p.x, p.y, p.z) < R2) {
+        const float bd = box_dist2(boxq, p.x, p.y, p.z);
+        if (by_reach ? bd <= Rq2 : bd < Rq2) {
             const int pos = atomicAdd(&nb, 1);
             if (pos < NEAR_CAP) { sx[pos] = p.x; sy[pos] = p.y; sz[pos] = p.z; }
         }
@@ -69,12 +82,17 @@
     const int n = nb;
     if (n > NEAR_CAP) { if (threadIdx.x == 0) atomicOr(&flags[blockIdx.y], 1); return; }
     if (n == 0) return;
-    for (int i0 = ab + blockIdx.x * 256; i0 < ae; i0 += NEAR_SPLIT * 256) {
+    for (int i0 = ab + (blockIdx.x % NEAR_SPLIT) * 256; i0 < ae; i0 += NEAR_SPLIT * 256) {
         const int i = i0 + threadIdx.x;
         bool hit = false;
         if (i < ae) {
             const float4 p = pool[i];
-            if (box_dist2(P.boxb, p.x, p.y, p.z) < R2)
+            if (by_reach) {
+                const float t = fmaxf(reach2[i], floor2);
+                if (box_dist2(boxo, p.x, p.y, p.z) <= t * NEAR_MARGIN)
+                    for (int j = 0; j < n; ++j)
+                        if (dist2f(p.x, p.y, p.z, sx[j], sy[j], sz[j]) <= t) { hit = true; break; }
+            } else if (box_dist2(boxo, p.x, p.y, p.z) < R2)
                 for (int j = 0; j < n; ++j)
                     if (dist2f(p.x, p.y, p.z, sx[j], sy[j], sz[j]) < R2) { hit = true; break; }
         }
@@ -279,8 +297,14 @@
                 if (segs[a] < 0 || segs[b] < 0) continue;
                 const std::array<int, 3> key = {pl, std::min(segs[a], segs[b]), std::max(segs[a], segs[b])};
                 const float *ba = h.bbox[pl] + 6 * (size_t)key[1], *bb = h.bbox[pl] + 6 * (size_t)key[2];
-                if (plan->near_id.count(key) || box_gap2(ba, bb) >= R * R) continue;
+                if (plan->near_id.count(key)) continue;
                 NearPair np;
+                np.ra2 = np.rb2 = -1.0f;
+                if (h.seg_reach2[pl]) {
+                    np.ra2 = std::max(h.seg_reach2[pl][key[1]], h.floor2[pl]) * NEAR_MARGIN;
+                    np.rb2 = std::max(h.seg_reach2[pl][key[2]], h.floor2[pl]) * NEAR_MARGIN;
+                    if (box_gap2(ba, bb) > (double)std::max(np.ra2, np.rb2)) continue;
+                } else if (box_gap2(ba, bb) >= R * R) continue;
                 np.pool = pl; np.a = key[1]; np.b = key[2]; np.pad = 0;
                 for (int c = 0; c < 6; ++c) { np.boxa[c] = ba[c]; np.boxb[c] = bb[c]; }
                 plan->near_id[key] = (int)plan->near.size();
@@ -431,7 +455,7 @@
     return IBL_OK;
 }
 
-static int test_near_pairs(ibl_reg_ctx* ctx, RegPass& ps, double R) {
+static int test_near_pairs(ibl_reg_ctx* ctx, RegPass& ps, const HostTables& h, double R) {
     std::vector<NearPair>& near = ps.plan.near;
     if (near.empty()) return IBL_OK;
     hipStream_t s = ps.s;
@@ -443,10 +467,14 @@
     if (st) return st;
     IBL_HIP_CHECK(hipMemsetAsync(d_flags, 0, sizeof(int) * near.size(), s));
     const float Rf = nextafterf((float)R, INFINITY);
+    bool any_reach = false;
+    for (const NearPair& p : near) any_reach = any_reach || p.ra2 >= 0.0f;
+    const RegCall& c = *ps.call;
     for (size_t p0 = 0; p0 < near.size(); p0 += 32768) {
         const unsigned np = (unsigned)std::min<size_t>(32768, near.size() - p0);
-        hipLaunchKernelGGL(ibl_near_pair_kernel, dim3(NEAR_SPLIT, np), dim3(256), 0, s, d_near + p0, ps.det, ps.call->det_off_dev, ps.mem,
-                           ps.call->mem_off_dev, Rf * Rf * 1.000001f, d_flags + p0);
+        hipLaunchKernelGGL(ibl_near_pair_kernel, dim3(any_reach ? 2 * NEAR_SPLIT : NEAR_SPLIT, np), dim3(256), 0, s, d_near + p0, ps.det,
+                           c.det_off_dev, ps.mem, c.mem_off_dev, Rf * Rf * 1.000001f, c.det_features ? c.det_features->reach2 : nullptr,
+                           c.mem_features ? c.mem_features->reach2 : nullptr, h.floor2[0], h.floor2[1], d_flags + p0);
         IBL_LAUNCH_CHECK();
     }
     IBL_HIP_CHECK(hipMemcpyAsync(ps.plan.near_flag.data(), d_flags, sizeof(int) * near.size(), hipMemcpyDeviceToHost, s));
@@ -477,7 +505,7 @@
     IBL_LAUNCH_CHECK();
     const std::vector<float> grp_bbox = group_boxes(h, plan);
     st = ibl_features_on_batch(ctx, Pd, d_grp_off, plan.grp_off.data(), G, grp_bbox.empty() ? nullptr : grp_bbox.data(), c.voxel_size, grad_radius,
-                               plan.grp_off[plan.G0], Nd, normals_d, fpfh_d, split_d, norm_d, grad_d, s);
+                               plan.grp_off[plan.G0], Nd, normals_d, fpfh_d, split_d, norm_d, grad_d, nullptr, s);
     if (st) return st;
     src->normals[2] = normals_d; src->fpfh[2] = fpfh_d; src->grad[2] = grad_d; src->split[2] = split_d; src->norm[2] = norm_d;
     return IBL_OK;
@@ -620,12 +648,20 @@
     const double grad_radius = ps.max_dist_icp * 2.0;
     int st = check_instance_features(c, grad_radius);
     if (st) return st;
-    const HostTables h = {ps.J, ps.jobs.data(), ps.job_off.data(), {c.det_off_host, c.mem_off_host},
-                          {c.det_features ? c.det_features->bbox : nullptr, c.mem_features ? c.mem_features->bbox : nullptr}};
     const double rn = c.voxel_size * 2, rf = c.voxel_size * 5;
     const double R = std::max(2 * rf + rn, grad_radius + rn) * 1.001 + 1e-4;
+    const char* efix = getenv("IBL_REUSE_FIXED_RADIUS");
+    const bool fixed = efix && atoi(efix);
+    const ibl_instance_features* feat[2] = {c.det_features, c.mem_features};
+    HostTables h = {ps.J, ps.jobs.data(), ps.job_off.data(), {c.det_off_host, c.mem_off_host}, {nullptr, nullptr}, {nullptr, nullptr}, {0.0f, 0.0f}};
+    for (int pl = 0; pl < 2; ++pl) {
+        if (!feat[pl]) continue;
+        h.bbox[pl] = feat[pl]->bbox;
+        if (!fixed && feat[pl]->reach2 && feat[pl]->seg_reach2) h.seg_reach2[pl] = feat[pl]->seg_reach2;
+        if (pl == 1 && grad_radius > rf) h.floor2[pl] = nextafterf((float)(grad_radius * grad_radius), INFINITY);
+    }
     list_near_candidates(h, R, &plan);
-    st = test_near_pairs(ctx, ps, R);
+    st = test_near_pairs(ctx, ps, h, R);
     if (st) return st;
     ps.phase("near-pair test");
     plan_feature_reuse(h, &plan);
diff --git a/instance-based-loc_amd/csrc/reg_stages.h b/instance-based-loc_amd/csrc/reg_stages.h
--- a/instance-based-loc_amd/csrc/reg_stages.h
+++ b/instance-based-loc_amd/csrc/reg_stages.h
@@ -33,7 +33,7 @@
 };
 struct GroupDesc { int pool; int seg[3]; };
 struct FeatCopy { int dst, src, count, kind; };
-struct NearPair { int pool, a, b, pad; float boxa[6], boxb[6]; };
+struct NearPair { int pool, a, b, pad; float boxa[6], boxb[6]; float ra2, rb2; };
 struct SidePairs { int qcnt[3]; int dcnt[3]; int pair[3][3]; };
 
 struct RansacState {
@@ -51,7 +51,7 @@
     int iter, done, started;
 };
 
-struct HostTables { int J; const JobDesc* jobs; const int* job_off; const int* off[2]; const float* bbox[2]; };
+struct HostTables { int J; const JobDesc* jobs; const int* job_off; const int* off[2]; const float* bbox[2]; const float* seg_reach2[2]; float floor2[2]; };
 struct SlotPlan { int dst, count, pool, seg, grp, pos, side, kind, src; };
 struct MatchPlan {
     std::vector<NearPair> near;
diff --git a/instance-based-loc_amd/engine.py b/instance-based-loc_amd/engine.py
--- a/instance-based-loc_amd/engine.py
+++ b/instance-based-loc_amd/engine.py
@@ -63,7 +63,7 @@
         key = (float(voxel_size), float(local_dist_factor))
         if key not in self._features:
             self._features[key] = instance_features_batch(self.ctx, self.clouds, voxel_size, 2.0 * (voxel_size * local_dist_factor),
-                                                          compact=self.compact_features)
+                                                          compact=self.compact_features, reach=True)
         return self._features[key]
 
     def close(self):
@@ -334,22 +334,31 @@
             arrays["fpfh_split"] = mem_feat.fpfh_split
         if mem_feat.grad is not None:
             arrays["grad"] = mem_feat.grad
-        store = InstanceStore(mem.lo, mem.clouds.seg_off_host, arrays, {"bbox": mem_feat.bbox})
+        per_instance = {"bbox": mem_feat.bbox}
+        if mem_feat.reach2 is not None:
+            arrays["reach2"] = mem_feat.reach2
+            per_instance["seg_reach2"] = mem_feat.seg_reach2
+        store = InstanceStore(mem.lo, mem.clouds.seg_off_host, arrays, per_instance)
 
         def compute(pool_pts, pool_off, n_home, arr, per_inst, mem_off, js, jt, ids):
             det_pool = CloudBatch(pool_pts.contiguous(), pool_off.astype(np.int32))
             feat = det_feat
             if det_pool.n_seg > n_home:
                 b0 = int(pool_off[n_home])
-                extra = instance_features_batch(ctx, CloudBatch(pool_pts[b0:].contiguous(), (pool_off[n_home:] - b0).astype(np.int32)), voxel)
+                extra = instance_features_batch(ctx, CloudBatch(pool_pts[b0:].contiguous(), (pool_off[n_home:] - b0).astype(np.int32)), voxel,
+                                                reach=det_feat.reach2 is not None)
                 feat = InstanceFeatures(torch.cat([det_feat.normals[:clean.n], extra.normals]), torch.cat([det_feat.fpfh[:clean.n], extra.fpfh]),
                                         torch.cat([det_feat.fpfh_split[:clean.n], extra.fpfh_split]),
                                         torch.cat([det_feat.fpfh_norm[:clean.n], extra.fpfh_norm]), None,
-                                        np.concatenate([det_feat.bbox[:clean.n_seg], extra.bbox]), voxel, 0.0)
+                                        np.concatenate([det_feat.bbox[:clean.n_seg], extra.bbox]), voxel, 0.0,
+                                        torch.cat([det_feat.reach2[:clean.n], extra.reach2]) if det_feat.reach2 is not None else None,
+                                        np.concatenate([det_feat.seg_reach2[:clean.n_seg], extra.seg_reach2]) if det_feat.reach2 is not None else None)
             mem_pool = CloudBatch(arr["pts"].contiguous(), np.asarray(mem_off).astype(np.int32))
             mf = InstanceFeatures(arr["normals"].contiguous(), arr["fpfh"].contiguous(), arr["fpfh_split"].contiguous() if "fpfh_split" in arr else None,
                                   arr["fpfh_norm"].contiguous(), arr["grad"].contiguous() if "grad" in arr else None,
-                                  np.ascontiguousarray(per_inst["bbox"]), mem_feat.voxel_size, mem_feat.grad_radius)
+                                  np.ascontiguousarray(per_inst["bbox"]), mem_feat.voxel_size, mem_feat.grad_radius,
+                                  arr["reach2"].contiguous() if "reach2" in arr else None,
+                                  np.ascontiguousarray(per_inst["seg_reach2"]) if "seg_reach2" in per_inst else None)
             r = register_batch(ctx, det_pool, mem_pool, js, jt, voxel, gdf, ldf, seed=seed, ransac_max_iter=ransac_max_iter,
                                have_colors=True, center=True, det_features=feat, mem_features=mf, job_ids=ids)
             return {k: r[k] for k in ("T", "rmse", "fitness", "means", "T_ransac", "ransac_stats")}
@@ -443,7 +452,7 @@
             return results
         det_feat = mem_feat = None
         if self.reuse_features:
-            det_feat = instance_features_batch(ctx, clean, fpfh_voxel_size)
+            det_feat = instance_features_batch(ctx, clean, fpfh_voxel_size, reach=True)
             mem_feat = mem.features(fpfh_voxel_size, fpfh_local_dist_factor)
         tick("det_features")
         if self.route is not None:
diff --git a/instance-based-loc_amd/registration.py b/instance-based-loc_amd/registration.py
--- a/instance-based-loc_amd/registration.py
+++ b/instance-based-loc_amd/registration.py
@@ -131,12 +131,14 @@
 class _FeatStruct(C.Structure):
     _fields_ = [("normals4", C.c_void_p), ("fpfh", C.c_void_p), ("fpfh_split", C.c_void_p), ("fpfh_norm", C.c_void_p),
                 ("grad4", C.c_void_p), ("bbox", C.c_void_p),
-                ("voxel_size", C.c_double), ("grad_radius", C.c_double)]
+                ("voxel_size", C.c_double), ("grad_radius", C.c_double), ("reach2", C.c_void_p), ("seg_reach2", C.c_void_p)]
 
 
 class InstanceFeatures:
 
-    def __init__(self, normals, fpfh, fpfh_split, fpfh_norm, grad, bbox, voxel_size, grad_radius):
+    def __init__(self, normals, fpfh, fpfh_split, fpfh_norm, grad, bbox, voxel_size, grad_radius, reach2=None, seg_reach2=None):
+        assert (reach2 is None) == (seg_reach2 is None)
+        self.reach2, self.seg_reach2 = reach2, seg_reach2
         self.normals, self.fpfh, self.grad, self.bbox = normals, fpfh, grad, bbox
         self.fpfh_split, self.fpfh_norm = fpfh_split, fpfh_norm
         self.voxel_size, self.grad_radius = float(voxel_size), float(grad_radius)
@@ -145,11 +147,13 @@
         return _FeatStruct(self.normals.data_ptr(), self.fpfh.data_ptr(), self.fpfh_split.data_ptr() if self.fpfh_split is not None else None,
                            self.fpfh_norm.data_ptr(),
                            self.grad.data_ptr() if self.grad is not None else None,
-                           self.bbox.ctypes.data, self.voxel_size, self.grad_radius)
+                           self.bbox.ctypes.data, self.voxel_size, self.grad_radius,
+                           self.reach2.data_ptr() if self.reach2 is not None else None,
+                           self.seg_reach2.ctypes.data if self.seg_reach2 is not None else None)
 
 
 def instance_features_batch(ctx: RegContext, batch: CloudBatch, voxel_size: float, grad_radius: float = 0.0,
-                            compact: bool = False) -> InstanceFeatures:
+                            compact: bool = False, reach: bool = False) -> InstanceFeatures:
     dev = batch.pts4.device
     n = max(batch.n, 1)
     normals = torch.empty((n, 4), dtype=torch.float32, device=dev)
@@ -158,12 +162,15 @@
     fpfh_norm = torch.empty((n,), dtype=torch.float32, device=dev)
     grad = torch.empty((n, 4), dtype=torch.float32, device=dev) if grad_radius > 0 else None
     bbox = np.zeros((max(batch.n_seg, 1), 6), dtype=np.float32)
+    reach2 = torch.empty((n,), dtype=torch.float32, device=dev) if reach else None
+    seg_reach2 = np.zeros((max(batch.n_seg, 1), 1), dtype=np.float32) if reach else None
     st = _lib.lib.ibl_instance_features_batch(ctx.handle, batch.pts4.data_ptr(), batch.seg_off.data_ptr(), batch.seg_off_host.ctypes.data,
                                               batch.n_seg, float(voxel_size), float(grad_radius), normals.data_ptr(), fpfh.data_ptr(),
                                               fpfh_split.data_ptr() if fpfh_split is not None else None, fpfh_norm.data_ptr(),
-                                              grad.data_ptr() if grad is not None else None, bbox.ctypes.data, _stream())
+                                              grad.data_ptr() if grad is not None else None, bbox.ctypes.data,
+                                              reach2.data_ptr() if reach else None, seg_reach2.ctypes.data if reach else None, _stream())
     _lib.check(st, "ibl_instance_features_batch")
-    return InstanceFeatures(normals, fpfh, fpfh_split, fpfh_norm, grad, bbox, voxel_size, grad_radius)
+    return InstanceFeatures(normals, fpfh, fpfh_split, fpfh_norm, grad, bbox, voxel_size, grad_radius, reach2, seg_reach2)
 
 
 REG_HAVE_COLORS = 1
```

Result: no change. 826.2 query-frames/s (-0.9%).
